# csiro-crop-informatics/biokanga

Hardware: AMD Instinct MI355X
Metric: aligned reads/s (SAM-identical) on 100 bp SE vs GRCh38, 1->8 MI355X (higher is better)
Workload: dtype u8

## Files before the change

biokanga_amd/csrc/bk_ctx_int.h:

```cpp
#pragma once
#include <atomic>
#include <thread>
#include <hip/hip_runtime.h>

#include <cstdio>
#include <string>
#include <vector>

#include "bk_device.h"
#include "bk_devbuf.h"

#define HIP_TRY(expr)                                                                              \
    do {                                                                                           \
        hipError_t e__ = (expr);                                                                   \
        if (e__ != hipSuccess) {                                                                   \
            fprintf(stderr, "biokanga_amd: %s failed: %s (%s:%d)\n", #expr, hipGetErrorString(e__), __FILE__, __LINE__); \
            return e__ == hipErrorOutOfMemory ? BK_ERR_MEM : BK_ERR_INTERNAL;                      \
        }                                                                                          \
    } while (0)

namespace bk {
struct BatchBufs {
    DevBuf<uint64_t> rd4, rd2, iv_first;
    DevBuf<uint2> iv2, iv32;
    DevBuf<uint32_t> iv_n, rmeta;
    DevBuf<uint32_t> act[2], heavy, wave, wave_work;
    DevBuf<uint32_t> stage[3], stripe_cnt;
    DevBuf<uint32_t> slist, slist_stage;
    DevBuf<uint32_t> sort[3];
    DevBuf<uint8_t> sort_tmp, scan_tmp;
    DevBuf<bk_seg2> seg2;
    DevBuf<uint8_t> in_bases;
    DevBuf<uint64_t> in_offs;
    DevBuf<uint32_t> in_lens;
    DevBuf<bk_hit> in_out;
    DevBuf<uint16_t> in_lens16;
    DevBuf<uint32_t> in_words;
    DevBuf<bk_nbase> in_exc;
    DevBuf<bk_snp_site> snp_sites;
    DevBuf<bk_site_req> site_reqs;
    DevBuf<bk_site_res> site_res;
    DevBuf<uint8_t> chrom_accept;
    DevBuf<unsigned long long> htab;
    DevBuf<uint32_t> slot_epoch;
    DevBuf<uint2> plan;
};
struct ImageBufs {
    DevBuf<uint64_t> tgt4, tgt2, tgt2s;
    DevBuf<uint32_t> sa_lo, isa;
    DevBuf<uint8_t> sa_hi, nflag;
    DevBuf<uint64_t> ent_start, ent_end;
    DevBuf<uint32_t> ent_id, id2idx;
    DevBuf<uint8_t> ktab;
    DevBuf<uint64_t> ktab_hi;
    DevBuf<uint32_t> k2, kx[kMoreKeys];
    DevBuf<uint8_t> swin;
    DevBuf<uint32_t> swmap;
    DevBuf<uint32_t> grow_kx[kMoreKeys];
    DevBuf<uint8_t> grow_ktab2;
};
struct FixedBufs {
    DevBuf<uint32_t> small;
    DevBuf<PhaseCtl> ctl;
    DevBuf<unsigned long long> seq_counts, ctr, ctr_aux, snp_tot;
    DevBuf<unsigned long long> seq_global;
    DevBuf<uint32_t> snp_planes;
};
}

struct bk_ctx {
    int device = 0;
    hipStream_t stream = nullptr;
    bk_align_params params{};
    bk::DevAlignCfg cfg{};
    bk::DevIndex ix{};
    bk::ImageBufs image;
    bk::FixedBufs fixed;
    void release_image_buffers() { image = bk::ImageBufs{}; fixed = bk::FixedBufs{}; }
    uint64_t n_tgt4_words = 0;
    uint32_t cap_rd2w = 0;
    int use_tgt2 = 2;
    int sort_lists = 7;
    bool sort_lists_set = false;
    int sort_shift = 0;
    int use_k2 = 1;
    int use_k3 = bk::kMoreKeys;
    bool grow_enabled = false, grow_wait = false;
    uint64_t grow_after = 5 * BK_POLICY_MIN_READS, grow_seen = 0;
    std::atomic<int> grow_state{0};
    std::thread grow_thread;
    bk::DevIndex grow_ix{};
    bool grow_want_ktab2 = false;
    bool grow_elem = false, grow_want_elem = false;
    int use_ktab2 = 1;
    bool ktab_is2 = false;
    int use_iv32 = 1;
    uint32_t wave_waves = 256u * 8u * 4u;
    int use_isa = 1;
    int use_swin = 1;
    uint64_t swin_budget = 0;
    int swin_skip_short = 0;
    int swin_w = 0;
    uint64_t swin_bytes = 0;
    double swin_setup_s = 0;
    double swin_covered = 0;
    bool swin_denied = false;
    bool swin_rebuilt = false;
    int iv_poison = 0;
    int use_wave = 1;
    int lazy_search = 1;
    bool ktab64 = false;
    int ktab_wide = 0;
    int k_req = -1;
    int use_ktab = 1;
    uint32_t el_size = 4;
    uint64_t tot_seq_len = 0;
    std::string dataset;
    std::vector<bk_entry_info> entries;
    std::vector<bk_snp_site> snp_sites;

    bk::BatchBufs buf;
    void release_batch_buffers() { buf = bk::BatchBufs{}; }
    uint32_t cap_reads = 0, cap_wpr = 0, cap_iv_cores = 0;
    uint32_t *h_small = nullptr;
    bk::PhaseCtl *h_ctl = nullptr;
    hipEvent_t ev_ctl = nullptr;
    bool ctl_pending = false, hist_valid = false;
    uint32_t ctl_pending_reads = 0, ctl_pending_maxlen = 0;
    int ctl_pending_phases = 0;
    double hist_slist[bk::kMaxPhases] = {0}, hist_wave[bk::kMaxPhases] = {0};
    int async_error = 0;
    int async_phases = 1;
    bool force_rccl = false;
    uint64_t rccl_allreduces = 0;
    int rccl_ranks = 0;
    uint2 *h_plan = nullptr;
    size_t h_plan_cap = 0;
    uint32_t plan_maxlen = 0;
    int plan_key[4] = {-1, -1, -1, -1};
    hipEvent_t ev_plan = nullptr;
    bk::HeavyScratch hs{};
    int max_read_len = 500;
    uint32_t last_maxlen = 0;
    int dbg_stop_phase = -1, dbg_phase = 0, dbg_cur = 0;
    uint32_t dbg_n = 0, dbg_ivc = 0;
    bool dbg_valid = false;
    bool debug = false;
    uint32_t chunk_reads = 64u << 20;
    uint64_t site_chunk = 8u << 20;

    hipEvent_t ev_wait = nullptr;
    bool entries_set = false, tgt2_built = false;
    bool tables_built = false;
    bool tables_under_way = false;
    void *sam_text[2] = {nullptr, nullptr};
    uint64_t sam_text_cap = 0;
    uint32_t n_chrom_accept = 0;
    bk_timing timing{};
    std::vector<hipEvent_t> ev_pool;
    std::vector<uint64_t> loci_offs;
    std::vector<bk_loci> loci;
    std::vector<bk_loci_trims> loci_trims;
    std::vector<bk_seg2> seg2;
};


namespace bk {
struct DevReads {
    const uint8_t *bases = nullptr;
    const uint64_t *offs = nullptr;
    const uint32_t *lens = nullptr;
    const uint32_t *words = nullptr;
    const bk_nbase *exc = nullptr;
    uint64_t n_exc = 0;
};
int engine_align_device(bk_ctx *c, const DevReads &in, uint32_t nreads, bk_hit *d_out, hipStream_t s, uint32_t maxlen_known = 0);
void release_swin(bk_ctx *c);
void drop_swin(bk_ctx *c);
int engine_pair_device(bk_ctx *c, const DevReads &in, uint32_t n_pairs, bk_hit *d_hits, uint32_t maxlen, const bk_pe_params *pe, hipStream_t s,
                       bk_seg2 *seg2_host = nullptr, bk_seg2 *seg2_dev = nullptr);
int engine_prepare_packed(bk_ctx *c, const uint16_t *d_lens16, uint32_t nreads, uint64_t n_words, const bk_nbase *d_exc, uint64_t n_exc,
                          uint32_t *d_lens32, uint64_t *d_offs, uint32_t *maxlen, hipStream_t s);
}

namespace bk {
hipError_t dev_malloc_bytes(void **p, size_t bytes);
hipError_t dev_zero_now(void *p, size_t bytes);
template <class T> inline hipError_t dev_malloc(T **p, size_t bytes) { return dev_malloc_bytes(reinterpret_cast<void **>(p), bytes); }
int upload_host(void *d_dst, const void *h_src, size_t bytes, int device);
int upload_file(void *d_dst, int fd, uint64_t file_ofs, size_t bytes, int device);
bool host_is_pinned(const void *p);
}
```

biokanga_amd/csrc/bk_dev_k2.h:

```cpp
#pragma once
#include "bk_dev_util.h"

namespace bk {


constexpr uint32_t kKindShift = 30;
constexpr uint32_t kKindK2 = 1;
constexpr uint32_t kKindDeep = 2;
constexpr uint32_t kKindFull = 3;
constexpr uint32_t kInlineBucket = 16;
constexpr int kK2Bases = 15;
constexpr uint32_t kK2Above = 0xFFFFFFFFu;

constexpr uint64_t kTab2BitmapMax = 64;
__device__ __forceinline__ bool ktab2_absent(uint32_t bitmap, uint32_t m, uint32_t q2)
{
    const uint32_t m5 = m >> 27, lo5 = (q2 >> 27) & m5, hi5 = lo5 | (~m5 & 31u);
    const uint32_t upto = hi5 == 31u ? 0xFFFFFFFFu : (1u << (hi5 + 1)) - 1u;
    return (bitmap & upto & ~((1u << lo5) - 1u)) == 0u;
}

__device__ __forceinline__ int k2_cmp(uint32_t key, uint32_t m, uint32_t q2)
{
    if (key == kK2Above) return 1;
    key &= m;
    return key < q2 ? -1 : (key > q2 ? 1 : 0);
}
__device__ __forceinline__ bool k2_nkind(uint32_t key) { return key != kK2Above && (key & 3u) == 1u; }

__host__ __device__ __forceinline__ uint32_t k2_mask(int rem2)
{
    const int L = rem2 < kK2Bases ? rem2 : kK2Bases;
    return L <= 0 ? 0u : ~0u << (32 - 2 * L);
}

__device__ __forceinline__ uint32_t k2_make(const uint64_t *__restrict__ tgt4, uint64_t pos, int k)
{
    const uint64_t w0 = nib16(tgt4, pos);
    if (w0 & top_mask(k) & 0x4444444444444444ULL) return kK2Above;
    const uint64_t w1 = nib16(tgt4, pos + (uint64_t)k);
    const uint64_t bad = w1 & 0x4444444444444440ULL;
    const uint32_t code = squeeze2(w1) & ~3u;
    if (!bad) return code;
    const int j = __clzll((long long)bad) >> 2;
    return ((code | (0xFFFFFFFFu >> (2 * j))) & ~3u) | 1u;
}


#ifdef BK_DIAG_B
#define BK_K2_LINE(ctr) (ctr)++
#else
#define BK_K2_LINE(ctr) (void)0
#endif
__device__ __forceinline__ void k2_count_range(const uint32_t *__restrict__ L, uint64_t a, uint64_t b, uint32_t m, uint32_t q2, uint32_t &n_lt, uint32_t &n_le,
                                               unsigned long long &lines)
{
    n_lt = 0; n_le = 0;
    (void)lines;
    for (uint64_t base = a & ~15ULL; base < b; base += 16) {
        const uint4 *__restrict__ p = reinterpret_cast<const uint4 *>(L + base);
        const uint4 v0 = p[0], v1 = p[1], v2 = p[2], v3 = p[3];
        BK_K2_LINE(lines);
        const uint32_t key[16] = {v0.x, v0.y, v0.z, v0.w, v1.x, v1.y, v1.z, v1.w, v2.x, v2.y, v2.z, v2.w, v3.x, v3.y, v3.z, v3.w};
        const uint32_t lo = a > base ? (uint32_t)(a - base) : 0u, hi = b - base < 16 ? (uint32_t)(b - base) : 16u;
#pragma unroll
        for (uint32_t j = 0; j < 16; j++) {
            const bool in = j >= lo && j < hi;
            const uint32_t km = key[j] == kK2Above ? 0xFFFFFFFFu : (key[j] & m);
            n_lt += (in && km < q2) ? 1u : 0u;
            n_le += (in && km <= q2) ? 1u : 0u;
        }
        if ((uint64_t)n_le < base + hi - a) break;
    }
}

__device__ __forceinline__ void k2_bounds(const uint32_t *__restrict__ k2, const uint64_t *lv, uint64_t first, uint64_t cnt, uint32_t m, uint32_t q2,
                                          uint64_t &lb, uint64_t &ub, unsigned long long &lines)
{
    uint64_t l1 = first, h1 = first + cnt, l2 = l1, h2 = h1;
    int ktop = cnt >= 16 ? (63 - __clzll((long long)cnt)) >> 2 : 0;
    if (ktop > kK2Levels) ktop = kK2Levels;
    for (int j = ktop; j >= 0; j--) {
        const int sh = 4 * j;
        const uint32_t *__restrict__ L = j ? k2 + lv[j] : k2;
        const uint64_t a1 = l1 >> sh, b1 = h1 >> sh, a2 = l2 >> sh, b2 = h2 >> sh;
        uint32_t lt = 0, le = 0;
        if (a1 < b1) {
            k2_count_range(L, a1, b1, m, q2, lt, le, lines);
            const uint64_t g = a1 + lt;
            if (lt) l1 = g << sh;
            if (g < b1) h1 = ((g + 1) << sh) - 1;
        }
        if (a2 < b2) {
            if (a2 != a1 || b2 != b1) { uint32_t lt2; k2_count_range(L, a2, b2, m, q2, lt2, le, lines); }
            const uint64_t g = a2 + le;
            if (le) l2 = g << sh;
            if (g < b2) h2 = ((g + 1) << sh) - 1;
        }
    }
    lb = l1;
    ub = l2;
}

__device__ __forceinline__ uint32_t kx_make(const uint64_t *__restrict__ tgt4, uint64_t pos, int from, uint32_t before)
{
    if (before == kK2Above || (before & 3u) != 0u) return kK2Above;
    const uint64_t w1 = nib16(tgt4, pos + (uint64_t)from);
    const uint64_t bad = w1 & 0x4444444444444440ULL;
    const uint32_t code = squeeze2(w1) & ~3u;
    if (!bad) return code;
    const int j = __clzll((long long)bad) >> 2;
    return ((code | (0xFFFFFFFFu >> (2 * j))) & ~3u) | 1u;
}

template <typename Row>
__device__ __forceinline__ int cmp_core_from(const Row &rdw, int ofs, int cl, int start,
                                             const uint64_t *__restrict__ tgt, uint64_t pos)
{
    for (int i = start; i < cl; i += 16) {
        uint64_t m = top_mask(cl - i);
        uint64_t p = row_nib16(rdw, ofs + i) & m;
        uint64_t t = nib16(tgt, pos + i) & m;
        if (p != t) return p < t ? -1 : 1;
    }
    return 0;
}

}
```

biokanga_amd/csrc/bk_dev_util.h:

```cpp
#pragma once
#include "bk_device.h"

namespace bk {


__device__ __forceinline__ uint64_t nib16(const uint64_t *__restrict__ w, uint64_t pos)
{
    uint64_t i = pos >> 4;
    unsigned s = (unsigned)(pos & 15) << 2;
    uint64_t a = w[i];
    uint64_t b = w[i + 1];
    return (a << s) | ((b >> 1) >> (63 - s));
}

__device__ __forceinline__ uint64_t top_mask(int nibs)
{
    return nibs >= 16 ? ~0ULL : (~0ULL << (64 - 4 * nibs));
}

__device__ __forceinline__ uint64_t spread2to4(uint32_t v)
{
    uint64_t x = v;
    x = (x | (x << 16)) & 0x0000FFFF0000FFFFULL;
    x = (x | (x << 8)) & 0x00FF00FF00FF00FFULL;
    x = (x | (x << 4)) & 0x0F0F0F0F0F0F0F0FULL;
    x = (x | (x << 2)) & 0x3333333333333333ULL;
    return x;
}

__device__ __forceinline__ uint64_t bits64_2(const uint64_t *__restrict__ w, int pos)
{
    const int i = pos >> 5;
    const unsigned s = (unsigned)(pos & 31) << 1;
    const uint64_t a = w[i], b = w[i + 1];
    return (a << s) | ((b >> 1) >> (63 - s));
}

struct RdRow {
    const uint64_t *p;
    bool four;
    __device__ __forceinline__ uint64_t nib16(int pos) const
    {
        return four ? bk::nib16(p, (uint64_t)pos) : spread2to4((uint32_t)(bits64_2(p, pos) >> 32));
    }
    __device__ __forceinline__ uint64_t word16(int k) const
    {
        if (four) return p[k];
        const uint64_t v = p[k >> 1];
        return spread2to4((k & 1) ? (uint32_t)v : (uint32_t)(v >> 32));
    }
};

__device__ __forceinline__ RdRow read_row(const DevBatch &b, uint32_t r, int strand, bool has_n)
{
    RdRow q;
    q.four = b.rd2 == nullptr || has_n;
    q.p = q.four ? b.rd4 + ((uint64_t)r * 2 + strand) * b.wpr : b.rd2 + ((uint64_t)r * 2 + strand) * (b.nw / 2);
    return q;
}

__device__ __forceinline__ uint64_t iv_slot(const DevBatch &b, uint32_t a, int st, int c)
{
    return (uint64_t)(st * (int)b.iv_cores + c) * b.iv_stride + a;
}

__device__ __forceinline__ uint32_t iv_count(const DevBatch &b, uint64_t slot)
{
    return b.iv2 ? b.iv2[slot].y : b.iv_n[slot];
}
__device__ __forceinline__ uint64_t iv_start(const DevBatch &b, uint64_t slot)
{
    return b.iv2 ? (uint64_t)b.iv2[slot].x : b.iv_first[slot];
}
__device__ __forceinline__ void iv_get(const DevBatch &b, uint64_t slot, uint64_t &first, uint32_t &n)
{
    if (b.iv2) { const uint2 v = b.iv2[slot]; first = v.x; n = v.y; }
    else { first = b.iv_first[slot]; n = b.iv_n[slot]; }
}
__device__ __forceinline__ void iv_put(const DevBatch &b, uint64_t slot, uint64_t first, uint32_t n)
{
    if (b.iv2) b.iv2[slot] = make_uint2((uint32_t)first, n);
    else { b.iv_first[slot] = first; b.iv_n[slot] = n; }
}

__device__ __forceinline__ uint32_t stripe_reserve(const StripeSet &l, int li, uint32_t n)
{
    return atomicAdd(&l.cnt[(blockIdx.x & (kListStripes - 1)) * 16 + li], n);
}
__device__ __forceinline__ void stripe_put(const StripeSet &l, int li, uint32_t at, uint32_t v)
{
    l.stage[li][(uint64_t)(blockIdx.x & (kListStripes - 1)) * l.cap + at] = v;
}
__device__ __forceinline__ uint32_t stripe_reserve_tile(const StripeSet &l, int li, uint32_t n, uint64_t tile)
{
    return atomicAdd(&l.cnt[(uint32_t)(tile & (kListStripes - 1)) * 16 + li], n);
}
__device__ __forceinline__ void stripe_put_tile(const StripeSet &l, int li, uint32_t at, uint32_t v, uint64_t tile)
{
    l.stage[li][(tile & (kListStripes - 1)) * l.cap + at] = v;
}
__device__ __forceinline__ void stripe_max(const StripeSet &l, uint32_t v)
{
    atomicMax(&l.cnt[(kListStripes + (blockIdx.x & (kListStripes - 1))) * 16], v);
}

__device__ __forceinline__ uint32_t ctr_stripe() { return (blockIdx.x & (kCtrStripes - 1)) * 8; }

template <bool WIDE>
__device__ __forceinline__ uint64_t sa_get(const DevIndex &ix, uint64_t i)
{
    uint64_t v = ix.sa_lo[i];
    if (WIDE) v |= (uint64_t)ix.sa_hi[i] << 32;
    return v;
}

__device__ __forceinline__ uint64_t row_nib16(const uint64_t *__restrict__ rdw, int pos) { return nib16(rdw, (uint64_t)pos); }
__device__ __forceinline__ uint64_t row_nib16(const RdRow &rdw, int pos) { return rdw.nib16(pos); }

template <typename Row>
__device__ __forceinline__ int cmp_core(const Row &rdw, int ofs, int cl, uint64_t p0,
                                        const uint64_t *__restrict__ tgt, uint64_t pos)
{
    uint64_t t0 = nib16(tgt, pos) & top_mask(cl);
    if (p0 != t0) return p0 < t0 ? -1 : 1;
    for (int i = 16; i < cl; i += 16) {
        uint64_t m = top_mask(cl - i);
        uint64_t p = row_nib16(rdw, ofs + i) & m;
        uint64_t t = nib16(tgt, pos + i) & m;
        if (p != t) return p < t ? -1 : 1;
    }
    return 0;
}

struct LdsEntries {
    uint64_t start[128], end[128];
    bool on;
};
__device__ __forceinline__ void lds_entries_load(LdsEntries &le, const DevIndex &ix)
{
    le.on = ix.n_ent <= 128;
    if (le.on)
        for (uint32_t i = threadIdx.x; i < ix.n_ent; i += blockDim.x) { le.start[i] = ix.ent_start[i]; le.end[i] = ix.ent_end[i]; }
    __syncthreads();
}

__device__ __forceinline__ int find_entry(const DevIndex &ix, uint64_t t)
{
    int lo = 0, hi = (int)ix.n_ent - 1;
    while (lo <= hi) {
        int mid = (lo + hi) >> 1;
        if (t < ix.ent_start[mid]) hi = mid - 1;
        else if (t > ix.ent_end[mid]) lo = mid + 1;
        else return mid;
    }
    return -1;
}

__device__ __forceinline__ int find_entry_lds(const LdsEntries &le, const DevIndex &ix, uint64_t t)
{
    if (!le.on) return find_entry(ix, t);
    int lo = 0, hi = (int)ix.n_ent - 1;
    while (lo <= hi) {
        int mid = (lo + hi) >> 1;
        if (t < le.start[mid]) hi = mid - 1;
        else if (t > le.end[mid]) lo = mid + 1;
        else return mid;
    }
    return -1;
}

__device__ __forceinline__ int hamming(const uint64_t *__restrict__ rdw, int len, const uint64_t *__restrict__ tgt,
                                       uint64_t t, int limit)
{
    int mm = 0;
    for (int i = 0; i < len; i += 16) {
        uint64_t x = (nib16(rdw, i) ^ nib16(tgt, t + i)) & top_mask(len - i);
        x = (x | (x >> 1) | (x >> 2) | (x >> 3)) & 0x1111111111111111ULL;
        mm += __popcll(x);
        if (mm > limit) break;
    }
    return mm;
}

__device__ __forceinline__ int hamming_eos(const uint64_t *__restrict__ rdw, int len, const uint64_t *__restrict__ tgt,
                                           uint64_t t, int limit)
{
    int mm = 0;
    uint64_t eos = 0;
    for (int i = 0; i < len; i += 16) {
        const uint64_t w = nib16(tgt, t + i), m = top_mask(len - i);
        eos |= w & (w >> 1) & (w >> 2) & m & 0x1111111111111111ULL;
        uint64_t x = (nib16(rdw, i) ^ w) & m;
        x = (x | (x >> 1) | (x >> 2) | (x >> 3)) & 0x1111111111111111ULL;
        mm += __popcll(x);
    }
    return (eos || mm > limit) ? 127 : mm;
}

__device__ __forceinline__ uint32_t squeeze2(uint64_t x)
{
    x &= 0x3333333333333333ULL;
    x = (x | (x >> 2)) & 0x0F0F0F0F0F0F0F0FULL;
    x = (x | (x >> 4)) & 0x00FF00FF00FF00FFULL;
    x = (x | (x >> 8)) & 0x0000FFFF0000FFFFULL;
    x = (x | (x >> 16)) & 0x00000000FFFFFFFFULL;
    return (uint32_t)x;
}

__device__ __forceinline__ uint32_t flags_to_bits16(uint64_t f)
{
    uint64_t g = __brevll(f) >> 3;
    g = (g | (g >> 3)) & 0x0303030303030303ULL;
    g = (g | (g >> 6)) & 0x000F000F000F000FULL;
    g = (g | (g >> 12)) & 0x000000FF000000FFULL;
    g = (g | (g >> 24)) & 0xFFFFULL;
    return (uint32_t)g;
}

__device__ __forceinline__ uint64_t ktab_get(const DevIndex &ix, uint64_t c)
{
    if (ix.ktab2) return (uint64_t)ix.ktab2[c].x;
    if (ix.ktab_hi) return ix.ktab_hi[c >> 16] + (uint64_t)ix.ktab32[c];
    return ix.ktab32 ? (uint64_t)ix.ktab32[c] : ix.ktab64[c];
}

__device__ __forceinline__ void ktab_get_pair(const DevIndex &ix, uint64_t c, uint64_t &lo, uint64_t &hi)
{
    if (ix.ktab_hi && !ix.ktab2) {
        const uint64_t base = ix.ktab_hi[c >> 16];
        const uint32_t o0 = ix.ktab32[c], o1 = ix.ktab32[c + 1];
        lo = base + o0;
        hi = ((c + 1) & 0xFFFFULL) ? base + o1 : ix.ktab_hi[(c + 1) >> 16];
        return;
    }
    lo = ktab_get(ix, c);
    hi = ktab_get(ix, c + 1);
}

__device__ __forceinline__ void core_range(const DevIndex &ix, uint64_t p0, int cl, uint64_t &lo, uint64_t &hi)
{
    lo = 0;
    hi = ix.n;
    int k = ix.k;
    if (k <= 0) return;
    int kk = cl < k ? cl : k;
    if (p0 & 0x4444444444444444ULL & top_mask(kk)) return;
    uint32_t code = squeeze2(p0);
    uint64_t c_lo = (uint64_t)(code >> (32 - 2 * kk)) << (2 * (k - kk));
    uint64_t c_hi = c_lo | ((1ULL << (2 * (k - kk))) - 1);
    lo = ktab_get(ix, c_lo);
    hi = ktab_get(ix, c_hi + 1);
}

template <bool WIDE, typename Row>
__device__ __forceinline__ void search_core(const DevIndex &ix, const Row &rdw, int ofs, int cl,
                                            uint64_t cap, uint64_t &first, uint64_t &count)
{
    uint64_t p0 = row_nib16(rdw, ofs) & top_mask(cl);
    uint64_t lo, hi;
    core_range(ix, p0, cl, lo, hi);
    uint64_t end = hi;
    while (lo < hi) {
        uint64_t mid = lo + ((hi - lo) >> 1);
        int c = cmp_core(rdw, ofs, cl, p0, ix.tgt4, sa_get<WIDE>(ix, mid));
        if (c > 0) lo = mid + 1;
        else hi = mid;
    }
    first = lo;
    count = 0;
    if (lo >= end) return;
    if (cmp_core(rdw, ofs, cl, p0, ix.tgt4, sa_get<WIDE>(ix, lo)) != 0) return;
    if (end - lo == 1) { count = 1; return; }
    uint64_t limit = end - lo < cap ? end : lo + cap;
    uint64_t cur = lo, step = 1;
    while (cur + step < limit && cmp_core(rdw, ofs, cl, p0, ix.tgt4, sa_get<WIDE>(ix, cur + step)) == 0) {
        cur += step;
        step <<= 1;
    }
    uint64_t l2 = cur + 1, h2 = cur + step < limit ? cur + step : limit;
    while (l2 < h2) {
        uint64_t mid = l2 + ((h2 - l2) >> 1);
        if (cmp_core(rdw, ofs, cl, p0, ix.tgt4, sa_get<WIDE>(ix, mid)) == 0) l2 = mid + 1;
        else h2 = mid;
    }
    count = l2 - lo;
}

__device__ __forceinline__ int classify(int low_inst, int low_mm, int nxt, int init, int mm_delta, int max_hits)
{
    if (low_inst == 0 && low_mm == init) return BK_HR_NONE;
    if (low_inst >= 1 && (nxt - low_mm) < mm_delta) return BK_HR_MMDELTA;
    if (low_inst > max_hits) return BK_HR_HITINSTS;
    return BK_HR_HITS;
}

__device__ __forceinline__ void write_result(const DevIndex &ix, const DevAlignCfg &cfg, const DevBatch &b, uint32_t r,
                                             int len, int rslt, int low_inst, int low_mm, int nxt, uint64_t hit_left,
                                             int hit_ent, int hit_strand, int diag)
{
    bk_hit h;
    h.chrom_id = 0; h.match_loci = 0; h.match_len = 0; h.low_hit_instances = 0;
    h.rslt = (uint8_t)rslt; h.nar = BK_NAR_NOHIT; h.strand = '?'; h.low_mm = 0; h.nxt_low_mm = 0;
    h.num_hits = 0; h.mismatches = 0;
    h.flags = (uint8_t)diag;
    if (low_inst > cfg.max_hits) low_inst = cfg.max_hits + 1;
    switch (rslt) {
    case BK_HR_HITS:
        if (low_inst == 1) {
            h.nar = BK_NAR_ACCEPTED;
            h.num_hits = 1;
            h.strand = (uint8_t)hit_strand;
            h.chrom_id = ix.ent_id[hit_ent];
            h.match_loci = (uint32_t)(hit_left - ix.ent_start[hit_ent]);
            h.match_len = (uint16_t)len;
            h.mismatches = (uint8_t)low_mm;
        } else
            h.nar = BK_NAR_MULTIALIGN;
        break;
    case BK_HR_MMDELTA:
        h.nar = BK_NAR_MMDELTA;
        h.match_len = (uint16_t)len;
        break;
    case BK_HR_HITINSTS:
        h.nar = BK_NAR_MULTIALIGN;
        h.match_len = (uint16_t)len;
        break;
    default:
        break;
    }
    h.low_hit_instances = (int16_t)low_inst;
    h.low_mm = (int8_t)low_mm;
    h.nxt_low_mm = (int8_t)nxt;
    b.out[r] = h;
}

__device__ __forceinline__ uint64_t uniform64(uint64_t v)
{
    uint32_t lo = __builtin_amdgcn_readfirstlane((uint32_t)v), hi = __builtin_amdgcn_readfirstlane((uint32_t)(v >> 32));
    return ((uint64_t)hi << 32) | lo;
}

constexpr uint32_t kLazyBucket = 4;
constexpr uint32_t kLazyFlag = 0x80000000u;
constexpr uint32_t kElemFlag = 0x40000000u;
constexpr uint32_t kIvFlags = kLazyFlag | kElemFlag;
constexpr int kWaveGrab = 8;

void launch_fill_u64(unsigned long long *p, uint64_t n, unsigned long long v, hipStream_t s);
void launch_pack_rows(const DevBatch &b, hipStream_t s, const uint32_t *pairs = nullptr, uint32_t n_pairs = 0);
struct CompactJobs { StripeSet set; uint32_t *dense[3]; uint32_t *total[3]; uint32_t *max_out; int n; };
inline uint32_t stripe_cap(unsigned blocks, unsigned per_block) { return ((blocks + kListStripes - 1) / kListStripes) * per_block; }
void launch_compact(const StripeSet &set, uint32_t *const *dense, uint32_t *const *total, int n, uint32_t *max_out, hipStream_t s);
void expand_rd4(const DevBatch &b, const uint32_t *list, uint32_t n_list, hipStream_t s);

}
```

biokanga_amd/csrc/bk_device.h:

```cpp
#pragma once
#include <hip/hip_runtime.h>
#include <stdint.h>

#include "../../include/biokanga_amd.h"

namespace bk {

constexpr int kMoreKeys = 2;
constexpr int kK2Levels = 7;

__host__ __device__ __forceinline__ uint64_t k2s_pad(uint64_t words) { return (words + 15) & ~15ULL; }
__host__ __device__ __forceinline__ uint64_t k2s_count(uint64_t n, int j) { return (n + (1ULL << (4 * j)) - 1) >> (4 * j); }
__host__ __device__ __forceinline__ uint64_t k2s_start(uint64_t n, int j)
{
    uint64_t o = k2s_pad(n) + 16;
    for (int i = 1; i < j; i++) o += k2s_pad(k2s_count(n, i)) + 16;
    return o;
}


constexpr int kListStripes = 64;
struct StripeSet {
    uint32_t *cnt;
    uint32_t *stage[3];
    uint32_t cap;
};
constexpr int kCtrStripes = 64;
constexpr int kNwLong = 20;
constexpr int kNwLongest = 32;
constexpr int kPackedPadWords = 32;
constexpr int kMaxCoresFast = 16;
constexpr int kWave = 64;
constexpr int kMaxReadLenAbs = 2000;
constexpr uint32_t kNodeCap = 1024000;
constexpr uint64_t kEosWord = 0x7777777777777777ULL;
constexpr int kSwBases = 192, kSwPre = 92, kSwLen = 100;
template <int E> struct SwGeo { static constexpr int bases = 64 * E, pre = E == 3 ? 92 : 32 * E; };
template <int E> __host__ __device__ inline uint64_t sw_word_at(uint64_t idx, int q) { return (idx >> 5) * (32ULL * E) + (uint64_t)q * 32 + (idx & 31); }
constexpr int kSwBlkShift = 5;
constexpr uint32_t kSwNone = 0xFFFFFFFFu;
constexpr uint32_t kSwMinRun = 65, kSwHead = 192;
constexpr int kSwLevels = 8;
constexpr uint32_t kReadHasN = 1u << 15;
constexpr uint32_t kReadLenMask = kReadHasN - 1;

struct DevIndex {
    const uint64_t *tgt4;
    const uint64_t *tgt2;
    const uint64_t *tgt2s;
    const uint8_t *nflag;
    int flag_shift;
    uint32_t nflag_bytes;
    const uint32_t *sa_lo;
    const uint8_t *sa_hi;
    const uint64_t *ent_start;
    const uint64_t *ent_end;
    const uint32_t *ent_id;
    const uint32_t *id2idx;
    uint32_t max_id;
    const uint32_t *ktab32;
    const uint64_t *ktab64;
    const uint64_t *ktab_hi;
    const uint2 *ktab2;
    int ktab2_elem;
    const uint32_t *k2;
    const uint32_t *kx[kMoreKeys];
    const uint32_t *isa;
    const uint4 *swin;
    int sw_words;
    const uint32_t *swmap;
    uint64_t n;
    uint32_t n_ent;
    int k;
};

struct DevAlignCfg {
    int max_subs, mm_delta, align_strand, max_ns, max_hits;
    int min_core_len, slides_per100, max_iter;
    int heavy_thresh;
};

struct DevBatch {
    const uint8_t *bases;
    const uint64_t *offs;
    const uint32_t *lens;
    const uint32_t *pk_words;
    const bk_nbase *pk_exc;
    uint64_t pk_nexc;
    uint32_t pk_read0;
    uint64_t *rd4;
    uint64_t *rd2;
    uint32_t *rmeta;
    uint64_t *iv_first;
    uint32_t *iv_n;
    uint2 *iv2;
    uint32_t iv_stride;
    const uint32_t *act;
    uint32_t *wave_work;
    uint2 *iv32;
    bk_hit *out;
    unsigned long long *seq_counts;
    unsigned long long *ctr;
    uint32_t wpr;
    uint32_t n_reads;
    uint32_t nw;
    uint32_t iv_cores;
    const uint2 *plan;
    uint32_t plan_stride;
    uint32_t plan_n;
};

struct PhaseCtl {
    uint32_t n_act;
    uint32_t cmax;
    uint32_t n_slist;
    uint32_t n_wave;
    uint32_t n_heavy;
    uint32_t wave_cursor, heavy_cursor;
    uint32_t pad[9];
};
constexpr int kMaxPhases = 72;

struct HeavyScratch {
    unsigned long long *htab;
    uint32_t *slot_epoch;
    uint32_t tab_size;
    uint32_t n_slots;
};

struct ReadPlan {
    int len, max_tot_mm, core_len, core_delta, max_slides, n_loop, n_phases;
};

__host__ __device__ inline ReadPlan make_plan(int len, const DevAlignCfg &c)
{
    ReadPlan p;
    p.len = len;
    int m = c.max_subs == 0 ? 0 : (int)(0.5 + (double)(len * c.max_subs) / 100.0);
    if (c.max_subs != 0 && m < 1) m = 1;
    if (m > 63) m = 63;
    p.max_tot_mm = m;
    int cl = len / (c.mm_delta == 1 ? m + 1 : m + 2);
    p.core_len = cl > c.min_core_len ? cl : c.min_core_len;
    int ms = (c.slides_per100 * len + 99) / 100;
    p.max_slides = ms > 1 ? ms : 1;
    int cd = len / p.max_slides - 1;
    p.core_delta = cd > p.core_len ? cd : p.core_len;
    p.n_loop = 0;
    int has_final = 1;
    if (m > 0) {
        int a;
        for (a = 0; a <= m; a++) {
            if (len / (a + c.mm_delta) <= p.core_len) break;
            p.n_loop++;
        }
        has_final = a <= m;
    }
    p.n_phases = p.n_loop + has_final;
    return p;
}

__host__ __device__ inline void phase_params(const ReadPlan &p, const DevAlignCfg &c, int phase, int &mm, int &cl, int &cd)
{
    if (phase < p.n_loop) {
        mm = phase;
        cl = p.len / (phase + c.mm_delta);
        cd = cl;
    } else {
        mm = p.max_tot_mm;
        cl = p.core_len;
        cd = p.core_delta;
    }
}

__host__ __device__ inline int core_offsets(int plen, int cl, int cd, int max_slides, int *ofs, int maxn)
{
    int cur = cd, o = 0, n = 0;
    while (n < max_slides && o <= plen - cl && cur > cl / 3) {
        if (o + cl + cur > plen) cur = plen - (o + cl);
        n++;
        o += cur;
    }
    const int last = plen - cl;
    for (int i = 0; i < maxn; i++) {
        int v = i * cd;
        ofs[i] = v < last ? v : last;
    }
    return n;
}

}
```

biokanga_amd/csrc/bk_engine_int.h:

```cpp
#pragma once
#include <hip/hip_runtime.h>
#include <fcntl.h>
#include <unistd.h>
#include "bk_prim.h"

#include <algorithm>
#include <cstdio>
#include <cstdlib>
#include <ctime>
#include <cstring>
#include <map>
#include <mutex>
#include <string>
#include <atomic>
#include <thread>
#include <type_traits>
#include <vector>

#include <dlfcn.h>
#include <rccl/rccl.h>

#include "bk_ctx_int.h"
#include "bk_cpus.h"
#include "bk_wait.h"
#include "bk_env.h"
#include "sfx_file.h"


namespace bk {
void launch_pack_target(const uint8_t *seq, uint64_t n, uint64_t *tgt4, uint64_t nwords, hipStream_t s);
void launch_pack_target2(const uint64_t *tgt4, uint64_t nwords4, uint64_t *tgt2, unsigned int *nflag32, int flag_shift, hipStream_t s);
void launch_split_sa5(const uint8_t *sa5, uint64_t n, uint32_t *lo, uint8_t *hi, hipStream_t s);
void launch_build_ktab(const DevIndex &ix, void *tab, int k, bool tab64, hipStream_t s, uint64_t i0 = 0, uint64_t i1 = 0, unsigned long long *starts = nullptr, bool pairs = false);
void launch_fill_ktab2_y(void *tab2, const uint32_t *k2, uint64_t n_entries, hipStream_t s, const uint32_t *sa_elem = nullptr);
void launch_max_len(const uint32_t *lens, uint32_t n, uint32_t *out, hipStream_t s);
void launch_widen_lens(const uint16_t *lens16, uint32_t n, uint32_t *lens32, unsigned long long *nwords, hipStream_t s);
void launch_check_exc(const bk_nbase *exc, uint64_t n_exc, const uint32_t *lens, uint32_t n_reads, uint32_t *bad, hipStream_t s);
void launch_packed_extent(const uint64_t *offs, const uint32_t *lens, uint32_t n, unsigned long long *out, hipStream_t s);
void launch_snp_pileup(const DevIndex &ix, const uint8_t *bases, const uint64_t *offs, const uint32_t *id2idx, const bk_snp_aln *alns, uint64_t n_alns,
                       uint32_t *planes, hipStream_t s);
void launch_site_octamers(const DevIndex &ix, const bk_site_req *reqs, uint64_t n, int32_t rel_ofs, bk_site_res *out, hipStream_t s);
void launch_snp_gather(const DevIndex &ix, const uint32_t *planes, uint64_t g0, uint32_t n, uint32_t *out, hipStream_t s);
void launch_snp_centroids(const DevIndex &ix, const uint32_t *planes, uint64_t g0, uint32_t chrom_len, uint32_t min_reads, uint32_t *hist, hipStream_t s);
void launch_snp_sites(const DevIndex &ix, const uint32_t *planes, uint64_t g0, uint32_t chrom_len, uint32_t min_reads, double min_prop,
                      bk_snp_site *sites, uint32_t cap, uint32_t *n_sites, unsigned long long *totals, hipStream_t s);
void launch_count_seqs(const bk_hit *out, uint32_t n, const uint32_t *id2idx, uint32_t n_ent, unsigned long long *counts, hipStream_t s);
void launch_fill_u64(unsigned long long *p, uint64_t n, unsigned long long v, hipStream_t s);
void launch_prep(const DevAlignCfg &cfg, const DevBatch &b, uint32_t *act, uint32_t *act_cnt, uint32_t *cmax, uint32_t *stage,
                 uint32_t *stripe_cnt, hipStream_t s);
void launch_search(const DevIndex &ix, const DevAlignCfg &cfg, const DevBatch &b, const uint32_t *act, uint32_t n_act,
                   int phase, int cmax, int nstr, int lazy, hipStream_t s);
void launch_extend(const DevIndex &ix, const DevAlignCfg &cfg, const DevBatch &b, const uint32_t *act, uint32_t n_act,
                   int phase, uint32_t *next_act, uint32_t *next_cnt, uint32_t *heavy, uint32_t *heavy_cnt,
                   uint32_t *cmax_next, hipStream_t s);
void launch_build_isa(const uint32_t *sa, uint64_t n, uint32_t *isa, hipStream_t s, uint64_t i0 = 0, uint64_t i1 = 0);
void launch_build_swin(const DevIndex &ix, void *swin, int words, hipStream_t s);
void launch_swin_breaks(const DevIndex &ix, const int *w, int n_levels, unsigned long long *const *brk, uint64_t a, uint64_t e, uint64_t n_words,
                        const unsigned long long *starts, hipStream_t s);
void launch_swin_cover(const unsigned long long *brk, uint64_t n, uint32_t max_run, uint32_t min_run, uint32_t *flags, uint64_t n_blocks, int first_level, hipStream_t s);
void launch_pack_ktab64(const uint64_t *tab, uint64_t n_entries, uint32_t *off, uint64_t *hi, uint32_t *overflow, hipStream_t s);
void launch_count_nonzero(const uint32_t *flags, uint64_t n, unsigned long long *count, hipStream_t s);
void launch_swin_map(const uint32_t *flags, const uint32_t *incl, uint64_t n_blocks, uint32_t cap_blocks, uint32_t *used, uint32_t *map, hipStream_t s);
void launch_swin_fill(const DevIndex &ix, const uint32_t *map, void *swin, int words, uint64_t a, uint64_t e, hipStream_t s);
void launch_build_k2(const DevIndex &ix, uint32_t *k2, uint32_t *k3, uint32_t *k4, unsigned long long *bad, hipStream_t s, uint64_t i0 = 0, uint64_t i1 = 0, bool write_k2 = true);
void launch_build_k2_levels(uint32_t *k2, uint64_t n, hipStream_t s);
void launch_make_ktab2(const uint32_t *tab, const uint32_t *k2, uint64_t n_entries, uint64_t n, void *out, hipStream_t s, const uint32_t *sa_elem = nullptr);
void launch_search_a(const DevIndex &ix, const DevAlignCfg &cfg, const DevBatch &b, const uint32_t *act, const uint32_t *p_n_act, uint32_t n_act_bound,
                     int phase, int cmax, int nstr, int lazy, uint32_t *list, uint32_t *list_cnt, uint32_t *stage, uint32_t *stripe_cnt,
                     hipStream_t s);
void launch_search_b(const DevIndex &ix, const DevAlignCfg &cfg, const DevBatch &b, int phase, int lazy, const uint32_t *list, const uint32_t *sorted,
                     uint32_t n_sorted, const uint32_t *p_n_list, uint64_t n_bound, hipStream_t s);
void launch_clear_iv(const DevBatch &b, const uint32_t *p_n_act, uint32_t n_act_bound, int cmax, int st0, int st1, uint32_t word, hipStream_t s);
void launch_pe(const DevIndex &ix, const DevAlignCfg &cfg, const DevBatch &b, int pe_mode, int min_len, int max_len, int pair_strand,
               bk_hit *hits, uint32_t n_pairs, uint32_t *orphans, uint32_t *counters, uint32_t *h_count, bk_seg2 *seg2, int min_chim,
               int long_reads, const uint8_t *accept, uint32_t n_accept, hipStream_t s);
void launch_flat(const DevIndex &ix, const DevAlignCfg &cfg, const DevBatch &b, const uint32_t *act, const uint32_t *p_n_act, uint32_t n_act_bound, int phase,
                 int slots_max, uint32_t *next_act, uint32_t *next_cnt, uint32_t *heavy, uint32_t *heavy_cnt, uint32_t *wave,
                 uint32_t *wave_cnt, uint32_t *cmax_next, uint32_t *const *stage, uint32_t *stripe_cnt, int nw, hipStream_t s);
void launch_wave(const DevIndex &ix, const DevAlignCfg &cfg, const DevBatch &b, const HeavyScratch &hs, const uint32_t *list, const uint32_t *sorted,
                 uint32_t n_sorted, const uint32_t *p_n_list, uint32_t n_bound, int phase, uint32_t *cursor, uint32_t *next_act, uint32_t *next_cnt,
                 uint32_t *cmax_next, int nw, uint32_t max_waves, hipStream_t s);
void launch_heavy(const DevIndex &ix, const DevAlignCfg &cfg, const DevBatch &b, const HeavyScratch &hs, const uint32_t *list,
                  uint32_t n_list, int phase, uint32_t *cursor, uint32_t *next_act, uint32_t *next_cnt, uint32_t *cmax_next,
                  hipStream_t s);
int build_sa_device(const uint8_t *d_seq, uint64_t n, void *d_sa_out, int el_size, hipStream_t s);
int scan_counts_u64(const unsigned long long *in, unsigned long long *out, uint32_t n, void *tmp, size_t *tmp_bytes, hipStream_t s);
void launch_loci_count(const bk_hit *out, uint32_t n, int clamp_to, unsigned long long *cnt, hipStream_t s);
void launch_best(const DevIndex &ix, const DevAlignCfg &cfg, const DevBatch &b, const HeavyScratch &hs, const uint32_t *list,
                 uint32_t n_list, uint32_t *cursor, unsigned long long *cnt, bk_loci *dense, hipStream_t s);
void launch_indel(const DevIndex &ix, const DevAlignCfg &cfg, const DevBatch &b, uint32_t n, int max_indel, int max_junct, int keep_state, uint32_t *list,
                  uint32_t *list_cnt_dev, uint32_t *list_cnt_host, uint32_t *cursor, bk_seg2 *seg2, hipStream_t s);
void launch_unaligned_list(const bk_hit *out, uint32_t n, uint32_t *list, uint32_t *cnt, hipStream_t s);
void launch_chimeric(const DevIndex &ix, const DevAlignCfg &cfg, const DevBatch &b, const HeavyScratch &hs, const uint32_t *list, uint32_t n_list,
                     int min_pct, int long_reads, uint32_t *cursor, bk_seg2 *seg2, hipStream_t s);
void launch_loci_compact(const bk_loci *dense, uint32_t width, const unsigned long long *offs, uint32_t n, bk_loci *out, hipStream_t s);
void launch_loci_single(const bk_hit *out, uint32_t n, const unsigned long long *offs, bk_loci *loci, uint32_t *list, uint32_t *list_cnt,
                        const bk_seg2 *seg2, bk_loci_trims *trims, hipStream_t s);
void launch_loci_enum(const DevIndex &ix, const DevAlignCfg &cfg, const DevBatch &b, const HeavyScratch &hs, const uint32_t *list,
                      uint32_t n_list, uint32_t *cursor, const unsigned long long *offs, bk_loci *loci, uint32_t *err, int min_pct, int long_reads,
                      bk_seg2 *seg2, bk_loci_trims *trims, hipStream_t s);
int sort_list_by_key(const uint32_t *keys_in, uint32_t *keys_out, const uint32_t *vals_in, uint32_t *vals_out, uint32_t n,
                     void *tmp, size_t *tmp_bytes, hipStream_t s);
void launch_keys_search(const DevBatch &b, const uint32_t *list, const uint32_t *p_n, uint32_t n_sort, int shift, uint32_t *keys, hipStream_t s);
void launch_keys_wave(const DevAlignCfg &cfg, const DevBatch &b, int phase, const uint32_t *list, const uint32_t *p_n, uint32_t n_sort, int shift, uint32_t *keys,
                      const uint32_t *work_of, hipStream_t s);

struct StageClock {
    bool on = env::timing();
    double t0 = now();
    static double now() { timespec ts; clock_gettime(CLOCK_MONOTONIC, &ts); return (double)ts.tv_sec + 1e-9 * (double)ts.tv_nsec; }
    static double wall() { timespec ts; clock_gettime(CLOCK_REALTIME, &ts); return (double)(ts.tv_sec % 60) + 1e-9 * (double)ts.tv_nsec; }
    void lap(const char *what) { if (!on) return; const double t = now(); fprintf(stderr, "bk timing: %-28s %7.1f ms   (done at :%06.3f)\n", what, 1e3 * (t - t0), wall()); t0 = t; }
};


inline uint32_t words_per_read(uint32_t maxlen)
{
    return ((maxlen + 15) / 16 + 2) & ~1u;
}

inline uint32_t iv_cores_for(const bk_ctx *c, uint32_t maxlen)
{
    const uint32_t ms = std::max(1u, ((uint32_t)c->cfg.slides_per100 * maxlen + 99) / 100);
    return std::min<uint32_t>(ms, kMaxCoresFast);
}

inline uint32_t rd2w_for(uint32_t maxlen)
{
    return maxlen <= 128 ? 4u : (maxlen <= 256 ? 8u : (maxlen <= 16u * (uint32_t)kNwLong ? (uint32_t)kNwLong / 2 : (uint32_t)kNwLongest / 2));
}

inline uint64_t scratch_bytes_per_read(uint32_t wpr, uint32_t rd2w = 8, uint32_t iv_cores = kMaxCoresFast)
{
    return 2ULL * wpr * 8 + 2ULL * rd2w * 8 + 2ULL * iv_cores * (12 + 8) + 52 + 24;
}


int derive_cfg(bk_ctx *c);
hipError_t clear_dev(void *p, size_t bytes, hipStream_t s);
struct TablePlan {
    bool ktab = false, k2 = false, isa = false;
    bool ktab2 = false;
    int kx = 0;
    int k = 0;
    DevBuf<unsigned long long> d_bad;
};

int tables_begin(bk_ctx *c, TablePlan &tp);
int tables_range(bk_ctx *c, const TablePlan &tp, uint64_t i0, uint64_t i1, unsigned long long *bucket_starts = nullptr);
int tables_end(bk_ctx *c, TablePlan &tp);
int build_tables(bk_ctx *c);
int build_tgt2(bk_ctx *c);
void publish_index(bk_ctx *c);
void grow_take_in(bk_ctx *c);
void grow_drop(bk_ctx *c);
void grow_tick(bk_ctx *c, uint64_t nreads, bool now = false);
int setup_entries(bk_ctx *c, const bk_entry_info *entries, uint32_t n_entries);
int finish_ctx(bk_ctx *c, const bk_entry_info *entries, uint32_t n_entries);
int new_ctx(bk_ctx **out, int device_id, const bk_align_params *p, bk_ctx **pc);
int adopt_device_image(bk_ctx *c, const uint8_t *d_seq, uint64_t n, const uint8_t *d_sa, int el);
int maybe_build_swin(bk_ctx *c, uint32_t maxlen, uint32_t nreads, hipStream_t s);
int size_heavy_scratch(bk_ctx *c);
int ensure_batch_scratch(bk_ctx *c, uint32_t n_reads, uint32_t wpr, uint32_t rd2w = 0, uint32_t iv_cores = kMaxCoresFast);
int ensure_sort_scratch(bk_ctx *c, uint32_t n, hipStream_t s);
int ensure_slist(bk_ctx *c, uint64_t lanes, hipStream_t s);
int plan_table_for(bk_ctx *c, uint32_t maxlen, hipStream_t s);
bool plan_table_covers(const bk_ctx *c, uint32_t maxlen);
inline int ensure_seg2(bk_ctx *c, uint32_t n) { HIP_TRY(c->buf.seg2.ensure(n)); return BK_OK; }
struct HostExtent {
    uint64_t lo = ~0ULL, hi = 0;
    uint32_t maxlen = 0;
    std::vector<uint64_t> rel;
};
HostExtent host_extent(const uint64_t *offs, const uint32_t *lens, uint32_t nreads);
int align_device(bk_ctx *c, const DevReads &in, uint32_t nreads, bk_hit *d_out, hipStream_t s, uint32_t maxlen_known = 0, bool enqueue_only = false);
}
```

biokanga_amd/csrc/bk_env.h:

```cpp
#pragma once
#include <cstdlib>

namespace bk {
namespace env {

inline bool set(const char *name) { return getenv(name) != nullptr; }
inline unsigned long long u64(const char *name, unsigned long long dflt)
{
    const char *e = getenv(name);
    if (!e) return dflt;
    const unsigned long long v = strtoull(e, nullptr, 10);
    return v ? v : dflt;
}

inline bool timing() { static const bool v = set("BK_TIMING"); return v; }
inline bool debug_phases() { return set("BK_DEBUG"); }
inline int poison() { static const int v = set("BK_POISON") ? atoi(getenv("BK_POISON")) : -1; return v; }
inline bool inflate_debug() { static const bool v = set("BK_INFLATE_DEBUG"); return v; }
inline unsigned long long grow_after_reads() { return u64("BK_GROW_AFTER_READS", 0); }
inline unsigned long long table_slices() { return u64("BK_TABLE_SLICES", 0); }
inline unsigned long long sa_wide_chunk() { return u64("BK_SA_WIDE_CHUNK", 0); }
inline unsigned long long sam_device_min(unsigned long long dflt) { const char *e = getenv("BK_SAM_DEVICE_MIN"); return e ? strtoull(e, nullptr, 10) : dflt; }
inline unsigned long long sam_early_min(unsigned long long dflt) { const char *e = getenv("BK_SAM_EARLY_MIN"); return e ? strtoull(e, nullptr, 10) : dflt; }
inline bool sam_device_fail() { return set("BK_SAM_DEVICE_FAIL"); }
inline unsigned long long inflate_piece_min(unsigned long long dflt) { const char *e = getenv("BK_INFLATE_PIECE_MIN"); return e ? strtoull(e, nullptr, 10) : dflt; }
inline int local_world_size() { static const int v = [] { const char *e = getenv("LOCAL_WORLD_SIZE"); const int r = e ? atoi(e) : 1; return r > 1 ? r : 1; }(); return v; }

}
}
```

biokanga_amd/csrc/bk_image.cpp:

```cpp
#include "bk_engine_int.h"

#define SW_TRY(x) do { hipError_t e_ = (x); if (e_ != hipSuccess) { (void)hipGetLastError(); return e_ == hipErrorOutOfMemory ? BK_ERR_MEM : BK_ERR_INTERNAL; } } while (0)

namespace bk {
hipError_t dev_zero_now(void *p, size_t bytes)
{
    hipError_t e = hipMemset(p, 0, bytes);
    if (e == hipSuccess) e = hipStreamSynchronize(nullptr);
    return e;
}

hipError_t dev_malloc_bytes(void **p, size_t bytes)
{
    const int poison = env::poison();
    const bool timing = env::timing();
    timespec ta, tb;
    if (timing) clock_gettime(CLOCK_MONOTONIC, &ta);
    hipError_t e = hipMalloc(p, bytes);
    if (timing) {
        clock_gettime(CLOCK_MONOTONIC, &tb);
        const double ms = 1e3 * (double)(tb.tv_sec - ta.tv_sec) + 1e-6 * (double)(tb.tv_nsec - ta.tv_nsec);
        if (ms > 2.0) fprintf(stderr, "bk timing: hipMalloc of %.2f GB took %.1f ms\n", (double)bytes / 1e9, ms);
    }
    if (e == hipSuccess && poison >= 0 && bytes) {
        e = hipMemset(*p, poison & 0xff, bytes);
        if (e == hipSuccess) e = hipDeviceSynchronize();
    }
    return e;
}


int derive_cfg(bk_ctx *c)
{
    const bk_align_params &p = c->params;
    if (p.max_subs < 0 || p.max_subs > 25 || p.min_edit_dist < 1 || p.min_edit_dist > 2 || p.align_strand < 0 ||
        p.align_strand > 2 || p.pmode < 0 || p.pmode > 3 || p.max_ns < 0 || p.max_ns > 5)
        return BK_ERR_PARAMS;
    if (p.max_ml < 0 || p.max_ml > BK_MAX_ML) return BK_ERR_PARAMS;
    if (p.best_matches && p.max_ml < 2) return BK_ERR_PARAMS;
    if (p.micro_indel_len < 0 || p.micro_indel_len > 20) return BK_ERR_PARAMS;
    if ((p.micro_indel_len || p.splice_junct_len) && p.max_ml > 1 && p.best_matches) return BK_ERR_PARAMS;
    if (p.min_chimeric_len != 0 && (p.min_chimeric_len < 50 || p.min_chimeric_len > 99)) return BK_ERR_PARAMS;
    if (p.min_chimeric_len != 0 && p.max_ml > 1 && p.best_matches) return BK_ERR_PARAMS;
    if (p.splice_junct_len != 0 && (p.splice_junct_len < 25 || p.splice_junct_len > 100000)) return BK_ERR_PARAMS;
    DevAlignCfg &g = c->cfg;
    g.max_subs = p.max_subs;
    g.mm_delta = p.min_edit_dist;
    g.align_strand = p.align_strand;
    g.max_ns = p.max_ns;
    g.max_hits = p.max_ml > 1 ? p.max_ml : 1;
    uint64_t t = c->tot_seq_len;
    int m;
    if (t <= 500000ULL) m = 4;
    else if (t <= 20000000ULL) m = 7;
    else if (t <= 250000000ULL) m = 11;
    else if (t <= 3500000000ULL) m = 12;
    else m = 15;
    switch (p.pmode) {
    case 2: g.slides_per100 = 9; break;
    case 1: m += 1; g.slides_per100 = 8; break;
    case 0: m += 2; g.slides_per100 = 8; break;
    default: m += 4; g.slides_per100 = 6; break;
    }
    g.min_core_len = m;
    switch (p.pmode) {
    case 0: g.max_iter = 5000; break;
    case 1: g.max_iter = 10000; break;
    case 2: g.max_iter = 20000; break;
    default: g.max_iter = 2500; break;
    }
    if (g.heavy_thresh < 0 || g.heavy_thresh > 100) g.heavy_thresh = 64;
    return BK_OK;
}


void free_dev(void *p)
{
    if (!p) return;
    const bool timing = env::timing();
    timespec ta, tb;
    if (timing) clock_gettime(CLOCK_MONOTONIC, &ta);
    (void)hipFree(p);
    if (timing) {
        clock_gettime(CLOCK_MONOTONIC, &tb);
        const double ms = 1e3 * (double)(tb.tv_sec - ta.tv_sec) + 1e-6 * (double)(tb.tv_nsec - ta.tv_nsec);
        if (ms > 2.0) fprintf(stderr, "bk timing: hipFree took %.1f ms\n", ms);
    }
}

hipError_t clear_dev(void *p, size_t bytes, hipStream_t s)
{
    if (bytes < (1ULL << 30) || ((uintptr_t)p & 7)) {
        for (size_t at = 0; at < bytes; at += (1ULL << 30)) {
            hipError_t e = hipMemsetAsync((uint8_t *)p + at, 0, std::min<size_t>(1ULL << 30, bytes - at), s);
            if (e != hipSuccess) return e;
        }
        return hipSuccess;
    }
    const size_t words = bytes / 8;
    launch_fill_u64((unsigned long long *)p, words, 0ULL, s);
    hipError_t e = hipGetLastError();
    if (e == hipSuccess && (bytes & 7)) e = hipMemsetAsync((uint8_t *)p + words * 8, 0, bytes & 7, s);
    return e;
}


int pick_k(uint64_t n)
{
    int k = 1;
    while (k < 16 && (1ULL << (2 * k)) < n) k++;
    return k < 8 ? 8 : k;
}


void publish_index(bk_ctx *c)
{
    const ImageBufs &im = c->image;
    DevIndex &ix = c->ix;
    ix.tgt4 = im.tgt4.get(); ix.sa_lo = im.sa_lo.get(); ix.sa_hi = im.sa_hi.get();
    ix.ent_start = im.ent_start.get(); ix.ent_end = im.ent_end.get(); ix.ent_id = im.ent_id.get(); ix.id2idx = im.id2idx.get();
    const bool tabs = !c->tables_under_way;
    const void *kt = tabs ? im.ktab.get() : nullptr;
    const bool packed = c->ktab64 && im.ktab_hi.get() != nullptr, pairs = !c->ktab64 && c->ktab_is2;
    ix.ktab64 = c->ktab64 && !packed ? static_cast<const uint64_t *>(kt) : nullptr;
    ix.ktab_hi = packed ? im.ktab_hi.get() : nullptr;
    ix.ktab2 = pairs ? static_cast<const uint2 *>(kt) : nullptr;
    ix.ktab32 = packed || (!c->ktab64 && !pairs) ? static_cast<const uint32_t *>(kt) : nullptr;
    ix.k2 = tabs ? im.k2.get() : nullptr;
    for (int i = 0; i < kMoreKeys; i++) ix.kx[i] = tabs ? im.kx[i].get() : nullptr;
    ix.ktab2_elem = (ix.ktab2 != nullptr && c->use_ktab2 >= 2 && im.sa_hi.get() == nullptr && ix.k2 != nullptr) ? 1 : 0;
    ix.isa = tabs ? im.isa.get() : nullptr; ix.tgt2 = im.tgt2.get(); ix.tgt2s = im.tgt2s.get(); ix.nflag = im.nflag.get();
    ix.swin = reinterpret_cast<const uint4 *>(im.swin.get()); ix.swmap = im.swmap.get();
}

void grow_worker(bk_ctx *c)
{
    int st = 3;
    hipStream_t s = nullptr;
    DevBuf<unsigned long long> d_bad;
    ImageBufs &im = c->image;
    do {
        if (hipSetDevice(c->device) != hipSuccess || hipStreamCreateWithFlags(&s, hipStreamNonBlocking) != hipSuccess) break;
        const DevIndex &ix = c->grow_ix;
        const uint64_t n = ix.n;
        const uint64_t n_keys = k2s_start(n, kK2Levels + 1), need = n_keys * 4;
        int nk = 0;
        if (ix.k2 != nullptr && ix.kx[0] == nullptr) {
            for (int i = 0; i < kMoreKeys; i++) {
                size_t free_b = 0, total_b = 0;
                if (hipMemGetInfo(&free_b, &total_b) != hipSuccess || need > free_b || free_b - need < total_b / 5) break;
                if (im.grow_kx[i].ensure(n_keys) != hipSuccess) { (void)hipGetLastError(); break; }
                nk = i + 1;
            }
        }
        if (nk) {
            unsigned long long bad2[2] = {0, 0};
            bool ok = d_bad.ensure(2) == hipSuccess && hipMemsetAsync(d_bad.get(), 0, 16, s) == hipSuccess;
            if (ok) {
                launch_build_k2(ix, const_cast<uint32_t *>(ix.k2), im.grow_kx[0].get(), nk > 1 ? im.grow_kx[1].get() : nullptr, d_bad.get(), s, 0, n, false);
                ok = hipMemcpyAsync(bad2, d_bad.get(), 16, hipMemcpyDeviceToHost, s) == hipSuccess && hipStreamSynchronize(s) == hipSuccess && !bad2[0] && !bad2[1];
            }
            if (ok) {
                for (int i = 0; i < nk; i++) launch_build_k2_levels(im.grow_kx[i].get(), n, s);
                ok = hipStreamSynchronize(s) == hipSuccess;
            }
            if (!ok) {
                (void)hipGetLastError();
                for (auto &b : im.grow_kx) b.reset();
                nk = 0;
            }
        }
        if (c->grow_want_ktab2 && ix.k2 != nullptr && ix.ktab32 != nullptr) {
            const uint64_t n_entries = (1ULL << (2 * ix.k)) + 1;
            size_t free_b = 0, total_b = 0;
            if (hipMemGetInfo(&free_b, &total_b) == hipSuccess && n_entries * 8 + (total_b / 5) < free_b && im.grow_ktab2.ensure(n_entries * 8) == hipSuccess) {
                launch_make_ktab2(ix.ktab32, ix.k2, n_entries, n, im.grow_ktab2.get(), s, c->grow_want_elem ? ix.sa_lo : nullptr);
                if (hipStreamSynchronize(s) != hipSuccess) { (void)hipGetLastError(); im.grow_ktab2.reset(); }
            } else
                (void)hipGetLastError();
        }
        st = (nk || im.grow_ktab2.get()) ? 2 : 3;
    } while (false);
    if (s) (void)hipStreamDestroy(s);
    c->grow_state.store(st, std::memory_order_release);
}

void grow_take_in(bk_ctx *c)
{
    if (c->grow_thread.joinable()) c->grow_thread.join();
    if (c->grow_state.load(std::memory_order_acquire) == 2) {
        ImageBufs &im = c->image;
        for (int i = 0; i < kMoreKeys; i++)
            if (im.grow_kx[i].get()) im.kx[i] = std::move(im.grow_kx[i]);
        if (im.kx[0].get()) c->use_k3 = kMoreKeys;
        if (im.grow_ktab2.get()) {
            (void)hipDeviceSynchronize();
            im.ktab = std::move(im.grow_ktab2);
            c->ktab_is2 = true;
            c->use_ktab2 = c->grow_want_elem ? 2 : 1;
        }
        publish_index(c);
        if (!c->sort_lists_set) c->sort_lists = (c->sort_lists & ~1) | (c->ix.kx[0] == nullptr ? 1 : 0);
        if (env::timing())
            fprintf(stderr, "biokanga_amd: long-run tables taken in after %llu reads: %d key array(s) behind the second-level keys%s\n",
                    (unsigned long long)c->grow_seen, (c->ix.kx[0] != nullptr) + (c->ix.kx[1] != nullptr), c->ix.ktab2 ? ", first keys in the k-mer table" : "");
    }
    c->grow_state.store(4, std::memory_order_release);
}

void grow_drop(bk_ctx *c)
{
    if (c->grow_thread.joinable()) c->grow_thread.join();
    for (auto &b : c->image.grow_kx) b.reset();
    c->image.grow_ktab2.reset();
    if (c->grow_state.load() != 0) c->grow_state.store(4);
}

void grow_tick(bk_ctx *c, uint64_t nreads, bool now)
{
    if (!c->grow_enabled) return;
    const int st = c->grow_state.load(std::memory_order_acquire);
    if (st != 0 && st != 4) c->grow_seen += nreads;
    if (st == 0) {
        c->grow_seen += nreads;
        if ((now || c->grow_seen >= c->grow_after) && c->tables_built && c->ix.k2 != nullptr) {
            c->grow_ix = c->ix;
            c->grow_want_ktab2 = !c->ktab64 && !c->ktab_is2;
            c->grow_want_elem = c->grow_elem && c->image.sa_hi.get() == nullptr;
            c->grow_state.store(1);
            c->grow_thread = std::thread(grow_worker, c);
        }
    } else if (st == 2 || st == 3 || (st == 1 && c->grow_wait))
        grow_take_in(c);
}

int tables_begin(bk_ctx *c, TablePlan &tp)
{
    ImageBufs &im = c->image;
    grow_drop(c);
    im.ktab.reset(); im.ktab_hi.reset(); im.k2.reset(); im.isa.reset();
    for (auto &b : im.kx) b.reset();
    c->ktab_is2 = false;
    c->ix.k = 0;
    c->tables_under_way = true;
    publish_index(c);
    if (c->use_ktab) {
        int k = c->k_req > 0 ? c->k_req : pick_k(c->ix.n);
        if (k > 16) k = 16;
        if (k < 2) k = 2;
        const uint64_t ncodes = 1ULL << (2 * k);
        c->ktab64 = c->ix.n >= (1ULL << 32) || c->ktab_wide != 0;
        const uint64_t ktab_bytes = (ncodes + 1) * (c->ktab64 ? 8 : 4);
        const uint64_t need = k2s_start(c->ix.n, kK2Levels + 1) * 4;
        const bool want_isa = c->use_wave && c->use_isa && im.sa_hi.get() == nullptr && c->ix.n < (1ULL << 32);
        size_t free_b = 0, total_b = 0;
        HIP_TRY(hipMemGetInfo(&free_b, &total_b));
        uint64_t planned = ktab_bytes;
        auto fits = [&](uint64_t more) { return planned + more <= free_b && free_b - planned - more >= total_b / 5; };
        if (c->use_k2 && fits(need)) { tp.k2 = true; planned += need; }
        if (want_isa) planned += c->ix.n * 4;
        for (int i = 0; tp.k2 && i < kMoreKeys && i < c->use_k3; i++) {
            if (!fits(need)) break;
            tp.kx = i + 1;
            planned += need;
        }
        if (tp.k2 && c->use_ktab2 && !c->ktab64 && fits(ktab_bytes)) tp.ktab2 = true;
        HIP_TRY(im.ktab.ensure((size_t)ktab_bytes * (tp.ktab2 ? 2 : 1)));
        tp.ktab = true;
        tp.k = k;
        if (tp.k2) {
            HIP_TRY(im.k2.ensure(need / 4));
            HIP_TRY(tp.d_bad.ensure(2));
            HIP_TRY(hipMemsetAsync(tp.d_bad.get(), 0, 16, c->stream));
            for (int i = 0; i < tp.kx; i++) HIP_TRY(im.kx[i].ensure(need / 4));
        }
    }
    if (c->use_wave && c->use_isa && im.sa_hi.get() == nullptr && c->ix.n < (1ULL << 32)) {
        HIP_TRY(im.isa.ensure(c->ix.n));
        tp.isa = true;
    }
    return BK_OK;
}

int tables_range(bk_ctx *c, const TablePlan &tp, uint64_t i0, uint64_t i1, unsigned long long *bucket_starts)
{
    DevIndex ix = c->ix;
    ix.k = tp.k;
    const bool last = i1 >= c->ix.n;
    const ImageBufs &im = c->image;
    if (tp.ktab) launch_build_ktab(ix, im.ktab.get(), tp.k, c->ktab64, c->stream, i0, last ? c->ix.n + 1 : i1, bucket_starts, tp.ktab2);
    if (tp.k2) launch_build_k2(ix, im.k2.get(), tp.kx > 0 ? im.kx[0].get() : nullptr, tp.kx > 1 ? im.kx[1].get() : nullptr, tp.d_bad.get(), c->stream, i0, i1);
    if (tp.isa) launch_build_isa(im.sa_lo.get(), c->ix.n, im.isa.get(), c->stream, i0, i1);
    HIP_TRY(hipGetLastError());
    return BK_OK;
}

int tables_end(bk_ctx *c, TablePlan &tp)
{
    ImageBufs &im = c->image;
    unsigned long long bad2[2] = {0, 0};
    if (tp.k2) HIP_TRY(hipMemcpyAsync(bad2, tp.d_bad.get(), 16, hipMemcpyDeviceToHost, c->stream));
    HIP_TRY(hipStreamSynchronize(c->stream));
    if (tp.ktab && c->ktab64 && c->ktab_wide != 2) {
        const uint64_t n_entries = (1ULL << (2 * tp.k)) + 1, n_hi = (n_entries >> 16) + 2;
        DevBuf<uint8_t> d_off;
        DevBuf<uint64_t> d_hi;
        DevBuf<uint32_t> d_flag;
        uint32_t flag = 1;
        if (d_off.ensure(n_entries * 4) == hipSuccess && d_hi.ensure(n_hi) == hipSuccess && d_flag.ensure(1) == hipSuccess &&
            hipMemsetAsync(d_flag.get(), 0, 4, c->stream) == hipSuccess) {
            launch_pack_ktab64((const uint64_t *)im.ktab.get(), n_entries, (uint32_t *)d_off.get(), d_hi.get(), d_flag.get(), c->stream);
            if (hipMemcpyAsync(&flag, d_flag.get(), 4, hipMemcpyDeviceToHost, c->stream) != hipSuccess || hipStreamSynchronize(c->stream) != hipSuccess) flag = 1;
        }
        (void)hipGetLastError();
        d_flag.reset();
        if (flag == 0) {
            im.ktab = std::move(d_off);
            im.ktab_hi = std::move(d_hi);
        }
    }
    if (tp.ktab) {
        c->ktab_is2 = tp.ktab2;
        c->ix.k = tp.k;
    }
    const unsigned long long bad = bad2[0];
    if (tp.kx && (bad || bad2[1])) {
        if (!bad) fprintf(stderr, "biokanga_amd: suffix array not in nibble order at %llu place(s) beyond the second-level keys; third-level keys disabled\n", bad2[1]);
        for (auto &b : im.kx) b.reset();
        tp.kx = 0;
    }
    if (tp.k2 && bad) {
        fprintf(stderr, "biokanga_amd: suffix array not in nibble order inside %llu k-mer bucket(s); second-level keys disabled\n", bad);
        im.k2.reset();
    } else if (tp.k2) {
        launch_build_k2_levels(im.k2.get(), c->ix.n, c->stream);
        for (int i = 0; i < tp.kx; i++) launch_build_k2_levels(im.kx[i].get(), c->ix.n, c->stream);
        HIP_TRY(hipGetLastError());
    }
    c->tables_under_way = false;
    publish_index(c);
    if (tp.ktab2) {
        launch_fill_ktab2_y(im.ktab.get(), im.k2.get(), (1ULL << (2 * tp.k)) + 1, c->stream, c->ix.ktab2_elem ? im.sa_lo.get() : nullptr);
        HIP_TRY(hipGetLastError());
    }
    HIP_TRY(hipStreamSynchronize(c->stream));
    if (!c->sort_lists_set) c->sort_lists = (c->sort_lists & ~1) | (c->ix.kx[0] == nullptr ? 1 : 0);
    c->tables_built = true;
    return BK_OK;
}

int build_tables(bk_ctx *c)
{
    TablePlan tp;
    int rc = tables_begin(c, tp);
    if (!rc) rc = tables_range(c, tp, 0, c->ix.n);
    if (!rc) rc = tables_end(c, tp);
    return rc;
}

int build_tgt2(bk_ctx *c)
{
    ImageBufs &im = c->image;
    im.tgt2.reset(); im.nflag.reset(); im.tgt2s.reset();
    publish_index(c);
    if (!c->use_tgt2) return BK_OK;
    const uint64_t nblocks = c->n_tgt4_words / 4;
    static_assert(16 * kNwLongest <= 512, "a register-kernel window must not span more than two flag regions");
    int shift = 9;
    while ((((nblocks * 64) >> shift) + 7) / 8 > 16384) shift++;
    const uint64_t flag_bytes = (((((nblocks * 64) >> shift) + 1) + 31) / 32) * 4 + 16;
    HIP_TRY(im.tgt2.ensure(nblocks * 2 + 8));
    HIP_TRY(im.nflag.ensure(flag_bytes));
    HIP_TRY(hipMemsetAsync(im.nflag.get(), 0, flag_bytes, c->stream));
    HIP_TRY(hipMemsetAsync(im.tgt2.get() + nblocks * 2, 0, 64, c->stream));
    launch_pack_target2(im.tgt4.get(), c->n_tgt4_words, im.tgt2.get(), (unsigned int *)im.nflag.get(), shift, c->stream);
    HIP_TRY(hipGetLastError());
    HIP_TRY(hipStreamSynchronize(c->stream));
    c->ix.nflag_bytes = (uint32_t)flag_bytes;
    if (c->use_tgt2 >= 2) {
        HIP_TRY(im.tgt2s.ensure(nblocks * 2 + 8));
        HIP_TRY(clear_dev(im.tgt2s.get(), nblocks * 16 + 64, c->stream));
        HIP_TRY(hipMemcpyAsync(im.tgt2s.get(), im.tgt2.get() + 4, (nblocks * 2 - 4) * 8, hipMemcpyDeviceToDevice, c->stream));
        HIP_TRY(hipStreamSynchronize(c->stream));
    }
    c->ix.flag_shift = shift;
    publish_index(c);
    return BK_OK;
}


int setup_entries(bk_ctx *c, const bk_entry_info *entries, uint32_t n_entries)
{
    StageClock clk0;
    c->entries.assign(entries, entries + n_entries);
    c->tot_seq_len = 0;
    std::vector<uint64_t> es(n_entries), ee(n_entries);
    std::vector<uint32_t> ei(n_entries);
    for (uint32_t i = 0; i < n_entries; i++) {
        es[i] = entries[i].start_ofs;
        ee[i] = entries[i].end_ofs;
        ei[i] = entries[i].entry_id;
        c->tot_seq_len += entries[i].seq_len;
        if (i && es[i] <= ee[i - 1]) return BK_ERR_PARAMS;
    }
    ImageBufs &im = c->image; FixedBufs &fx = c->fixed;
    HIP_TRY(im.ent_start.ensure(n_entries));
    HIP_TRY(im.ent_end.ensure(n_entries));
    HIP_TRY(im.ent_id.ensure(n_entries));
    HIP_TRY(hipMemcpy(im.ent_start.get(), es.data(), n_entries * 8, hipMemcpyHostToDevice));
    HIP_TRY(hipMemcpy(im.ent_end.get(), ee.data(), n_entries * 8, hipMemcpyHostToDevice));
    HIP_TRY(hipMemcpy(im.ent_id.get(), ei.data(), n_entries * 4, hipMemcpyHostToDevice));
    {
        uint32_t max_id = 0;
        for (uint32_t i = 0; i < n_entries; i++) max_id = std::max(max_id, ei[i]);
        if ((uint64_t)max_id > 16ULL * n_entries + (1u << 20)) return BK_ERR_PARAMS;
        std::vector<uint32_t> map((size_t)max_id + 1, 0xFFFFFFFFu);
        for (uint32_t i = 0; i < n_entries; i++) map[ei[i]] = i;
        HIP_TRY(im.id2idx.ensure(map.size()));
        HIP_TRY(hipMemcpy(im.id2idx.get(), map.data(), map.size() * 4, hipMemcpyHostToDevice));
        c->ix.max_id = max_id;
    }
    c->ix.n_ent = n_entries;
    publish_index(c);
    HIP_TRY(fx.seq_counts.ensure(n_entries));
    HIP_TRY(dev_zero_now(fx.seq_counts.get(), n_entries * 8));
    HIP_TRY(fx.ctr.ensure((size_t)kCtrStripes * 8));
    HIP_TRY(dev_zero_now(fx.ctr.get(), (size_t)kCtrStripes * 8 * 8));
    HIP_TRY(fx.small.ensure(16));
    HIP_TRY(fx.ctl.ensure(kMaxPhases + 2));
    HIP_TRY(hipHostMalloc(&c->h_ctl, sizeof(PhaseCtl) * (kMaxPhases + 2)));
    HIP_TRY(bk::make_wait_event(&c->ev_ctl));
    HIP_TRY(bk::make_wait_event(&c->ev_wait));
    HIP_TRY(fx.ctr_aux.ensure(4));
    HIP_TRY(hipHostMalloc(&c->h_small, 2 * sizeof(PhaseCtl)));
    int rc = derive_cfg(c);
    clk0.lap("entry table, small buffers");
    return rc;
}

int finish_ctx(bk_ctx *c, const bk_entry_info *entries, uint32_t n_entries)
{
    int rc = c->entries_set ? BK_OK : setup_entries(c, entries, n_entries);
    if (rc) return rc;
    c->entries_set = true;
    StageClock clk;
    if (!c->tables_built) {
        rc = build_tables(c);
        clk.lap("k-mer table, second-level keys, inverse suffix array");
        if (rc) return rc;
    }
    if (!c->tgt2_built) {
        rc = build_tgt2(c);
        clk.lap("2-bit target");
    }
    return rc;
}

int new_ctx(bk_ctx **out, int device_id, const bk_align_params *p, bk_ctx **pc)
{
    if (!out || !p) return BK_ERR_PARAMS;
    *out = nullptr;
    int ndev = 0;
    if (hipGetDeviceCount(&ndev) != hipSuccess || ndev <= 0) return BK_ERR_NODEVICE;
    if (device_id < 0 || device_id >= ndev) return BK_ERR_PARAMS;
    HIP_TRY(hipSetDevice(device_id));
    bk_ctx *c = new bk_ctx();
    bk::live_contexts()++;
    c->device = device_id;
    c->params = *p;
    c->cfg.heavy_thresh = 64;
    c->debug = env::debug_phases();
    if (c->params.max_ml == 0) c->params.max_ml = 1;
    if (hipStreamCreate(&c->stream) != hipSuccess) { bk::live_contexts()--; delete c; return BK_ERR_INTERNAL; }
    *pc = c;
    return BK_OK;
}

int adopt_device_image(bk_ctx *c, const uint8_t *d_seq, uint64_t n, const uint8_t *d_sa, int el)
{
    c->el_size = (uint32_t)el;
    c->ix.n = n;
    uint64_t nwords = ((n + 15) / 16 + (kMaxReadLenAbs / 16) + 4 + 3) & ~3ULL;
    ImageBufs &im = c->image;
    HIP_TRY(im.tgt4.ensure(nwords));
    launch_pack_target(d_seq, n, im.tgt4.get(), nwords, c->stream);
    HIP_TRY(hipGetLastError());
    c->n_tgt4_words = nwords;
    c->sort_shift = 0;
    while ((n >> c->sort_shift) >= (1ULL << 32)) c->sort_shift++;
    if (d_sa == nullptr) {
        if (el != 4 || !im.sa_lo.get()) return BK_ERR_INTERNAL;
    } else {
        HIP_TRY(im.sa_lo.ensure(n));
        if (el == 5) {
            HIP_TRY(im.sa_hi.ensure(n));
            launch_split_sa5(d_sa, n, im.sa_lo.get(), im.sa_hi.get(), c->stream);
            HIP_TRY(hipGetLastError());
        } else
            HIP_TRY(hipMemcpyAsync(im.sa_lo.get(), d_sa, n * 4, hipMemcpyDeviceToDevice, c->stream));
    }
    HIP_TRY(hipStreamSynchronize(c->stream));
    publish_index(c);
    return BK_OK;
}


}

void bk::drop_swin(bk_ctx *c)
{
    c->image.swin.reset();
    c->image.swmap.reset();
    publish_index(c);
    c->swin_bytes = 0;
}

void bk::release_swin(bk_ctx *c)
{
    if (!c || !c->image.swin.get()) return;
    (void)hipSetDevice(c->device);
    if (c->stream) (void)hipStreamSynchronize(c->stream);
    (void)hipDeviceSynchronize();
    drop_swin(c);
    c->swin_denied = true;
    fprintf(stderr, "biokanga_amd: window array released to make room\n");
}


namespace bk {
struct SwinBuild {
    int w[kSwLevels] = {}, n_levels = 0;
    int words = 3;
    uint32_t max_run = 0, cap_blocks = 0;
    uint32_t min_run = kSwMinRun;
    int mode = 0;
    uint64_t done = 0;
    uint64_t range_cap = 0;
    DevBuf<unsigned long long> d_brk[kSwLevels];
    DevBuf<uint32_t> d_flags, d_incl, d_map, d_used;
    DevBuf<uint8_t> d_tmp, d_ent;
    size_t tmp_bytes = 0;
    DevBuf<unsigned long long> d_starts;
    std::thread ent_alloc;
    std::atomic<int> ent_state{0};
    DevBuf<uint8_t> ent_mem;
    uint64_t filled = 0;
    double t0 = 0;
    void drop_scratch() { for (auto &q : d_brk) q.reset(); d_flags.reset(); d_incl.reset(); d_tmp.reset(); d_starts.reset(); }
    ~SwinBuild() { if (ent_alloc.joinable()) ent_alloc.join(); }
    void take_ahead() { if (ent_state == 2) { if (ent_alloc.joinable()) ent_alloc.join(); if (ent_mem.get()) d_ent = std::move(ent_mem); } }
    void brk_ptrs(unsigned long long **out) { for (int l = 0; l < kSwLevels; l++) out[l] = d_brk[l].get(); }
    void alloc_ahead(int device, uint64_t bytes)
    {
        ent_state = 1;
        ent_alloc = std::thread([this, device, bytes]() {
            if (hipSetDevice(device) != hipSuccess || ent_mem.ensure(bytes) != hipSuccess) { (void)hipGetLastError(); ent_state = 3; return; }
            ent_state = 2;
        });
    }
};


int swin_core_lens_k(const bk_ctx *c, uint32_t maxlen, int k, int *w, double *wave_share = nullptr)
{
    const ReadPlan p = make_plan((int)std::max<uint32_t>(maxlen, 1), c->cfg);
    int n = 0;
    for (int ph = p.n_phases - 1; ph >= 0; ph--) {
        int mm, cl, cd;
        phase_params(p, c->cfg, ph, mm, cl, cd);
        cl = std::min(std::max(cl, k), 120);
        if (n == 0 || cl > w[n - 1]) {
            if (n == kSwLevels) break;
            w[n] = cl;
            if (wave_share) wave_share[n] = 0.0;
            n++;
        }
        if (wave_share && ph < kMaxPhases) wave_share[n - 1] += c->hist_wave[ph];
    }
    return n;
}
int swin_core_lens(const bk_ctx *c, uint32_t maxlen, int *w, bool skip_auto = false)
{
    double share[kSwLevels];
    int n = swin_core_lens_k(c, maxlen, c->ix.k, w, share);
    int skip = c->swin_skip_short > 0 ? std::min(c->swin_skip_short, n - 1) : 0;
    if (!skip && skip_auto && c->hist_valid) {
        double total = 0.0, acc = 0.0;
        for (int i = 0; i < n; i++) total += share[i];
        while (skip < n - 1 && acc + share[skip] < 0.05 * total) acc += share[skip++];
    }
    if (skip) { for (int i = skip; i < n; i++) w[i - skip] = w[i]; n -= skip; }
    return n;
}


int swin_begin(bk_ctx *c, SwinBuild &sb, const int *w, int n_levels, int words, uint64_t budget, uint64_t range_cap, int mode, hipStream_t s)
{
    const uint64_t n = c->ix.n;
    const uint64_t n_blocks = (n + (1u << kSwBlkShift) - 1) >> kSwBlkShift;
    sb.words = words;
    const uint64_t block_bytes = (uint64_t)(16 * words) << kSwBlkShift;
    sb.t0 = StageClock::now();
    sb.n_levels = n_levels;
    for (int l = 0; l < n_levels; l++) sb.w[l] = w[l];
    sb.max_run = c->cfg.max_iter > 0 ? (uint32_t)c->cfg.max_iter + 256u : 1u << 20;
    sb.cap_blocks = (uint32_t)std::min<uint64_t>(n_blocks, budget / block_bytes);
    if (sb.cap_blocks == 0) return 1;
    sb.range_cap = std::min<uint64_t>(range_cap, n) + 64;
    const uint64_t brk_words = (sb.range_cap >> 6) + 4, blocks = (sb.range_cap >> kSwBlkShift) + 2;
    for (int l = 0; l < n_levels; l++) SW_TRY(sb.d_brk[l].ensure(brk_words));
    SW_TRY(sb.d_flags.ensure(blocks));
    SW_TRY(sb.d_incl.ensure(blocks));
    SW_TRY(sb.d_map.ensure(n_blocks));
    SW_TRY(sb.d_used.ensure(1));
    SW_TRY(hipMemsetAsync(sb.d_used.get(), 0, 4, s));
    SW_TRY(bk::prim::inclusive_sum(nullptr, sb.tmp_bytes, sb.d_flags.get(), sb.d_incl.get(), (size_t)blocks, s));
    SW_TRY(sb.d_tmp.ensure(sb.tmp_bytes + 256));
    sb.mode = mode;
    if (mode == 1) {
        if (sb.ent_state == 0) SW_TRY(sb.d_ent.ensure((uint64_t)sb.cap_blocks * block_bytes));
        SW_TRY(sb.d_starts.ensure((n >> 6) + 4));
        SW_TRY(clear_dev(sb.d_starts.get(), ((n >> 6) + 4) * 8, s));
    }
    return BK_OK;
}

int swin_range(bk_ctx *c, SwinBuild &sb, const DevIndex &ix, uint64_t upto, hipStream_t s)
{
    const uint64_t n = ix.n;
    unsigned long long *brk[kSwLevels];
    sb.brk_ptrs(brk);
    while (sb.done < n) {
        uint64_t e = upto >= n ? n : (upto & ~63ULL);
        if (e > sb.done && e - sb.done > sb.range_cap - 64) e = (sb.done + sb.range_cap - 64) & ~63ULL;
        if (e <= sb.done) break;
        const uint64_t a = sb.done, len = e - a;
        const uint64_t n_words = (len >> 6) + 2, n_blocks = (len + (1u << kSwBlkShift) - 1) >> kSwBlkShift;
        launch_swin_breaks(ix, sb.w, sb.n_levels, brk, a, e, n_words, sb.d_starts.get(), s);
        for (int l = 0; l < sb.n_levels; l++) launch_swin_cover(brk[l], len, sb.max_run, sb.min_run, sb.d_flags.get(), n_blocks, l == 0, s);
        SW_TRY(hipGetLastError());
        size_t tb = sb.tmp_bytes;
        SW_TRY(bk::prim::inclusive_sum(sb.d_tmp.get(), tb, sb.d_flags.get(), sb.d_incl.get(), (size_t)n_blocks, s));
        launch_swin_map(sb.d_flags.get(), sb.d_incl.get(), n_blocks, sb.cap_blocks, sb.d_used.get(), sb.d_map.get() + (a >> kSwBlkShift), s);
        if (sb.d_ent.get() == nullptr) sb.take_ahead();
        if (sb.d_ent.get() == nullptr && sb.ent_state == 1) { sb.done = e; continue; }
        if (sb.d_ent.get() == nullptr && sb.ent_state == 3) return BK_ERR_MEM;
        if (sb.d_ent.get() == nullptr) {
            if (a != 0 || e != n) return BK_ERR_INTERNAL;
            uint32_t used = 0;
            SW_TRY(hipMemcpyAsync(&used, sb.d_used.get(), 4, hipMemcpyDeviceToHost, s));
            SW_TRY(hipStreamSynchronize(s));
            if (used == 0) { sb.done = e; return BK_OK; }
            sb.cap_blocks = used;
            SW_TRY(sb.d_ent.ensure((uint64_t)used * ((uint64_t)(16 * sb.words) << kSwBlkShift)));
        }
        launch_swin_fill(ix, sb.d_map.get(), sb.d_ent.get(), sb.words, sb.filled, e, s);
        SW_TRY(hipGetLastError());
        sb.filled = e;
        sb.done = e;
    }
    return BK_OK;
}

int swin_fit(bk_ctx *c, SwinBuild &sb, const DevIndex &ix, hipStream_t s)
{
    static const uint32_t ladder[] = {kSwMinRun, 96, 128, 160, 192, 224, 256, 288, 320, 352, 384, 416, 448, 480, 512, 576, 640, 704, 768, 832, 896, 960, 1024, 1088, 1152, 1216, 1280,
                                      1344, 1408, 1472, 1536, 1664, 1792, 1920, 2048, 2304, 2560, 3072, 4096, 6144, 8192};
    constexpr int NL = (int)(sizeof(ladder) / sizeof(ladder[0]));
    const uint64_t n = ix.n;
    DevBuf<unsigned long long> d_cnt;
    unsigned long long *brk[kSwLevels];
    sb.brk_ptrs(brk);
    SW_TRY(d_cnt.ensure(NL));
    SW_TRY(hipMemsetAsync(d_cnt.get(), 0, NL * 8, s));
    for (uint64_t a = 0; a < n;) {
        uint64_t e = std::min<uint64_t>(n, (a + sb.range_cap - 64) & ~63ULL);
        const uint64_t len = e - a, n_words = (len >> 6) + 2, n_blocks = (len + (1u << kSwBlkShift) - 1) >> kSwBlkShift;
        launch_swin_breaks(ix, sb.w, sb.n_levels, brk, a, e, n_words, nullptr, s);
        for (int q = 0; q < NL; q++) {
            if (ladder[q] > sb.max_run) break;
            for (int l = 0; l < sb.n_levels; l++) launch_swin_cover(brk[l], len, sb.max_run, ladder[q], sb.d_flags.get(), n_blocks, l == 0, s);
            launch_count_nonzero(sb.d_flags.get(), n_blocks, d_cnt.get() + q, s);
        }
        SW_TRY(hipGetLastError());
        a = e;
    }
    unsigned long long cnt[NL] = {};
    SW_TRY(hipMemcpyAsync(cnt, d_cnt.get(), NL * 8, hipMemcpyDeviceToHost, s));
    SW_TRY(hipStreamSynchronize(s));
    d_cnt.reset();
    int pick = 0;
    while (pick + 1 < NL && ladder[pick + 1] <= sb.max_run && cnt[pick] > sb.cap_blocks) pick++;
    sb.min_run = ladder[pick];
    const uint64_t blocks = std::min<uint64_t>(cnt[pick], sb.cap_blocks);
    if (blocks == 0) return 1;
    sb.cap_blocks = (uint32_t)blocks;
    SW_TRY(sb.d_ent.ensure(blocks * ((uint64_t)(16 * sb.words) << kSwBlkShift)));
    StageClock clk;
    if (clk.on) fprintf(stderr, "biokanga_amd: window array: runs of %u and more suffixes covered whole (the rule at 65: %.1f %% of the suffix array, this: %.1f %%, room for %.1f %%)\n", sb.min_run,
                        100.0 * (double)cnt[0] * 32.0 / (double)n, 100.0 * (double)cnt[pick] * 32.0 / (double)n, 100.0 * (double)blocks * 32.0 / (double)n);
    return BK_OK;
}

int swin_end(bk_ctx *c, SwinBuild &sb, hipStream_t s)
{
    if (sb.ent_alloc.joinable()) sb.ent_alloc.join();
    if (sb.ent_state == 3) return BK_ERR_MEM;
    if (sb.d_ent.get() == nullptr) sb.take_ahead();
    if (sb.d_ent.get() != nullptr && sb.filled < sb.done) {
        launch_swin_fill(c->ix, sb.d_map.get(), sb.d_ent.get(), sb.words, sb.filled, sb.done, s);
        sb.filled = sb.done;
    }
    uint32_t used = 0;
    SW_TRY(hipMemcpyAsync(&used, sb.d_used.get(), 4, hipMemcpyDeviceToHost, s));
    SW_TRY(hipStreamSynchronize(s));
    sb.drop_scratch();
    if (sb.done < c->ix.n) return BK_ERR_INTERNAL;
    if (used == 0) return 1;
    const uint64_t block_bytes = (uint64_t)(16 * sb.words) << kSwBlkShift;
    const uint64_t n_blocks = (c->ix.n + (1u << kSwBlkShift) - 1) >> kSwBlkShift;
    c->image.swin = std::move(sb.d_ent);
    c->image.swmap = std::move(sb.d_map);
    c->swin_w = sb.w[0] | (sb.w[sb.n_levels - 1] << 8) | (sb.n_levels << 16) | (sb.words << 24);
    c->ix.sw_words = sb.words;
    c->swin_bytes = (uint64_t)std::max(used, sb.cap_blocks) * block_bytes + n_blocks * 4;
    c->swin_covered = (double)used / (double)n_blocks;
    publish_index(c);
    c->swin_setup_s = StageClock::now() - sb.t0;
    return BK_OK;
}

uint64_t swin_budget_for(const bk_ctx *c, uint64_t free_b, uint64_t reserve, int words)
{
    const bool ranged = c->ix.n >= (1ULL << 32);
    const uint64_t span = ranged ? (1ULL << 31) : c->ix.n;
    const uint64_t work = ((span >> kSwBlkShift) + 1) * 8 + ((c->ix.n >> kSwBlkShift) + 1) * 4 + (span >> 3) * (kSwLevels + 1) + (64ULL << 20);
    if (free_b < reserve + work + (1ULL << 30)) return 0;
    uint64_t budget = std::min<uint64_t>(c->ix.n * 16 * (uint64_t)words / 3, ranged ? (free_b - reserve - work) / 16 * 15 : (free_b - reserve - work) / 2);
    if (c->swin_budget) budget = std::min<uint64_t>(budget, c->swin_budget);
    return budget;
}

int maybe_build_swin(bk_ctx *c, uint32_t maxlen, uint32_t nreads, hipStream_t s)
{
    ImageBufs &im = c->image;
    const bool wide = im.sa_hi.get() != nullptr || c->ix.n >= (1ULL << 32);
    if (!c->use_swin || c->swin_denied || !c->ix.tgt2 || (!wide && !c->ix.isa) || !c->ix.k2 || !c->use_wave) return BK_OK;
    if (wide && c->use_swin != 2) return BK_OK;
    const bool full = c->use_swin == 3;
    if (wide && !c->hist_valid && c->swin_skip_short == 0) return BK_OK;
    int w[kSwLevels];
    const int n_levels = swin_core_lens(c, maxlen, w, wide);
    const int words = maxlen <= 128 ? 3 : 5;
    const int w_key = w[0] | (w[n_levels - 1] << 8) | (n_levels << 16) | (words << 24);
    if (wide && im.swin.get() && c->ix.sw_words == words) return BK_OK;
    if (im.swin.get()) {
        if (full == (im.swmap.get() == nullptr) && (full ? c->ix.sw_words == words : (c->swin_w == w_key || (c->swin_rebuilt && c->ix.sw_words == words)))) return BK_OK;
        c->swin_rebuilt = true;
        HIP_TRY(hipStreamSynchronize(s));
        drop_swin(c);
    }
    if (c->use_swin == 1 && maxlen > 256) return BK_OK;
    size_t free_b = 0, total_b = 0;
    HIP_TRY(hipMemGetInfo(&free_b, &total_b));
    const uint64_t want = (uint64_t)std::min(nreads, c->chunk_reads) * scratch_bytes_per_read(words_per_read(maxlen), rd2w_for(maxlen), iv_cores_for(c, maxlen));
    const uint64_t have = (uint64_t)c->cap_reads * scratch_bytes_per_read(c->cap_wpr, c->cap_rd2w, c->cap_iv_cores);
    const uint64_t missing = want > have ? want - have : 0;
    const uint64_t reserve = missing * 4 / 3 + (6ULL << 30);
    StageClock clk;
    const double t0 = StageClock::now();
    if (full) {
        const uint64_t need = ((c->ix.n + 31) & ~31ULL) * 16 * (uint64_t)words;
        if ((uint64_t)free_b < need + reserve) { c->swin_denied = true; return BK_OK; }
        if (im.swin.ensure(need) != hipSuccess) { (void)hipGetLastError(); c->swin_denied = true; return BK_OK; }
        launch_build_swin(c->ix, im.swin.get(), words, s);
        HIP_TRY(hipGetLastError());
        HIP_TRY(hipStreamSynchronize(s));
        c->swin_bytes = need;
        c->swin_covered = 1.0;
        c->ix.sw_words = words;
    } else {
        const uint64_t budget = swin_budget_for(c, (uint64_t)free_b, reserve, words);
        if (!budget) { c->swin_denied = true; return BK_OK; }
        SwinBuild sb;
        const bool ranged = c->ix.n >= (1ULL << 32);
        int rb = swin_begin(c, sb, w, n_levels, words, budget, ranged ? (1ULL << 31) : c->ix.n, ranged ? 2 : 0, s);
        if (!rb && ranged) rb = swin_fit(c, sb, c->ix, s);
        if (!rb) rb = swin_range(c, sb, c->ix, c->ix.n, s);
        if (!rb) rb = swin_end(c, sb, s);
        if (rb == BK_ERR_INTERNAL) return rb;
        if (rb) { c->swin_denied = true; return BK_OK; }
    }
    publish_index(c);
    if (full) c->swin_setup_s = StageClock::now() - t0;
    if (clk.on) fprintf(stderr, "biokanga_amd: window array for %.1f %% of the suffix array (runs sharing %d .. %d bases, %d levels), entries of %d bytes, %.2f GB\n", 100.0 * c->swin_covered, w[0], w[n_levels - 1], n_levels, 16 * words, c->swin_bytes / 1e9);
    clk.lap("suffix-ordered windows");
    return BK_OK;
}


}

using namespace bk;

extern "C" {

uint32_t bk_image_policy(uint64_t reads_per_device)
{
    return reads_per_device >= BK_POLICY_MIN_READS ? BK_CTX_WINDOW_ARRAY_EAGER : BK_CTX_GROW_IMAGE;
}

int bk_ctx_create(bk_ctx **out, const char *sfx_path, int device_id, const bk_align_params *p)
{
    return bk_ctx_create_ex(out, sfx_path, device_id, p, 0);
}

int bk_ctx_create_ex(bk_ctx **out, const char *sfx_path, int device_id, const bk_align_params *p, uint32_t flags)
{
    if (!sfx_path) return BK_ERR_PARAMS;
    bk_ctx *c = nullptr;
    StageClock clk;
    int rc = new_ctx(out, device_id, p, &c);
    if (rc) return rc;
    clk.lap("HIP runtime + device + stream");
    if (flags & BK_CTX_LEAN_IMAGE) { c->use_ktab2 = 0; c->use_k3 = 0; }
    if (flags & BK_CTX_NO_DEEP_KEYS) c->use_k3 = 0;
    if (flags & BK_CTX_GROW_IMAGE) {
        c->use_ktab2 = 0; c->use_k3 = 0; c->grow_enabled = true;
        if (const unsigned long long v = env::grow_after_reads()) { c->grow_after = v; c->grow_wait = true; }
    }
    SfxFile f;
    std::string err;
    rc = sfx_open(sfx_path, f, &err);
    clk.lap("sfx_open");
    if (rc) {
        fprintf(stderr, "biokanga_amd: %s\n", err.c_str());
        bk_ctx_destroy(c);
        return rc;
    }
    c->dataset = f.dataset;
    const bool eager_swin = (flags & BK_CTX_WINDOW_ARRAY_EAGER) && f.el_size == 4 && f.concat_len < (1ULL << 32) && c->use_swin && c->use_swin != 3;
    SwinBuild sb;
    uint64_t swin_ahead = 0;
    if (eager_swin) {
        size_t free_b = 0, total_b = 0;
        if (hipMemGetInfo(&free_b, &total_b) == hipSuccess && free_b > f.concat_len * 24 + (16ULL << 30)) {
            swin_ahead = std::min<uint64_t>(f.concat_len * 10, total_b / 4);
            if (c->swin_budget) swin_ahead = std::min<uint64_t>(swin_ahead, c->swin_budget);
        } else
            (void)hipGetLastError();
    }
    std::vector<bk_entry_info> ents(f.entries.size());
    for (size_t i = 0; i < ents.size(); i++) {
        ents[i].entry_id = f.entries[i].entry_id;
        ents[i].seq_len = f.entries[i].seq_len;
        ents[i].start_ofs = f.entries[i].start_ofs;
        ents[i].end_ofs = f.entries[i].end_ofs;
        memcpy(ents[i].name, f.entries[i].name, 81);
    }
    DevBuf<uint8_t> d_seq, d_sa;
    const bool sa_in_place = f.el_size == 4;
    if (d_seq.ensure(f.concat_len + 16) != hipSuccess ||
        (sa_in_place ? c->image.sa_lo.ensure(f.concat_len) : d_sa.ensure(f.concat_len * f.el_size)) != hipSuccess) {
        bk_ctx_destroy(c); return BK_ERR_MEM;
    }
    clk.lap("device allocations");
    const int fd = ::open(sfx_path, O_RDONLY);
    if (fd < 0) { bk_ctx_destroy(c); return BK_ERR_OPNFILE; }
    const uint64_t seq_ofs = (uint64_t)(f.seq - (const uint8_t *)f.map_base), sa_ofs = (uint64_t)(f.sa - (const uint8_t *)f.map_base);
    bool sent = upload_file(d_seq.get(), fd, seq_ofs, f.concat_len, device_id) == BK_OK;
    clk.lap("upload bases");
    if (sent && sa_in_place) {
        rc = adopt_device_image(c, d_seq.get(), f.concat_len, nullptr, 4);
        d_seq.reset();
        TablePlan tp;
        if (!rc) rc = tables_begin(c, tp);
        const uint64_t n = f.concat_len;
        uint64_t n_slices = std::max<uint64_t>(1, std::min<uint64_t>(16, n >> 26));
        if (const unsigned long long ts = env::table_slices()) n_slices = std::max<uint64_t>(1, std::min<uint64_t>(ts, n));
        bool swin_sliced = false;
        if (!rc && eager_swin && swin_ahead && tp.ktab && tp.k2 && tp.isa && !c->ktab64 && c->use_wave && c->use_tgt2) {
            rc = setup_entries(c, ents.data(), (uint32_t)ents.size());
            if (!rc) { c->entries_set = true; rc = build_tgt2(c); }
            if (!rc) {
                c->tgt2_built = true;
                clk.lap("entry table, 2-bit target");
                int w[kSwLevels];
                const int n_levels = swin_core_lens_k(c, 100, tp.k, w);
                sb.ent_state = 1;
                swin_sliced = swin_begin(c, sb, w, n_levels, 3, swin_ahead, n / n_slices + 128, 1, c->stream) == BK_OK;
                if (!swin_sliced) { (void)hipGetLastError(); sb.ent_state = 0; }
                else sb.alloc_ahead(device_id, swin_ahead);
            }
        }
        for (uint64_t k = 0; k < n_slices && !rc && sent; k++) {
            const uint64_t i0 = (n * k / n_slices) & ~63ULL, i1 = k + 1 == n_slices ? n : (n * (k + 1) / n_slices) & ~63ULL;
            if (i1 <= i0) continue;
            sent = upload_file(c->image.sa_lo.get() + i0, fd, sa_ofs + i0 * 4, (i1 - i0) * 4, device_id) == BK_OK;
            if (sent) rc = tables_range(c, tp, i0, i1, swin_sliced ? sb.d_starts.get() : nullptr);
            if (sent && !rc && swin_sliced) {
                DevIndex ix = c->ix;
                ix.k = tp.k;
                ix.k2 = c->image.k2.get();
                if (swin_range(c, sb, ix, i1, c->stream) != BK_OK) { (void)hipGetLastError(); swin_sliced = false; }
            }
        }
        clk.lap("upload suffix array, tables enqueued behind its slices");
        if (!rc && sent) rc = tables_end(c, tp);
        clk.lap("tables finished");
        if (!rc && sent && swin_sliced && c->ix.k2 != nullptr) {
            const int re = swin_end(c, sb, c->stream);
            if (re == BK_ERR_INTERNAL) rc = re;
            clk.lap("window array finished");
            if (clk.on && c->image.swin.get()) fprintf(stderr, "biokanga_amd: window array for %.1f %% of the suffix array, %.2f GB, made behind the upload\n", 100.0 * c->swin_covered, c->swin_bytes / 1e9);
        }
    } else if (sent) {
        sent = upload_file(d_sa.get(), fd, sa_ofs, f.concat_len * f.el_size, device_id) == BK_OK;
        clk.lap("upload suffix array");
        if (sent) rc = adopt_device_image(c, d_seq.get(), f.concat_len, d_sa.get(), (int)f.el_size);
        clk.lap("pack target, adopt");
    }
    ::close(fd);
    d_seq.reset(); d_sa.reset();
    if (!sent) { bk_ctx_destroy(c); return BK_ERR_INTERNAL; }
    if (rc) { bk_ctx_destroy(c); return rc; }
    rc = finish_ctx(c, ents.data(), (uint32_t)ents.size());
    if (rc) { bk_ctx_destroy(c); return rc; }
    clk.lap("(rest of bk_ctx_create)");
    if (eager_swin) {
        rc = maybe_build_swin(c, 100, c->chunk_reads, c->stream);
        if (rc) { bk_ctx_destroy(c); return rc; }
    }
    *out = c;
    return BK_OK;
}

int bk_ctx_create_from_device(bk_ctx **out, const void *d_seq, uint64_t concat_len, const void *d_sa, int sfx_el_size,
                              const bk_entry_info *entries, uint32_t n_entries, int device_id, const bk_align_params *p)
{
    if (!d_seq || !d_sa || !entries || !n_entries || !concat_len || (sfx_el_size != 4 && sfx_el_size != 5)) return BK_ERR_PARAMS;
    bk_ctx *c = nullptr;
    int rc = new_ctx(out, device_id, p, &c);
    if (rc) return rc;
    c->dataset = "device";
    rc = adopt_device_image(c, (const uint8_t *)d_seq, concat_len, (const uint8_t *)d_sa, sfx_el_size);
    if (!rc) rc = finish_ctx(c, entries, n_entries);
    if (rc) { bk_ctx_destroy(c); return rc; }
    *out = c;
    return BK_OK;
}

int bk_ctx_clone(bk_ctx **out, const bk_ctx *src, int device_id)
{
    if (!src) return BK_ERR_PARAMS;
    bk_ctx *c = nullptr;
    int rc = new_ctx(out, device_id, &src->params, &c);
    if (rc) return rc;
    StageClock clk;
    c->dataset = src->dataset;
    c->el_size = src->el_size;
    c->n_tgt4_words = src->n_tgt4_words;
    c->sort_shift = src->sort_shift;
    c->ktab64 = src->ktab64;
    c->ktab_wide = src->ktab_wide;
    c->ktab_is2 = src->ktab_is2;
    c->use_ktab2 = src->use_ktab2;
    c->grow_elem = src->grow_elem;
    c->use_k3 = src->use_k3;
    c->sort_lists = src->sort_lists; c->sort_lists_set = src->sort_lists_set;
    c->grow_enabled = src->grow_enabled && src->grow_state.load() != 4; c->grow_after = src->grow_after; c->grow_wait = src->grow_wait;
    c->use_ktab = src->use_ktab; c->k_req = src->k_req; c->use_k2 = src->use_k2; c->use_isa = src->use_isa; c->use_wave = src->use_wave; c->use_tgt2 = src->use_tgt2;
    c->ix.n = src->ix.n;
    c->ix.k = src->ix.k;
    c->ix.flag_shift = src->ix.flag_shift;
    c->ix.nflag_bytes = src->ix.nflag_bytes;
    bool ok = true;
    auto dup = [&](auto &dst, const auto &from) {
        if (!ok || !from.get()) return;
        if (dst.ensure(from.cap()) != hipSuccess) { ok = false; rc = BK_ERR_MEM; return; }
        const size_t bytes = from.cap() * sizeof(*from.get());
        hipError_t e = c->device == src->device ? hipMemcpyAsync(dst.get(), from.get(), bytes, hipMemcpyDeviceToDevice, c->stream)
                                                : hipMemcpyPeerAsync(dst.get(), c->device, from.get(), src->device, bytes, c->stream);
        if (e != hipSuccess) { ok = false; rc = BK_ERR_INTERNAL; }
    };
    ImageBufs &im = c->image;
    const ImageBufs &sim = src->image;
    dup(im.tgt4, sim.tgt4);
    dup(im.sa_lo, sim.sa_lo);
    dup(im.sa_hi, sim.sa_hi);
    dup(im.ktab, sim.ktab);
    dup(im.ktab_hi, sim.ktab_hi);
    dup(im.k2, sim.k2);
    for (int i = 0; i < kMoreKeys; i++) dup(im.kx[i], sim.kx[i]);
    dup(im.isa, sim.isa);
    dup(im.tgt2, sim.tgt2);
    dup(im.tgt2s, sim.tgt2s);
    dup(im.nflag, sim.nflag);
    c->use_swin = src->use_swin;
    if (ok && hipStreamSynchronize(c->stream) != hipSuccess) { ok = false; rc = BK_ERR_INTERNAL; }
    if (!ok) { bk_ctx_destroy(c); return rc; }
    publish_index(c);
    clk.lap("index image copied from the first device");
    rc = setup_entries(c, src->entries.data(), (uint32_t)src->entries.size());
    if (rc) { bk_ctx_destroy(c); return rc; }
    *out = c;
    return BK_OK;
}

void bk_ctx_destroy(bk_ctx *c)
{
    if (!c) return;
    (void)hipSetDevice(c->device);
    grow_drop(c);
    if (c->stream) (void)hipStreamSynchronize(c->stream);
    c->release_image_buffers();
    c->release_batch_buffers();
    if (c->h_small) (void)hipHostFree(c->h_small);
    for (void *&t : c->sam_text) if (t) { (void)hipHostFree(t); t = nullptr; }
    if (c->h_ctl) (void)hipHostFree(c->h_ctl);
    if (c->h_plan) (void)hipHostFree(c->h_plan);
    if (c->ev_plan) (void)hipEventDestroy(c->ev_plan);
    if (c->ev_ctl) (void)hipEventDestroy(c->ev_ctl);
    if (c->ev_wait) (void)hipEventDestroy(c->ev_wait);
    for (hipEvent_t e : c->ev_pool) (void)hipEventDestroy(e);
    if (c->stream) (void)hipStreamDestroy(c->stream);
    bk::live_contexts()--;
    delete c;
}


}
```

biokanga_amd/csrc/bk_index.hip:

```cpp
#include <algorithm>

#include "bk_dev_k2.h"
#include "bk_dev_window.h"

namespace bk {


__global__ void k_pack_target(const uint8_t *__restrict__ seq, uint64_t n, uint64_t *__restrict__ tgt4, uint64_t nwords)
{
    uint64_t w = (uint64_t)blockIdx.x * blockDim.x + threadIdx.x;
    uint64_t stride = (uint64_t)gridDim.x * blockDim.x;
    for (; w < nwords; w += stride) {
        uint64_t base = w << 4;
        uint64_t v = 0;
        if (base + 16 <= n) {
            const uint4 q = *reinterpret_cast<const uint4 *>(seq + base);
            uint32_t d[4] = {q.x, q.y, q.z, q.w};
#pragma unroll
            for (int j = 0; j < 4; j++)
#pragma unroll
                for (int k = 0; k < 4; k++) v = (v << 4) | ((d[j] >> (8 * k)) & 0x0f);
        } else {
            for (int k = 0; k < 16; k++) {
                uint64_t p = base + k;
                uint64_t nb = p < n ? (uint64_t)(seq[p] & 0x0f) : 7ULL;
                v = (v << 4) | nb;
            }
        }
        tgt4[w] = v;
    }
}

__global__ void k_pack_target2(const uint64_t *__restrict__ tgt4, uint64_t nwords4, uint64_t *__restrict__ tgt2,
                               unsigned int *__restrict__ nflag32, int flag_shift)
{
    uint64_t nblocks = nwords4 / 4;
    for (uint64_t blk = (uint64_t)blockIdx.x * blockDim.x + threadIdx.x; blk < nblocks; blk += (uint64_t)gridDim.x * blockDim.x) {
        uint64_t a = tgt4[4 * blk], b = tgt4[4 * blk + 1], c = tgt4[4 * blk + 2], d = tgt4[4 * blk + 3];
        tgt2[2 * blk] = ((uint64_t)squeeze2(a) << 32) | squeeze2(b);
        tgt2[2 * blk + 1] = ((uint64_t)squeeze2(c) << 32) | squeeze2(d);
        if ((a | b | c | d) & 0x4444444444444444ULL) {
            uint64_t g = blk >> (flag_shift - 6);
            atomicOr(&nflag32[g >> 5], 1u << (g & 31));
        }
    }
}

__global__ void k_split_sa5(const uint8_t *__restrict__ sa5, uint64_t n, uint32_t *__restrict__ lo, uint8_t *__restrict__ hi)
{
    uint64_t i = (uint64_t)blockIdx.x * blockDim.x + threadIdx.x;
    uint64_t stride = (uint64_t)gridDim.x * blockDim.x;
    for (; i < n; i += stride) {
        const uint8_t *p = sa5 + i * 5;
        lo[i] = (uint32_t)p[0] | ((uint32_t)p[1] << 8) | ((uint32_t)p[2] << 16) | ((uint32_t)p[3] << 24);
        hi[i] = p[4];
    }
}

__device__ __forceinline__ uint64_t suffix_bucket(const uint64_t *__restrict__ tgt, uint64_t pos, int k)
{
    uint64_t w = nib16(tgt, pos);
    uint64_t bad = w & 0x4444444444444444ULL;
    if (bad) {
        int j = __clzll(bad) >> 2;
        if (j < 16) w |= (~0ULL >> (4 * j)) & 0x3333333333333333ULL;
    }
    return (uint64_t)(squeeze2(w) >> (32 - 2 * k));
}

template <bool WIDE, typename TabT>
__global__ void k_build_ktab(DevIndex ix, TabT *__restrict__ tab, int k, uint64_t i0, uint64_t i1, unsigned long long *__restrict__ starts, int tab_stride)
{
    uint64_t n = ix.n;
    uint64_t ncodes = 1ULL << (2 * k);
    uint64_t i = i0 + (uint64_t)blockIdx.x * blockDim.x + threadIdx.x;
    uint64_t stride = (uint64_t)gridDim.x * blockDim.x;
    for (; i < i1; i += stride) {
        uint64_t cur = i < n ? suffix_bucket(ix.tgt4, sa_get<WIDE>(ix, i), k) : ncodes;
        uint64_t from = i > 0 ? suffix_bucket(ix.tgt4, sa_get<WIDE>(ix, i - 1), k) + 1 : 0;
        for (uint64_t c = from; c <= cur; c++) tab[c * (uint64_t)tab_stride] = (TabT)i;
        if (starts != nullptr) {
            const unsigned long long m = __ballot(from != cur + 1);
            if ((i & 63) == 0 && m) atomicOr(&starts[i >> 6], m);
        }
    }
}

template <bool WIDE>
__global__ void k_build_k2(DevIndex ix, uint32_t *__restrict__ k2, uint32_t *__restrict__ k3, uint32_t *__restrict__ k4, uint64_t i0, uint64_t i1)
{
    for (uint64_t i = i0 + (uint64_t)blockIdx.x * blockDim.x + threadIdx.x; i < i1; i += (uint64_t)gridDim.x * blockDim.x) {
        const uint64_t pos = sa_get<WIDE>(ix, i);
        const uint32_t key = k2_make(ix.tgt4, pos, ix.k);
        if (k2 != nullptr) k2[i] = key;
        if (k3 != nullptr) {
            const uint32_t key3 = kx_make(ix.tgt4, pos, ix.k + kK2Bases, key);
            k3[i] = key3;
            if (k4 != nullptr) k4[i] = kx_make(ix.tgt4, pos, ix.k + 2 * kK2Bases, key3);
        }
    }
}

__global__ void k_build_k2_levels(uint32_t *__restrict__ k2, uint64_t n)
{
    const uint64_t w0 = n, w1 = k2s_start(n, kK2Levels + 1);
    for (uint64_t w = w0 + (uint64_t)blockIdx.x * blockDim.x + threadIdx.x; w < w1; w += (uint64_t)gridDim.x * blockDim.x) {
        uint32_t v = kK2Above;
        uint64_t start = k2s_start(n, 1);
        for (int j = 1; j <= kK2Levels && w >= start; j++) {
            const uint64_t cnt = k2s_count(n, j);
            if (w - start < cnt) {
                const uint64_t src = ((w - start + 1) << (4 * j)) - 1;
                v = k2[src < n ? src : n - 1];
                break;
            }
            start += k2s_pad(cnt) + 16;
        }
        k2[w] = v;
    }
}

template <bool WIDE>
__global__ void k_check_k2(DevIndex ix, const uint32_t *__restrict__ k2, unsigned long long *__restrict__ bad, uint64_t i0, uint64_t i1)
{
    for (uint64_t i = i0 + (uint64_t)blockIdx.x * blockDim.x + threadIdx.x; i < i1 && i + 1 < ix.n; i += (uint64_t)gridDim.x * blockDim.x) {
        const uint32_t a = k2[i], c = k2[i + 1];
        if (a < c) continue;
        if (a == c) {
            if ((a & 3u) != 0u || ix.kx[0] == nullptr) continue;
            const uint32_t a3 = ix.kx[0][i], c3 = ix.kx[0][i + 1];
            if (a3 < c3) continue;
            if (a3 == c3 && ((a3 & 3u) != 0u || ix.kx[1] == nullptr || ix.kx[1][i] <= ix.kx[1][i + 1])) continue;
        }
        if (suffix_bucket(ix.tgt4, sa_get<WIDE>(ix, i), ix.k) == suffix_bucket(ix.tgt4, sa_get<WIDE>(ix, i + 1), ix.k))
            atomicAdd(bad + (a == c ? 1 : 0), 1ULL);
    }
}

template <int E>
__device__ __forceinline__ void swin_entry(const DevIndex &ix, uint64_t i, uint4 *__restrict__ swin, uint64_t idx)
{
    const int64_t base0 = (int64_t)(ix.sa_hi != nullptr ? sa_get<true>(ix, i) : (uint64_t)ix.sa_lo[i]) - SwGeo<E>::pre;
    uint64_t wd[2 * E];
#pragma unroll
    for (int k = 0; k < 2 * E; k++) {
        const int64_t pos = base0 + 32 * k;
        uint64_t v;
        if (pos >= 0) {
            const uint64_t wi = (uint64_t)pos >> 5;
            const unsigned sh = (unsigned)(pos & 31) << 1;
            const uint64_t a = ix.tgt2[wi], bq = ix.tgt2[wi + 1];
            v = (a << sh) | ((bq >> 1) >> (63 - sh));
        } else if (pos > -32)
            v = ix.tgt2[0] >> (unsigned)(2 * (-pos));
        else
            v = 0;
        wd[k] = v;
    }
#pragma unroll
    for (int q = 0; q < E; q++)
        swin[sw_word_at<E>(idx, q)] = make_uint4((uint32_t)wd[2 * q], (uint32_t)(wd[2 * q] >> 32), (uint32_t)wd[2 * q + 1], (uint32_t)(wd[2 * q + 1] >> 32));
}

template <int E>
__global__ void __launch_bounds__(256) k_build_swin(DevIndex ix, uint4 *__restrict__ swin)
{
    for (uint64_t i = (uint64_t)blockIdx.x * blockDim.x + threadIdx.x; i < ix.n; i += (uint64_t)gridDim.x * blockDim.x)
        swin_entry<E>(ix, i, swin, i);
}

void launch_build_swin(const DevIndex &ix, void *swin, int words, hipStream_t s)
{
    if (words == 5) hipLaunchKernelGGL(k_build_swin<5>, dim3(65536), dim3(256), 0, s, ix, reinterpret_cast<uint4 *>(swin));
    else hipLaunchKernelGGL(k_build_swin<3>, dim3(65536), dim3(256), 0, s, ix, reinterpret_cast<uint4 *>(swin));
}


struct SwinLevels {
    int n;
    int w[kSwLevels];
    unsigned long long *brk[kSwLevels];
};

__device__ __forceinline__ uint64_t tgt2_bases32(const uint64_t *__restrict__ tgt2, uint64_t pos)
{
    const uint64_t wi = pos >> 5;
    const unsigned sh = (unsigned)(pos & 31) << 1;
    const uint64_t a = tgt2[wi], bq = tgt2[wi + 1];
    return (a << sh) | ((bq >> 1) >> (63 - sh));
}

__global__ void __launch_bounds__(256) k_swin_breaks(DevIndex ix, SwinLevels lv, uint64_t a, uint64_t e, uint64_t n_words, const unsigned long long *__restrict__ starts)
{
    const int lane = threadIdx.x & 63;
    const uint64_t n = ix.n;
    const int k = ix.k, deep_from = k + kK2Bases;
    const int w_max = lv.w[lv.n - 1];
    for (uint64_t w = ((uint64_t)blockIdx.x * blockDim.x + threadIdx.x) >> 6; w < n_words; w += ((uint64_t)gridDim.x * blockDim.x) >> 6) {
        const uint64_t i = a + (w << 6) + lane;
        int shared = (i == a || i == e) ? 0 : 1 << 20;
        if (starts != nullptr && i < e && ((starts[i >> 6] >> (i & 63)) & 1)) shared = 0;
        if (shared && i > a && i < e) {
            const uint32_t a = ix.k2[i - 1], c = ix.k2[i];
            if (a == kK2Above || c == kK2Above) shared = 0;
            else {
                const uint32_t x = (a ^ c) & ~3u;
                if (x) shared = k + (__clz((int)x) >> 1);
                else if ((a | c) & 3u) shared = deep_from - 1;
                else if (w_max > deep_from) {
                    const bool wide_el = ix.sa_hi != nullptr;
                    const uint64_t pa = (wide_el ? sa_get<true>(ix, i - 1) : (uint64_t)ix.sa_lo[i - 1]) + (uint64_t)deep_from, pb = (wide_el ? sa_get<true>(ix, i) : (uint64_t)ix.sa_lo[i]) + (uint64_t)deep_from;
                    const int span = w_max - deep_from;
                    shared = deep_from;
                    if (pa + (uint64_t)span < n && pb + (uint64_t)span < n && !window_flagged(ix, pa, span) && !window_flagged(ix, pb, span)) {
                        for (int q = 0; q < span; q += 32) {
                            const uint64_t d = tgt2_bases32(ix.tgt2, pa + (uint64_t)q) ^ tgt2_bases32(ix.tgt2, pb + (uint64_t)q);
                            if (d) { shared += __clzll((long long)d) >> 1; break; }
                            shared += 32;
                        }
                    }
                }
            }
        }
        for (int l = 0; l < lv.n; l++) {
            const unsigned long long m = __ballot(i <= e && shared < lv.w[l]);
            if (lane == 0) lv.brk[l][w] = m;
        }
    }
}

__global__ void __launch_bounds__(256) k_swin_bucket_starts(DevIndex ix, uint64_t n_codes, SwinLevels lv, uint64_t a, uint64_t e)
{
    const int lane = threadIdx.x & 63;
    const uint64_t span = (n_codes + 63) & ~63ULL;
    for (uint64_t c = (uint64_t)blockIdx.x * blockDim.x + threadIdx.x; c < span; c += (uint64_t)gridDim.x * blockDim.x) {
        uint64_t lo = ~0ULL, hi = ~0ULL;
        if (c < n_codes) {
            if (ix.ktab2) { lo = ix.ktab2[c].x; hi = ix.ktab2[c + 1].x; }
            else { lo = ktab_get(ix, c); hi = ktab_get(ix, c + 1); }
        }
        const bool in = c < n_codes && hi != lo && lo >= a && lo < e;
        const uint32_t w = in ? (uint32_t)((lo - a) >> 5) : 0xFFFFFFFFu;
        uint32_t bits = in ? 1u << (uint32_t)(lo & 31) : 0u;
        for (int off = 1; off < 64; off <<= 1) {
            const uint32_t ob = __shfl_up(bits, off), ow = __shfl_up(w, off);
            if (lane >= off && ow == w) bits |= ob;
        }
        const uint32_t nw = __shfl_down(w, 1);
        if (bits && (lane == 63 || nw != w))
            for (int l = 0; l < lv.n; l++) atomicOr(reinterpret_cast<uint32_t *>(lv.brk[l]) + w, bits);
    }
}

__device__ __forceinline__ uint64_t swin_next_break(const unsigned long long *__restrict__ brk, uint64_t p, uint64_t limit)
{
    const uint64_t last = p + limit;
    uint64_t q = p + 1;
    while (q <= last) {
        unsigned long long w = brk[q >> 6] >> (q & 63);
        if (w) { const uint64_t r = q + (uint64_t)(__ffsll(w) - 1); return r <= last ? r : 0; }
        q = (q | 63) + 1;
    }
    return 0;
}

__device__ __forceinline__ uint64_t swin_prev_break(const unsigned long long *__restrict__ brk, uint64_t p, uint64_t limit)
{
    const uint64_t first = p > limit ? p - limit : 0;
    uint64_t q = p;
    for (;;) {
        unsigned long long w = brk[q >> 6] << (63 - (q & 63));
        if (w) { const uint64_t r = q - (uint64_t)__clzll((long long)w); return r >= first ? r : ~0ULL; }
        if ((q >> 6) == 0 || (q & ~63ULL) <= first) return ~0ULL;
        q = (q & ~63ULL) - 1;
    }
}

__global__ void __launch_bounds__(256) k_swin_cover(const unsigned long long *__restrict__ brk, uint64_t n, uint32_t max_run, uint32_t min_run, uint32_t *__restrict__ flags, uint64_t n_blocks, int first_level)
{
    constexpr uint64_t B = 1ULL << kSwBlkShift;
    for (uint64_t blk = (uint64_t)blockIdx.x * blockDim.x + threadIdx.x; blk < n_blocks; blk += (uint64_t)gridDim.x * blockDim.x) {
        const uint64_t b0 = blk << kSwBlkShift;
        bool cov = !first_level && flags[blk] != 0;
        if (cov) continue;
        const uint64_t s0 = swin_prev_break(brk, b0, max_run);
        if (s0 != ~0ULL) {
            const uint64_t e0 = swin_next_break(brk, b0, s0 + max_run - b0);
            if (e0) cov = e0 - s0 >= min_run;
            else cov = b0 - s0 < kSwHead;
        }
        if (!cov) {
            const unsigned long long w = (brk[b0 >> 6] >> (b0 & 63)) & ((1ULL << B) - 1) & ~1ULL;
            if (w) {
                const uint64_t s = b0 + (uint64_t)(63 - __clzll((long long)w));
                if (s < n) cov = swin_next_break(brk, s, min_run - 1) == 0;
            }
        }
        flags[blk] = cov ? 1u : 0u;
    }
}

__global__ void __launch_bounds__(256) k_swin_map(const uint32_t *__restrict__ flags, const uint32_t *__restrict__ incl, uint64_t n_blocks, uint32_t cap_blocks,
                                                  const uint32_t *__restrict__ used, uint32_t *__restrict__ map)
{
    const uint32_t base = *used;
    for (uint64_t blk = (uint64_t)blockIdx.x * blockDim.x + threadIdx.x; blk < n_blocks; blk += (uint64_t)gridDim.x * blockDim.x) {
        const uint64_t slot = (uint64_t)base + incl[blk] - 1;
        map[blk] = (flags[blk] && slot < cap_blocks) ? (uint32_t)slot : kSwNone;
    }
}

__global__ void k_swin_advance(const uint32_t *__restrict__ incl_last, uint32_t cap_blocks, uint32_t *__restrict__ used)
{
    const uint64_t u = (uint64_t)*used + *incl_last;
    *used = u < cap_blocks ? (uint32_t)u : cap_blocks;
}

template <int E>
__global__ void __launch_bounds__(256) k_swin_fill(DevIndex ix, const uint32_t *__restrict__ map, uint4 *__restrict__ swin, uint64_t a, uint64_t e)
{
    for (uint64_t i = a + (uint64_t)blockIdx.x * blockDim.x + threadIdx.x; i < e; i += (uint64_t)gridDim.x * blockDim.x) {
        const uint32_t s = map[i >> kSwBlkShift];
        if (s == kSwNone) continue;
        swin_entry<E>(ix, i, swin, ((uint64_t)s << kSwBlkShift) + (i & ((1u << kSwBlkShift) - 1)));
    }
}

void launch_swin_breaks(const DevIndex &ix, const int *w, int n_levels, unsigned long long *const *brk, uint64_t a, uint64_t e, uint64_t n_words,
                        const unsigned long long *starts, hipStream_t s)
{
    SwinLevels lv{};
    lv.n = n_levels;
    for (int l = 0; l < n_levels; l++) { lv.w[l] = w[l]; lv.brk[l] = brk[l]; }
    const unsigned blocks = (unsigned)std::min<uint64_t>((n_words + 3) / 4, 32768);
    hipLaunchKernelGGL(k_swin_breaks, dim3(blocks), dim3(256), 0, s, ix, lv, a, e, n_words, starts);
    if (starts == nullptr) {
        const uint64_t n_codes = 1ULL << (2 * ix.k);
        hipLaunchKernelGGL(k_swin_bucket_starts, dim3((unsigned)std::min<uint64_t>((n_codes + 255) / 256, 65536)), dim3(256), 0, s, ix, n_codes, lv, a, e);
    }
}

void launch_swin_cover(const unsigned long long *brk, uint64_t n, uint32_t max_run, uint32_t min_run, uint32_t *flags, uint64_t n_blocks, int first_level, hipStream_t s)
{
    const unsigned blocks = (unsigned)std::min<uint64_t>((n_blocks + 255) / 256, 262144);
    hipLaunchKernelGGL(k_swin_cover, dim3(blocks), dim3(256), 0, s, brk, n, max_run, min_run, flags, n_blocks, first_level);
}

void launch_swin_map(const uint32_t *flags, const uint32_t *incl, uint64_t n_blocks, uint32_t cap_blocks, uint32_t *used, uint32_t *map, hipStream_t s)
{
    if (!n_blocks) return;
    const unsigned blocks = (unsigned)std::min<uint64_t>((n_blocks + 255) / 256, 262144);
    hipLaunchKernelGGL(k_swin_map, dim3(blocks), dim3(256), 0, s, flags, incl, n_blocks, cap_blocks, used, map);
    hipLaunchKernelGGL(k_swin_advance, dim3(1), dim3(1), 0, s, incl + (n_blocks - 1), cap_blocks, used);
}

__global__ void __launch_bounds__(256) k_count_nonzero(const uint32_t *__restrict__ flags, uint64_t n, unsigned long long *__restrict__ count)
{
    unsigned long long mine = 0;
    for (uint64_t i = (uint64_t)blockIdx.x * blockDim.x + threadIdx.x; i < ((n + 63) & ~63ULL); i += (uint64_t)gridDim.x * blockDim.x)
        mine += (unsigned long long)__popcll(__ballot(i < n && flags[i] != 0));
    if ((threadIdx.x & 63) == 0 && mine) atomicAdd(count, mine);
}

void launch_count_nonzero(const uint32_t *flags, uint64_t n, unsigned long long *count, hipStream_t s)
{
    if (!n) return;
    const unsigned blocks = (unsigned)std::min<uint64_t>((n + 255) / 256, 16384);
    hipLaunchKernelGGL(k_count_nonzero, dim3(blocks), dim3(256), 0, s, flags, n, count);
}

void launch_swin_fill(const DevIndex &ix, const uint32_t *map, void *swin, int words, uint64_t a, uint64_t e, hipStream_t s)
{
    if (e <= a) return;
    const unsigned blocks = (unsigned)std::min<uint64_t>((e - a + 255) / 256, 65536);
    if (words == 5) hipLaunchKernelGGL(k_swin_fill<5>, dim3(blocks), dim3(256), 0, s, ix, map, reinterpret_cast<uint4 *>(swin), a, e);
    else hipLaunchKernelGGL(k_swin_fill<3>, dim3(blocks), dim3(256), 0, s, ix, map, reinterpret_cast<uint4 *>(swin), a, e);
}

__global__ void k_build_isa(const uint32_t *__restrict__ sa, uint64_t i0, uint64_t i1, uint32_t *__restrict__ isa)
{
    uint64_t i = i0 + (uint64_t)blockIdx.x * blockDim.x + threadIdx.x;
    uint64_t stride = (uint64_t)gridDim.x * blockDim.x;
    for (; i < i1; i += stride) isa[sa[i]] = (uint32_t)i;
}

__global__ void k_fill_u64(unsigned long long *__restrict__ p, uint64_t n, unsigned long long v)
{
    uint64_t i = (uint64_t)blockIdx.x * blockDim.x + threadIdx.x;
    uint64_t stride = (uint64_t)gridDim.x * blockDim.x;
    for (; i < n; i += stride) p[i] = v;
}


void launch_pack_target(const uint8_t *seq, uint64_t n, uint64_t *tgt4, uint64_t nwords, hipStream_t s)
{
    uint64_t blocks = (nwords + 255) / 256;
    if (blocks > 65536) blocks = 65536;
    hipLaunchKernelGGL(k_pack_target, dim3((unsigned)blocks), dim3(256), 0, s, seq, n, tgt4, nwords);
}

void launch_split_sa5(const uint8_t *sa5, uint64_t n, uint32_t *lo, uint8_t *hi, hipStream_t s)
{
    uint64_t blocks = (n + 255) / 256;
    if (blocks > 65536) blocks = 65536;
    hipLaunchKernelGGL(k_split_sa5, dim3((unsigned)blocks), dim3(256), 0, s, sa5, n, lo, hi);
}

void launch_build_ktab(const DevIndex &ix, void *tab, int k, bool tab64, hipStream_t s, uint64_t i0, uint64_t i1, unsigned long long *starts, bool pairs)
{
    const int stride = (pairs && !tab64) ? 2 : 1;
    if (i0 & 63) starts = nullptr;
    if (i1 == 0) i1 = ix.n + 1;
    if (i1 <= i0) return;
    uint64_t blocks = (i1 - i0 + 255) / 256;
    if (blocks > 262144) blocks = 262144;
    bool wide = ix.sa_hi != nullptr;
    if (wide) {
        if (tab64) hipLaunchKernelGGL((k_build_ktab<true, uint64_t>), dim3((unsigned)blocks), dim3(256), 0, s, ix, (uint64_t *)tab, k, i0, i1, starts, stride);
        else hipLaunchKernelGGL((k_build_ktab<true, uint32_t>), dim3((unsigned)blocks), dim3(256), 0, s, ix, (uint32_t *)tab, k, i0, i1, starts, stride);
    } else {
        if (tab64) hipLaunchKernelGGL((k_build_ktab<false, uint64_t>), dim3((unsigned)blocks), dim3(256), 0, s, ix, (uint64_t *)tab, k, i0, i1, starts, stride);
        else hipLaunchKernelGGL((k_build_ktab<false, uint32_t>), dim3((unsigned)blocks), dim3(256), 0, s, ix, (uint32_t *)tab, k, i0, i1, starts, stride);
    }
}

void launch_fill_u64(unsigned long long *p, uint64_t n, unsigned long long v, hipStream_t s)
{
    uint64_t blocks = (n + 255) / 256;
    if (blocks > 65536) blocks = 65536;
    if (!blocks) return;
    hipLaunchKernelGGL(k_fill_u64, dim3((unsigned)blocks), dim3(256), 0, s, p, n, v);
}

__global__ void __launch_bounds__(256) k_pack_ktab64(const uint64_t *__restrict__ tab, uint64_t n_entries, uint32_t *__restrict__ off, uint64_t *__restrict__ hi,
                                                     uint32_t *__restrict__ overflow)
{
    for (uint64_t c = (uint64_t)blockIdx.x * blockDim.x + threadIdx.x; c < n_entries; c += (uint64_t)gridDim.x * blockDim.x) {
        const uint64_t base = tab[c & ~0xFFFFULL], v = tab[c] - base;
        if (v >> 32) atomicOr(overflow, 1u);
        off[c] = (uint32_t)v;
        if ((c & 0xFFFFULL) == 0) hi[c >> 16] = base;
    }
}

void launch_pack_ktab64(const uint64_t *tab, uint64_t n_entries, uint32_t *off, uint64_t *hi, uint32_t *overflow, hipStream_t s)
{
    hipLaunchKernelGGL(k_pack_ktab64, dim3(65536), dim3(256), 0, s, tab, n_entries, off, hi, overflow);
}

void launch_pack_target2(const uint64_t *tgt4, uint64_t nwords4, uint64_t *tgt2, unsigned int *nflag32, int flag_shift, hipStream_t s)
{
    uint64_t blocks = (nwords4 / 4 + 255) / 256;
    if (blocks > 65536) blocks = 65536;
    hipLaunchKernelGGL(k_pack_target2, dim3((unsigned)blocks), dim3(256), 0, s, tgt4, nwords4, tgt2, nflag32, flag_shift);
}

__global__ void __launch_bounds__(256) k_make_ktab2(const uint32_t *__restrict__ tab, const uint32_t *__restrict__ k2, uint64_t n_entries, uint64_t n,
                                                    uint2 *__restrict__ out, const uint32_t *__restrict__ sa_elem)
{
    for (uint64_t c = (uint64_t)blockIdx.x * blockDim.x + threadIdx.x; c < n_entries; c += (uint64_t)gridDim.x * blockDim.x) {
        const uint32_t lo = tab[c];
        const uint64_t hi = c + 1 < n_entries ? (uint64_t)tab[c + 1] : (uint64_t)lo;
        uint32_t y = 0u;
        if (hi == (uint64_t)lo + 1) y = sa_elem != nullptr ? sa_elem[lo] : k2[lo];
        else if (hi > (uint64_t)lo + kTab2BitmapMax) y = 0xFFFFFFFFu;
        else
            for (uint64_t i = lo; i < hi; i++) {
                const uint32_t key = k2[i];
                if (key != kK2Above) y |= 1u << (key >> 27);
            }
        out[c] = make_uint2(lo, y);
    }
}

__global__ void __launch_bounds__(256) k_fill_ktab2_y(uint2 *__restrict__ tab, const uint32_t *__restrict__ k2, uint64_t n_entries, const uint32_t *__restrict__ sa_elem)
{
    for (uint64_t c = (uint64_t)blockIdx.x * blockDim.x + threadIdx.x; c < n_entries; c += (uint64_t)gridDim.x * blockDim.x) {
        const uint32_t lo = tab[c].x;
        const uint64_t hi = c + 1 < n_entries ? (uint64_t)tab[c + 1].x : (uint64_t)lo;
        uint32_t y = 0u;
        if (k2 == nullptr) y = 0xFFFFFFFFu;
        else if (hi == (uint64_t)lo + 1) y = sa_elem != nullptr ? sa_elem[lo] : k2[lo];
        else if (hi > (uint64_t)lo + kTab2BitmapMax) y = 0xFFFFFFFFu;
        else
            for (uint64_t i = lo; i < hi; i++) {
                const uint32_t key = k2[i];
                if (key != kK2Above) y |= 1u << (key >> 27);
            }
        tab[c].y = y;
    }
}

void launch_fill_ktab2_y(void *tab2, const uint32_t *k2, uint64_t n_entries, hipStream_t s, const uint32_t *sa_elem)
{
    hipLaunchKernelGGL(k_fill_ktab2_y, dim3(65536), dim3(256), 0, s, reinterpret_cast<uint2 *>(tab2), k2, n_entries, sa_elem);
}

void launch_make_ktab2(const uint32_t *tab, const uint32_t *k2, uint64_t n_entries, uint64_t n, void *out, hipStream_t s, const uint32_t *sa_elem)
{
    hipLaunchKernelGGL(k_make_ktab2, dim3(65536), dim3(256), 0, s, tab, k2, n_entries, n, reinterpret_cast<uint2 *>(out), sa_elem);
}

void launch_build_k2(const DevIndex &ix, uint32_t *k2, uint32_t *k3, uint32_t *k4, unsigned long long *bad, hipStream_t s, uint64_t i0, uint64_t i1, bool write_k2)
{
    if (i1 == 0) i1 = ix.n;
    if (i1 <= i0) return;
    uint64_t blocks = (i1 - i0 + 255) / 256;
    if (blocks > 262144) blocks = 262144;
    DevIndex t = ix;
    t.k2 = k2;
    t.kx[0] = k3;
    t.kx[1] = k3 ? k4 : nullptr;
    const uint64_t c0 = i0 ? i0 - 1 : 0, c1 = i1 == ix.n ? i1 : i1 - 1;
    if (ix.sa_hi) {
        hipLaunchKernelGGL(k_build_k2<true>, dim3((unsigned)blocks), dim3(256), 0, s, t, write_k2 ? k2 : nullptr, k3, t.kx[1] ? k4 : nullptr, i0, i1);
        hipLaunchKernelGGL(k_check_k2<true>, dim3((unsigned)blocks), dim3(256), 0, s, t, k2, bad, c0, c1);
    } else {
        hipLaunchKernelGGL(k_build_k2<false>, dim3((unsigned)blocks), dim3(256), 0, s, t, write_k2 ? k2 : nullptr, k3, t.kx[1] ? k4 : nullptr, i0, i1);
        hipLaunchKernelGGL(k_check_k2<false>, dim3((unsigned)blocks), dim3(256), 0, s, t, k2, bad, c0, c1);
    }
}

void launch_build_k2_levels(uint32_t *k2, uint64_t n, hipStream_t s)
{
    const uint64_t words = k2s_start(n, kK2Levels + 1) - n;
    uint64_t blocks = (words + 255) / 256;
    if (blocks > 262144) blocks = 262144;
    hipLaunchKernelGGL(k_build_k2_levels, dim3((unsigned)blocks), dim3(256), 0, s, k2, n);
}

void launch_build_isa(const uint32_t *sa, uint64_t n, uint32_t *isa, hipStream_t s, uint64_t i0, uint64_t i1)
{
    if (i1 == 0) i1 = n;
    if (i1 <= i0) return;
    uint64_t blocks = (i1 - i0 + 255) / 256;
    if (blocks > 262144) blocks = 262144;
    hipLaunchKernelGGL(k_build_isa, dim3((unsigned)blocks), dim3(256), 0, s, sa, i0, i1, isa);
}

}
```

biokanga_amd/csrc/bk_search.hip:

```cpp
#include <algorithm>

#include "bk_dev_k2.h"
#include "bk_dev_prof.h"
#include "bk_plan_table.h"

namespace bk {



template <bool WIDE>
__global__ void __launch_bounds__(256) k_search(DevIndex ix, DevAlignCfg cfg, DevBatch b, const uint32_t *__restrict__ act,
                                                uint32_t n_act, int phase, int cmax, int nstr, int lazy)
{
    uint64_t tid = (uint64_t)blockIdx.x * blockDim.x + threadIdx.x;
    uint32_t per_read = (uint32_t)(nstr * cmax);
    uint64_t a = tid / per_read;
    if (a >= n_act) return;
    uint32_t rem = (uint32_t)(tid - a * per_read);
    int si = (int)(rem / (uint32_t)cmax), c = (int)(rem % (uint32_t)cmax);
    uint32_t r = act[a];
    const uint32_t meta = b.rmeta[r];
    int len = (int)(meta & kReadLenMask);
    ReadPlan p = make_plan(len, cfg);
    int mm, cl, cd;
    phase_params(p, cfg, phase, mm, cl, cd);
    int cur = cd, o = 0, n = 0, my_ofs = -1;
    while (n < p.max_slides && o <= len - cl && cur > cl / 3) {
        if (o + cl + cur > len) cur = len - (o + cl);
        if (n == c) my_ofs = o;
        n++;
        o += cur;
    }
    if (my_ofs < 0 || n > kMaxCoresFast) return;
    int strand = cfg.align_strand == 2 ? 1 : si;
    const RdRow rdw = read_row(b, r, strand, (meta & kReadHasN) != 0);
    uint64_t first, count;
    uint64_t slot = iv_slot(b, (uint32_t)a, strand, c);
    if (lazy && ix.k > 0 && cl >= ix.k) {
        uint64_t p0 = rdw.nib16(my_ofs) & top_mask(cl);
        uint64_t lo, hi;
        core_range(ix, p0, cl, lo, hi);
        if (hi - lo <= kLazyBucket && !(lo == 0 && hi == ix.n)) {
            iv_put(b, slot, lo, (uint32_t)(hi - lo) | (hi > lo ? kLazyFlag : 0u));
            return;
        }
    }
    search_core<WIDE>(ix, rdw, my_ofs, cl, ~0ULL >> 1, first, count);
    iv_put(b, slot, first, count > 0x7FFFFFFFULL ? 0x7FFFFFFFu : (uint32_t)count);
}


template <int ILP>
__global__ void __launch_bounds__(256) k_search_a_ilp(DevIndex ix, DevAlignCfg cfg, DevBatch b, const uint32_t *__restrict__ act,
                                                      const uint32_t *__restrict__ p_n_act, int phase, int cmax, int nstr, int lazy,
                                                      StripeSet out, ItemGeo ig)
{
    __shared__ uint32_t s_cnt, s_base;
    extern __shared__ uint2 s_plan[];
    plan_stage(s_plan, b, phase, threadIdx.x, 256);
#if defined(BK_PROF) && BK_PROF == 2
    PROF_BEGIN;
#endif
    const uint32_t n_act = *p_n_act;
    const uint32_t per_read = (uint32_t)(nstr * cmax);
    const uint64_t total = (uint64_t)n_act * per_read;
    constexpr uint64_t stride = 256;
    const int k = ix.k;
    ItemCursor cur = item_cursor((uint64_t)blockIdx.x * (256 * ILP), per_read);
  for (uint64_t tile0 = (uint64_t)blockIdx.x * (256 * ILP); tile0 < total; tile0 += (uint64_t)gridDim.x * (256 * ILP), item_advance(cur, ig)) {
    if (threadIdx.x == 0) s_cnt = 0;
    __syncthreads();
    bool on[ILP], push[ILP], have_code[ILP];
    uint64_t slot[ILP], p0[ILP], first[ILP], lo[ILP], hi[ILP];
    uint32_t nval[ILP], q2raw[ILP];
    int cl[ILP];
    constexpr uint32_t kNoIv32 = 0xFFFFFFFFu;
    uint32_t cix[ILP];
    uint2 cv[ILP];
    bool cached[ILP];
    uint32_t key0[ILP];
#pragma unroll
    for (int u = 0; u < ILP; u++) {
        on[u] = false; push[u] = false; have_code[u] = false; slot[u] = 0; p0[u] = 0; q2raw[u] = 0; first[u] = 0; nval[u] = 0; cl[u] = 1; lo[u] = hi[u] = 0;
        cix[u] = kNoIv32; cv[u] = make_uint2(0, kNoIv32); cached[u] = false;
        uint64_t a;
        int si, c;
        item_decode(cur, threadIdx.x + (uint32_t)u * (uint32_t)stride, ig, a, si, c);
        if (a < n_act) {
            const uint32_t r = act[a];
            const uint32_t meta = b.rmeta[r];
            const int len = (int)(meta & kReadLenMask);
            const int strand_c = cfg.align_strand == 2 ? 1 : si;
            if (b.iv32 != nullptr && c == 0 && phase > 0) cv[u] = b.iv32[(uint32_t)strand_c * b.n_reads + r];
            const PlanGeo g = plan_lookup(s_plan, b.plan_n, len);
            const int cd = g.cd, nc = g.nc;
            cl[u] = g.cl;
            if (c < nc && nc <= kMaxCoresFast) {
                on[u] = true;
                if (b.iv32 != nullptr && c == 0 && cl[u] >= k + kK2Bases) {
                    cix[u] = (uint32_t)strand_c * b.n_reads + r;
                    cached[u] = phase > 0 && cv[u].y != kNoIv32 && (cv[u].y < (1u << kKindShift) || (lazy && (cv[u].y & kIvFlags) == kIvFlags));
                }
                const int my_ofs = c * cd < len - cl[u] ? c * cd : len - cl[u];
                const int strand = cfg.align_strand == 2 ? 1 : si;
                slot[u] = iv_slot(b, (uint32_t)a, strand, c);
                if (b.rd2 != nullptr && !(meta & kReadHasN)) {
                    const uint64_t *row = b.rd2 + ((uint64_t)r * 2 + strand) * (b.nw / 2);
                    const uint64_t x = bits64_2(row, my_ofs);
                    p0[u] = spread2to4((uint32_t)(x >> 32)) & top_mask(cl[u]);
                    q2raw[u] = k == 16 ? (uint32_t)x : (uint32_t)(bits64_2(row, my_ofs + k) >> 32);
                } else {
                    const uint64_t *rdw = b.rd4 + ((uint64_t)r * 2 + strand) * b.wpr;
                    p0[u] = nib16(rdw, my_ofs) & top_mask(cl[u]);
                    const uint64_t q4 = nib16(rdw, my_ofs + k);
                    q2raw[u] = squeeze2(q4);
                    const int rem2 = cl[u] - k;
                    if (rem2 > 0 && (q4 & 0x4444444444444444ULL & top_mask(rem2 < kK2Bases ? rem2 : kK2Bases))) p0[u] |= 0x4000000000000000ULL;
                }
            }
        }
    }
    PROFS(0);
#pragma unroll
    for (int u = 0; u < ILP; u++) {
        nval[u] = kKindFull << kKindShift;
        push[u] = on[u];
        have_code[u] = on[u] && !cached[u] && cl[u] >= k && !(p0[u] & 0x4444444444444444ULL & top_mask(k));
        key0[u] = kK2Above;
        if (have_code[u]) {
            const uint64_t code = (uint64_t)(squeeze2(p0[u]) >> (32 - 2 * k));
            if (ix.ktab2 != nullptr) {
                const uint2 e0 = ix.ktab2[code], e1 = ix.ktab2[code + 1];
                lo[u] = e0.x; hi[u] = e1.x; key0[u] = e0.y;
            } else {
                ktab_get_pair(ix, code, lo[u], hi[u]);
            }
        }
    }
    PROFS(1);
    uint32_t key[ILP][kInlineBucket];
    bool absent[ILP];
    bool carry[ILP];
#pragma unroll
    for (int u = 0; u < ILP; u++) {
        const uint64_t size = hi[u] - lo[u];
        const uint32_t m = k2_mask(cl[u] - k);
        absent[u] = have_code[u] && ix.ktab2 != nullptr && size >= 2 && ktab2_absent(key0[u], m, q2raw[u] & m);
        carry[u] = have_code[u] && lazy && ix.ktab2 != nullptr && ix.ktab2_elem && size == 1;
        const bool key_in_entry = size == 1 && ix.ktab2 != nullptr && !ix.ktab2_elem;
#pragma unroll
        for (uint32_t j = 0; j < kInlineBucket; j++)
            key[u][j] = (have_code[u] && !absent[u] && !carry[u] && size <= kInlineBucket && j < size) ? (key_in_entry ? key0[u] : ix.k2[lo[u] + j]) : kK2Above;
    }
    PROFS(2);
#pragma unroll
    for (int u = 0; u < ILP; u++) {
        uint2 leave = make_uint2(0, kNoIv32);
        if (cached[u] && (cv[u].y & kElemFlag)) {
            first[u] = cv[u].x;
            nval[u] = cv[u].y;
            push[u] = false;
        } else if (cached[u]) {
            first[u] = cv[u].x;
            const uint32_t cnt = cv[u].y;
            if (cnt == 0 || cl[u] <= k + kK2Bases) { nval[u] = cnt; push[u] = false; }
            else if (lazy && cnt <= kLazyBucket) { nval[u] = cnt | kLazyFlag; push[u] = false; }
            else nval[u] = cnt | (kKindDeep << kKindShift);
        }
        if (carry[u]) {
            first[u] = key0[u];
            nval[u] = 1u | kIvFlags;
            push[u] = false;
            leave = make_uint2(key0[u], 1u | kIvFlags);
        } else if (have_code[u]) {
            const uint64_t size = hi[u] - lo[u];
            if (size == 0 || absent[u]) { first[u] = lo[u]; nval[u] = 0; push[u] = false; leave = make_uint2((uint32_t)lo[u], 0u); }
            else if (size <= kInlineBucket) {
                const uint32_t m = k2_mask(cl[u] - k), q2 = q2raw[u] & m;
                uint32_t lb = 0, ub = 0;
                bool suspect = false;
#pragma unroll
                for (uint32_t j = 0; j < kInlineBucket; j++) {
                    const int cm = k2_cmp(key[u][j], m, q2);
                    lb += cm < 0;
                    ub += cm <= 0;
                    suspect |= cm == 0 && k2_nkind(key[u][j]);
                }
                if (suspect) {
                    first[u] = lo[u];
                    nval[u] = (uint32_t)size | (kKindK2 << kKindShift);
                } else {
                    first[u] = lo[u] + lb;
                    const uint32_t cnt = ub - lb;
                    leave = make_uint2((uint32_t)first[u], cnt);
                    if (cnt == 0 || cl[u] <= k + kK2Bases) { nval[u] = cnt; push[u] = false; }
                    else if (lazy && cnt <= kLazyBucket) { nval[u] = cnt | kLazyFlag; push[u] = false; }
                    else nval[u] = cnt | (kKindDeep << kKindShift);
                }
            } else if (size < (1ULL << kKindShift)) {
                first[u] = lo[u];
                nval[u] = (uint32_t)size | (kKindK2 << kKindShift);
            }
        }
        if (phase == 0 && cix[u] != kNoIv32) b.iv32[cix[u]] = leave;
    }
    PROFS(3);
    const int lane = threadIdx.x & 63;
    uint32_t my_off[ILP];
#pragma unroll
    for (int u = 0; u < ILP; u++) {
        my_off[u] = 0;
        const uint64_t m = __ballot(push[u]);
        if (m) {
            uint32_t w = 0;
            if (lane == 0) w = atomicAdd(&s_cnt, (uint32_t)__popcll(m));
            w = __builtin_amdgcn_readfirstlane(w);
            my_off[u] = w + (uint32_t)__popcll(m & ((1ULL << lane) - 1));
        }
    }
    PROFS(4);
    __syncthreads();
    const uint64_t tile = tile0 / (256 * ILP);
    if (threadIdx.x == 0 && s_cnt) s_base = stripe_reserve_tile(out, 0, s_cnt, tile);
    __syncthreads();
    PROFS(5);
#pragma unroll
    for (int u = 0; u < ILP; u++) {
        if (push[u]) stripe_put_tile(out, 0, s_base + my_off[u], (uint32_t)slot[u], tile);
        if (on[u]) iv_put(b, slot[u], first[u], nval[u]);
    }
    __syncthreads();
  }
#if defined(BK_PROF) && BK_PROF == 2
    PROFS(6);
    PROF_END;
#endif
}

template <bool WIDE>
__global__ void __launch_bounds__(256) k_search_b(DevIndex ix, DevAlignCfg cfg, DevBatch b, int phase, int lazy,
                                                  const uint32_t *__restrict__ list, const uint32_t *__restrict__ sorted, uint32_t n_sorted,
                                                  const uint32_t *__restrict__ p_n_list, SlotGeo sg)
{
    __shared__ uint64_t s_lv[kK2Levels + 1];
    extern __shared__ uint2 s_plan[];
    plan_stage(s_plan, b, phase, threadIdx.x, 256);
    if (threadIdx.x <= (unsigned)kK2Levels) s_lv[threadIdx.x] = threadIdx.x ? k2s_start(ix.n, (int)threadIdx.x) : 0;
    __syncthreads();
    const uint32_t n_list = *p_n_list;
    const uint32_t n_grouped = sorted != nullptr ? (n_list < n_sorted ? n_list : n_sorted) : 0u;
  for (uint32_t i = blockIdx.x * blockDim.x + threadIdx.x; i < n_list; i += gridDim.x * blockDim.x) {
#ifdef BK_DIAG_B
    unsigned long long d_k2 = 0, d_deep = 0, d_sa = 0;
    struct Fin { unsigned long long &a, &b, &c; DevBatch &bb; __device__ ~Fin() { if (a + b) atomicAdd(&bb.ctr[ctr_stripe() + 5], a + b); if (c) atomicAdd(&bb.ctr[ctr_stripe() + 6], c); } } fin{d_k2, d_deep, d_sa, b};
#endif
    const uint32_t slot32 = i < n_grouped ? sorted[i] : list[i];
    const uint64_t slot = slot32;
    uint32_t a;
    int strand, c;
    slot_decode(slot32, sg, a, strand, c);
    const uint32_t r = b.act[a];
    const uint32_t meta = b.rmeta[r];
    const int len = (int)(meta & kReadLenMask);
    const PlanGeo g = plan_lookup(s_plan, b.plan_n, len);
    const int cl = g.cl, cd = g.cd;
    const int my_ofs = c * cd < len - cl ? c * cd : len - cl;
    const RdRow rdw = read_row(b, r, strand, (meta & kReadHasN) != 0);
    uint64_t first;
    uint32_t raw;
    iv_get(b, slot, first, raw);
    const uint32_t kind = raw >> kKindShift;
    uint64_t cnt = raw & ((1u << kKindShift) - 1);
    const int k = ix.k;
    if (kind == kKindFull) {
        search_core<WIDE>(ix, rdw, my_ofs, cl, ~0ULL >> 1, first, cnt);
        iv_put(b, slot, first, cnt > 0x7FFFFFFFULL ? 0x7FFFFFFFu : (uint32_t)cnt);
        continue;
    }
    if (kind == kKindK2) {
        const uint32_t m = k2_mask(cl - k);
        const uint32_t q2 = squeeze2(rdw.nib16(my_ofs + k)) & m;
        uint64_t l1, l2;
        unsigned long long k2_lines = 0;
        k2_bounds(ix.k2, s_lv, first, cnt, m, q2, l1, l2, k2_lines);
#ifdef BK_DIAG_B
        d_k2 += 1 + (k2_lines << 32);
#endif
        {
            const int upto = cl < k + kK2Bases ? cl : k + kK2Bases;
            while (l2 > l1) {
                const uint32_t kv = ix.k2[l2 - 1];
                if (!k2_nkind(kv) || cmp_core_from(rdw, my_ofs, upto, k, ix.tgt4, sa_get<WIDE>(ix, l2 - 1)) == 0) break;
                l2--;
            }
        }
        first = l1;
        cnt = l2 - l1;
        if (!WIDE && b.iv32 != nullptr && phase == 0 && c == 0 && cl >= k + kK2Bases)
            b.iv32[(uint32_t)strand * b.n_reads + r] = make_uint2((uint32_t)first, (uint32_t)cnt);
        if (cnt == 0 || cl <= k + kK2Bases) {
            iv_put(b, slot, first, cnt > 0x7FFFFFFFULL ? 0x7FFFFFFFu : (uint32_t)cnt);
            continue;
        }
    }
    if (lazy && cnt <= kLazyBucket) {
        iv_put(b, slot, first, (uint32_t)cnt | kLazyFlag);
        continue;
    }
    int start = k + kK2Bases;
    bool settled = false;
    for (int lv = 0; lv < kMoreKeys && ix.kx[lv] != nullptr; lv++) {
        const uint32_t *__restrict__ kx = ix.kx[lv];
        const uint64_t p3 = rdw.nib16(my_ofs + start);
        if (p3 & 0x4444444444444444ULL & top_mask(cl - start < kK2Bases ? cl - start : kK2Bases)) break;
        const uint32_t m3 = k2_mask(cl - start);
        const uint32_t q3 = squeeze2(p3) & m3;
        uint64_t l1, l2;
        unsigned long long k3_lines = 0;
        k2_bounds(kx, s_lv, first, cnt, m3, q3, l1, l2, k3_lines);
#ifdef BK_DIAG_B
        d_deep += 1 + (k3_lines << 32);
#endif
        {
            const int upto = cl < start + kK2Bases ? cl : start + kK2Bases;
            while (l2 > l1) {
                const uint32_t kv = kx[l2 - 1];
                if (!k2_nkind(kv) || cmp_core_from(rdw, my_ofs, upto, start, ix.tgt4, sa_get<WIDE>(ix, l2 - 1)) == 0) break;
                l2--;
            }
        }
        first = l1;
        cnt = l2 - l1;
        start += kK2Bases;
        if (cnt == 0 || cl <= start) {
            iv_put(b, slot, first, cnt > 0x7FFFFFFFULL ? 0x7FFFFFFFu : (uint32_t)cnt);
            settled = true;
            break;
        }
        if (lazy && cnt <= kLazyBucket) {
            iv_put(b, slot, first, (uint32_t)cnt | kLazyFlag);
            settled = true;
            break;
        }
    }
    if (settled) continue;
    {
        uint64_t l1 = first, h1 = first + cnt, l2 = first, h2 = first + cnt;
        while (l1 < h1 || l2 < h2) {
            const bool a1 = l1 < h1, a2 = l2 < h2;
            const uint64_t m1 = l1 + ((h1 - l1) >> 1), m2 = l2 + ((h2 - l2) >> 1);
#ifdef BK_DIAG_B
            d_sa += (2ULL << 32) * (a1 + (a2 && m1 != m2));
#endif
            const uint64_t s1 = a1 ? sa_get<WIDE>(ix, m1) : 0, s2 = a2 ? sa_get<WIDE>(ix, m2) : 0;
            const int c1 = a1 ? cmp_core_from(rdw, my_ofs, cl, start, ix.tgt4, s1) : 0;
            const int c2 = a2 ? cmp_core_from(rdw, my_ofs, cl, start, ix.tgt4, s2) : 0;
            if (a1) { if (c1 > 0) l1 = m1 + 1; else h1 = m1; }
            if (a2) { if (c2 >= 0) l2 = m2 + 1; else h2 = m2; }
        }
        first = l1;
#ifdef BK_DIAG_B
        d_sa += 1;
#endif
        cnt = l2 - l1;
    }
    iv_put(b, slot, first, cnt > 0x7FFFFFFFULL ? 0x7FFFFFFFu : (uint32_t)cnt);
  }
}

void launch_search(const DevIndex &ix, const DevAlignCfg &cfg, const DevBatch &b, const uint32_t *act, uint32_t n_act,
                   int phase, int cmax, int nstr, int lazy, hipStream_t s)
{
    uint64_t threads = (uint64_t)n_act * (uint64_t)(cmax * nstr);
    unsigned blocks = (unsigned)((threads + 255) / 256);
    if (ix.sa_hi) hipLaunchKernelGGL(k_search<true>, dim3(blocks), dim3(256), 0, s, ix, cfg, b, act, n_act, phase, cmax, nstr, lazy);
    else hipLaunchKernelGGL(k_search<false>, dim3(blocks), dim3(256), 0, s, ix, cfg, b, act, n_act, phase, cmax, nstr, lazy);
}

__global__ void __launch_bounds__(256) k_keys_search(DevBatch b, const uint32_t *__restrict__ list, const uint32_t *__restrict__ p_n, uint32_t n_sort, int shift,
                                                     uint32_t *__restrict__ keys)
{
    const uint32_t n = *p_n;
    for (uint32_t i = blockIdx.x * blockDim.x + threadIdx.x; i < n_sort; i += gridDim.x * blockDim.x)
        keys[i] = i < n ? (uint32_t)(iv_start(b, list[i]) >> shift) : 0xFFFFFFFFu;
}

void launch_keys_search(const DevBatch &b, const uint32_t *list, const uint32_t *p_n, uint32_t n_sort, int shift, uint32_t *keys, hipStream_t s)
{
    if (!n_sort) return;
    unsigned blocks = (n_sort + 255) / 256;
    if (blocks > 16384) blocks = 16384;
    hipLaunchKernelGGL(k_keys_search, dim3(blocks), dim3(256), 0, s, b, list, p_n, n_sort, shift, keys);
}

void launch_search_a(const DevIndex &ix, const DevAlignCfg &cfg, const DevBatch &b, const uint32_t *act, const uint32_t *p_n_act, uint32_t n_act_bound,
                     int phase, int cmax, int nstr, int lazy, uint32_t *list, uint32_t *list_cnt, uint32_t *stage, uint32_t *stripe_cnt,
                     hipStream_t s)
{
    uint64_t threads = (uint64_t)n_act_bound * (uint64_t)(cmax * nstr);
    if (!threads) return;
    lazy &= 0xff;
    constexpr int ilp = 2;
    const uint64_t per = (uint64_t)256 * (uint64_t)ilp;
    const uint64_t tiles = (threads + per - 1) / per;
    const unsigned blocks = (unsigned)std::min<uint64_t>(tiles, 16384);
    StripeSet out;
    out.cnt = stripe_cnt;
    out.stage[0] = out.stage[1] = out.stage[2] = stage;
    out.cap = stripe_cap((unsigned)tiles, (unsigned)per);
    static_assert(256 * ilp <= (int)kItemMaxLaneOfs, "a lane's offset within a tile must stay in item_decode's range");
    const ItemGeo ig = item_geo_make((uint32_t)(cmax * nstr), (uint32_t)cmax, (uint64_t)blocks * per);
    const size_t lds = (size_t)b.plan_n * sizeof(uint2);
    hipLaunchKernelGGL(k_search_a_ilp<ilp>, dim3(blocks), dim3(256), lds, s, ix, cfg, b, act, p_n_act, phase, cmax, nstr, lazy, out, ig);
    launch_compact(out, &list, &list_cnt, 1, nullptr, s);
}

void launch_search_b(const DevIndex &ix, const DevAlignCfg &cfg, const DevBatch &b, int phase, int lazy, const uint32_t *list, const uint32_t *sorted,
                     uint32_t n_sorted, const uint32_t *p_n_list, uint64_t n_bound, hipStream_t s)
{
    if (!n_bound) return;
    unsigned blocks = (unsigned)std::min<uint64_t>((n_bound + 255) / 256, 32768);
    const SlotGeo sg = slot_geo_make(b.iv_stride, b.iv_cores);
    const size_t lds = (size_t)b.plan_n * sizeof(uint2);
    if (ix.sa_hi) hipLaunchKernelGGL(k_search_b<true>, dim3(blocks), dim3(256), lds, s, ix, cfg, b, phase, lazy, list, sorted, n_sorted, p_n_list, sg);
    else hipLaunchKernelGGL(k_search_b<false>, dim3(blocks), dim3(256), lds, s, ix, cfg, b, phase, lazy, list, sorted, n_sorted, p_n_list, sg);
}

__global__ void __launch_bounds__(256) k_clear_iv(DevBatch b, const uint32_t *__restrict__ p_n_act, int cmax, int st0, int st1, uint32_t word)
{
    const uint32_t n_act = *p_n_act;
    const uint64_t per_strand = (uint64_t)cmax * n_act, total = per_strand * (uint64_t)(st1 - st0 + 1);
    for (uint64_t i = (uint64_t)blockIdx.x * blockDim.x + threadIdx.x; i < total; i += (uint64_t)gridDim.x * blockDim.x) {
        const int st = st0 + (int)(i / per_strand);
        const uint64_t q = i % per_strand;
        const uint64_t slot = iv_slot(b, (uint32_t)(q % n_act), st, (int)(q / n_act));
        if (b.iv2) b.iv2[slot] = make_uint2(word, word);
        else { b.iv_first[slot] = word ? ~0ULL : 0ULL; b.iv_n[slot] = word; }
    }
}

void launch_clear_iv(const DevBatch &b, const uint32_t *p_n_act, uint32_t n_act_bound, int cmax, int st0, int st1, uint32_t word, hipStream_t s)
{
    const uint64_t total = (uint64_t)n_act_bound * (uint64_t)cmax * (uint64_t)(st1 - st0 + 1);
    if (!total) return;
    const unsigned blocks = (unsigned)std::min<uint64_t>((total + 255) / 256, 16384);
    hipLaunchKernelGGL(k_clear_iv, dim3(blocks), dim3(256), 0, s, b, p_n_act, cmax, st0, st1, word);
}

}

namespace bk { int prof_read_flat(unsigned long long *out16); }
extern "C" int bk_debug_prof(unsigned long long *out16)
{
#if defined(BK_PROF) && BK_PROF == 2
    return bk::prof_read(out16);
#elif defined(BK_PROF)
    return bk::prof_read_flat(out16);
#else
    (void)out16;
    return 1;
#endif
}
```

biokanga_amd/csrc/bk_tune.cpp:

```cpp
#include "bk_engine_int.h"

using namespace bk;

extern "C" {

int bk_ctx_reserve(bk_ctx *c, uint32_t max_batch_reads, uint32_t max_read_len)
{
    if (!c || !max_batch_reads || !max_read_len || max_read_len > (uint32_t)kMaxReadLenAbs) return BK_ERR_PARAMS;
    HIP_TRY(hipSetDevice(c->device));
    const uint32_t n = std::min(max_batch_reads, c->chunk_reads);
    const uint32_t wpr = words_per_read(max_read_len);
    const bool reg_path = c->use_wave && max_read_len <= 16u * (uint32_t)kNwLongest;
    const bool two_bit = reg_path && c->ix.tgt2 != nullptr;
    const uint32_t ivc = iv_cores_for(c, max_read_len);
    int rc = ensure_batch_scratch(c, n, wpr, two_bit ? rd2w_for(max_read_len) : 0u, ivc);
    if (rc) return rc;
    if (c->ix.k2) {
        const uint64_t lanes = (uint64_t)n * ivc * (c->cfg.align_strand == 0 ? 2u : 1u);
        rc = ensure_slist(c, lanes, c->stream);
        if (rc) return rc;
    }
    if (c->sort_lists) { rc = ensure_sort_scratch(c, n, c->stream); if (rc) return rc; }
    if (c->use_wave && c->ix.isa == nullptr) { rc = size_heavy_scratch(c); if (rc) return rc; }
    rc = plan_table_for(c, max_read_len, c->stream);
    if (rc) return rc;
    HIP_TRY(hipStreamSynchronize(c->stream));
    return BK_OK;
}

int bk_ctx_set_chrom_filter(bk_ctx *c, const uint8_t *accept, uint32_t n)
{
    if (!c || (n && !accept)) return BK_ERR_PARAMS;
    HIP_TRY(hipSetDevice(c->device));
    HIP_TRY(hipStreamSynchronize(c->stream));
    c->buf.chrom_accept.reset();
    c->n_chrom_accept = 0;
    if (!n) return BK_OK;
    HIP_TRY(c->buf.chrom_accept.ensure(n));
    HIP_TRY(hipMemcpy(c->buf.chrom_accept.get(), accept, n, hipMemcpyHostToDevice));
    c->n_chrom_accept = n;
    return BK_OK;
}

int bk_ctx_set_params(bk_ctx *c, const bk_align_params *p)
{
    if (!c || !p) return BK_ERR_PARAMS;
    bk_align_params old = c->params;
    c->params = *p;
    if (c->params.max_ml == 0) c->params.max_ml = 1;
    int rc = derive_cfg(c);
    if (rc) { c->params = old; derive_cfg(c); return rc; }
    (void)hipSetDevice(c->device);
    return BK_OK;
}

int64_t bk_ctx_tune(bk_ctx *c, const char *name, int64_t value)
{
    if (!c || !name) return BK_ERR_PARAMS;
    (void)hipSetDevice(c->device);
    std::string n(name);
    if (n == "heavy_thresh") {
        int64_t old = c->cfg.heavy_thresh;
        if (value < 0 || value > 100) return BK_ERR_PARAMS;
        c->cfg.heavy_thresh = (int)value;
        return old;
    }
    if (n == "chunk_reads") {
        int64_t old = c->chunk_reads;
        if (value < 1 || value > (1LL << 30)) return BK_ERR_PARAMS;
        c->chunk_reads = (uint32_t)value;
        return old;
    }
    if (n == "site_chunk") {
        int64_t old = (int64_t)c->site_chunk;
        if (value < 1 || value > (1LL << 30)) return BK_ERR_PARAMS;
        c->site_chunk = (uint64_t)value;
        return old;
    }
    if (n == "kmer_bits" || n == "use_ktab") {
        int64_t old = n == "use_ktab" ? c->use_ktab : c->ix.k;
        if (n == "use_ktab") c->use_ktab = value ? 1 : 0;
        else { if (value < 2 || value > 16) return BK_ERR_PARAMS; c->k_req = (int)value; }
        int rc = build_tables(c);
        return rc ? rc : old;
    }
    if (n == "ktab_wide") {
        int64_t old = c->ktab_wide;
        c->ktab_wide = value < 0 ? 0 : (value > 2 ? 2 : (int)value);
        int rc = build_tables(c);
        return rc ? rc : old;
    }
    if (n == "ktab_packed") return c->ix.ktab_hi != nullptr;
    if (n == "use_k3") {
        int64_t old = c->use_k3;
        c->use_k3 = value < 0 ? 0 : (value > kMoreKeys ? kMoreKeys : (int)value);
        int rc = build_tables(c);
        return rc ? rc : old;
    }
    if (n == "k3_resident") return (c->ix.kx[0] != nullptr) + (c->ix.kx[1] != nullptr);
    if (n == "ktab2_resident") return c->ix.ktab2 != nullptr;
    if (n == "ktab2_elem") return c->ix.ktab2 != nullptr && c->ix.ktab2_elem;
    if (n == "grow_after_reads") { int64_t old = (int64_t)c->grow_after; if (value > 0) c->grow_after = (uint64_t)value; return old; }
    if (n == "grow_state") return c->grow_enabled ? c->grow_state.load() : 5;
    if (n == "image_wait") {
        if (c->grow_enabled) {
            grow_tick(c, 0, true);
            if (c->grow_state.load() != 4 && c->grow_state.load() != 0) grow_take_in(c);
        }
        return (c->ix.kx[0] != nullptr) + (c->ix.kx[1] != nullptr) + (c->ix.ktab2 != nullptr ? 4 : 0);
    }
    if (n == "use_ktab2") {
        int64_t old = c->use_ktab2;
        c->use_ktab2 = value < 0 ? 0 : (value > 2 ? 2 : (int)value);
        c->grow_elem = c->use_ktab2 == 2;
        int rc = build_tables(c);
        return rc ? rc : old;
    }
    if (n == "sort_lists") {
        int64_t old = c->sort_lists;
        c->sort_lists = (int)value & 7;
        c->sort_lists_set = true;
        return old;
    }
    if (n == "use_tgt2") {
        int64_t old = c->use_tgt2;
        c->use_tgt2 = value < 0 ? 0 : (value > 2 ? 2 : (int)value);
        int rc = build_tgt2(c);
        return rc ? rc : old;
    }
    if (n == "wave_waves") {
        int64_t old = c->wave_waves;
        if (value < 64 || value > 65536) return BK_ERR_PARAMS;
        c->wave_waves = (uint32_t)value;
        return old;
    }
    if (n == "async_phases") {
        int64_t old = c->async_phases;
        c->async_phases = value ? 1 : 0;
        return old;
    }
    if (n == "swin_resident") return c->image.swin.get() != nullptr ? 1 : 0;
    if (n == "use_swin") {
        int64_t old = c->use_swin;
        c->use_swin = value < 0 ? 0 : (value > 3 ? 3 : (int)value);
        c->swin_denied = false;
        if (c->image.swin.get() && (!c->use_swin || (c->use_swin == 3) != (c->image.swmap.get() == nullptr))) {
            if (c->stream) (void)hipStreamSynchronize(c->stream);
            drop_swin(c);
        }
        return old;
    }
    if (n == "swin_skip_short") {
        int64_t old = c->swin_skip_short;
        c->swin_skip_short = value < 0 ? 0 : (int)std::min<int64_t>(value, kSwLevels - 1);
        return old;
    }
    if (n == "swin_budget_kb") {
        int64_t old = (int64_t)(c->swin_budget >> 10);
        c->swin_budget = value > 0 ? (uint64_t)value << 10 : 0;
        return old;
    }
    if (n == "swin_mbytes") return (int64_t)(c->swin_bytes >> 20);
    if (n == "swin_setup_us") return (int64_t)(c->swin_setup_s * 1e6);
    if (n == "swin_covered_ppm") return c->image.swin.get() ? (int64_t)(c->swin_covered * 1e6) : 0;
    if (n == "swin_core_lens") return c->image.swmap.get() ? c->swin_w : 0;
    if (n == "use_isa") {
        int64_t old = c->use_isa;
        c->use_isa = value ? 1 : 0;
        int rc = build_tables(c);
        return rc ? rc : old;
    }
    if (n == "use_k2") {
        int64_t old = c->use_k2;
        c->use_k2 = value ? 1 : 0;
        int rc = build_tables(c);
        return rc ? rc : old;
    }
    if (n == "use_iv32") {
        int64_t old = c->use_iv32;
        c->use_iv32 = value ? 1 : 0;
        return old;
    }
    if (n == "lazy_search") {
        int64_t old = c->lazy_search;
        c->lazy_search = value ? 1 : 0;
        return old;
    }
    if (n == "iv_poison") {
        int64_t old = c->iv_poison;
        c->iv_poison = value ? 1 : 0;
        return old;
    }
    if (n == "use_wave") {
        int64_t old = c->use_wave;
        c->use_wave = value ? 1 : 0;
        int rc = build_tables(c);
        return rc ? rc : old;
    }
    if (n == "force_rccl") {
        int64_t old = c->force_rccl ? 1 : 0;
        c->force_rccl = value != 0;
        return old;
    }
    if (n == "rccl_allreduces") return (int64_t)c->rccl_allreduces;
    if (n == "rccl_ranks") return (int64_t)c->rccl_ranks;
    if (n == "debug_stop_phase") {
        int64_t old = c->dbg_stop_phase + 1;
        c->dbg_stop_phase = value <= 0 ? -1 : (int)value - 1;
        c->dbg_valid = false;
        return old;
    }
    if (n == "max_read_len") {
        int64_t old = c->max_read_len;
        if (value < 16 || value > kMaxReadLenAbs) return BK_ERR_PARAMS;
        c->max_read_len = (int)value;
        return old;
    }
    return BK_ERR_PARAMS;
}


uint32_t bk_num_entries(const bk_ctx *c) { return c ? (uint32_t)c->entries.size() : 0; }
int bk_get_entry(const bk_ctx *c, uint32_t idx, bk_entry_info *out)
{
    if (!c || !out || idx >= c->entries.size()) return BK_ERR_PARAMS;
    *out = c->entries[idx];
    return BK_OK;
}
const char *bk_dataset_name(const bk_ctx *c) { return c ? c->dataset.c_str() : ""; }
uint64_t bk_concat_len(const bk_ctx *c) { return c ? c->ix.n : 0; }
int bk_sfx_el_size(const bk_ctx *c) { return c ? (int)c->el_size : 0; }
int bk_min_core_len(const bk_ctx *c) { return c ? c->cfg.min_core_len : 0; }


}
```

Baseline: 723.6 million.

## Add 16-byte quad k-mer table entries with start, key, element and next start

Adds a uint4 k-mer table layout that stores bucket start, key bitmap, the suffix-array element for singleton buckets, and the next bucket start in one entry. The seed search then needs a single 16-byte load instead of two pair loads, and for a singleton bucket with one match it hands the element straight on without a later SA lookup. The table doubles in memory relative to pairs, so it is only chosen when it fits. It is released back to the pair layout if that frees enough room for the sliding-window cache.

```diff
diff --git a/biokanga_amd/csrc/bk_ctx_int.h b/biokanga_amd/csrc/bk_ctx_int.h
--- a/biokanga_amd/csrc/bk_ctx_int.h
+++ b/biokanga_amd/csrc/bk_ctx_int.h
@@ -94,6 +94,9 @@
     bool grow_elem = false, grow_want_elem = false;
     int use_ktab2 = 1;
     bool ktab_is2 = false;
+    bool ktab_is4 = false;
+    int ktab_quad = 1;
+    bool ktab_quad_yielded = false;
     int use_iv32 = 1;
     uint32_t wave_waves = 256u * 8u * 4u;
     int use_isa = 1;
diff --git a/biokanga_amd/csrc/bk_dev_k2.h b/biokanga_amd/csrc/bk_dev_k2.h
--- a/biokanga_amd/csrc/bk_dev_k2.h
+++ b/biokanga_amd/csrc/bk_dev_k2.h
@@ -18,6 +18,24 @@
     const uint32_t m5 = m >> 27, lo5 = (q2 >> 27) & m5, hi5 = lo5 | (~m5 & 31u);
     const uint32_t upto = hi5 == 31u ? 0xFFFFFFFFu : (1u << (hi5 + 1)) - 1u;
     return (bitmap & upto & ~((1u << lo5) - 1u)) == 0u;
+}
+
+struct KtabCarry { uint32_t y, elem; };
+__host__ __device__ __forceinline__ KtabCarry ktab_carry(const uint32_t *__restrict__ k2, const uint32_t *__restrict__ sa, uint64_t lo, uint64_t hi, bool elem_for_key)
+{
+    KtabCarry r;
+    const bool one = hi == lo + 1;
+    r.elem = one && sa != nullptr ? sa[lo] : 0u;
+    r.y = 0u;
+    if (k2 == nullptr) r.y = 0xFFFFFFFFu;
+    else if (one) r.y = elem_for_key && sa != nullptr ? r.elem : k2[lo];
+    else if (hi > lo + kTab2BitmapMax) r.y = 0xFFFFFFFFu;
+    else
+        for (uint64_t i = lo; i < hi; i++) {
+            const uint32_t key = k2[i];
+            if (key != kK2Above) r.y |= 1u << (key >> 27);
+        }
+    return r;
 }
 
 __device__ __forceinline__ int k2_cmp(uint32_t key, uint32_t m, uint32_t q2)
diff --git a/biokanga_amd/csrc/bk_dev_util.h b/biokanga_amd/csrc/bk_dev_util.h
--- a/biokanga_amd/csrc/bk_dev_util.h
+++ b/biokanga_amd/csrc/bk_dev_util.h
@@ -219,6 +219,7 @@
 
 __device__ __forceinline__ uint64_t ktab_get(const DevIndex &ix, uint64_t c)
 {
+    if (ix.ktab4) return (uint64_t)ix.ktab4[c].x;
     if (ix.ktab2) return (uint64_t)ix.ktab2[c].x;
     if (ix.ktab_hi) return ix.ktab_hi[c >> 16] + (uint64_t)ix.ktab32[c];
     return ix.ktab32 ? (uint64_t)ix.ktab32[c] : ix.ktab64[c];
@@ -226,6 +227,12 @@
 
 __device__ __forceinline__ void ktab_get_pair(const DevIndex &ix, uint64_t c, uint64_t &lo, uint64_t &hi)
 {
+    if (ix.ktab4) {
+        const uint4 e = ix.ktab4[c];
+        lo = e.x;
+        hi = e.w;
+        return;
+    }
     if (ix.ktab_hi && !ix.ktab2) {
         const uint64_t base = ix.ktab_hi[c >> 16];
         const uint32_t o0 = ix.ktab32[c], o1 = ix.ktab32[c + 1];
diff --git a/biokanga_amd/csrc/bk_device.h b/biokanga_amd/csrc/bk_device.h
--- a/biokanga_amd/csrc/bk_device.h
+++ b/biokanga_amd/csrc/bk_device.h
@@ -63,6 +63,7 @@
     const uint64_t *ktab_hi;
     const uint2 *ktab2;
     int ktab2_elem;
+    const uint4 *ktab4;
     const uint32_t *k2;
     const uint32_t *kx[kMoreKeys];
     const uint32_t *isa;
diff --git a/biokanga_amd/csrc/bk_engine_int.h b/biokanga_amd/csrc/bk_engine_int.h
--- a/biokanga_amd/csrc/bk_engine_int.h
+++ b/biokanga_amd/csrc/bk_engine_int.h
@@ -31,7 +31,8 @@
 void launch_pack_target(const uint8_t *seq, uint64_t n, uint64_t *tgt4, uint64_t nwords, hipStream_t s);
 void launch_pack_target2(const uint64_t *tgt4, uint64_t nwords4, uint64_t *tgt2, unsigned int *nflag32, int flag_shift, hipStream_t s);
 void launch_split_sa5(const uint8_t *sa5, uint64_t n, uint32_t *lo, uint8_t *hi, hipStream_t s);
-void launch_build_ktab(const DevIndex &ix, void *tab, int k, bool tab64, hipStream_t s, uint64_t i0 = 0, uint64_t i1 = 0, unsigned long long *starts = nullptr, bool pairs = false);
+void launch_build_ktab(const DevIndex &ix, void *tab, int k, bool tab64, hipStream_t s, uint64_t i0 = 0, uint64_t i1 = 0, unsigned long long *starts = nullptr, int words = 1);
+void launch_fill_ktab4(void *tab4, const uint32_t *k2, uint64_t n_entries, hipStream_t s, const uint32_t *sa);
 void launch_fill_ktab2_y(void *tab2, const uint32_t *k2, uint64_t n_entries, hipStream_t s, const uint32_t *sa_elem = nullptr);
 void launch_max_len(const uint32_t *lens, uint32_t n, uint32_t *out, hipStream_t s);
 void launch_widen_lens(const uint16_t *lens16, uint32_t n, uint32_t *lens32, unsigned long long *nwords, hipStream_t s);
@@ -141,6 +142,8 @@
 struct TablePlan {
     bool ktab = false, k2 = false, isa = false;
     bool ktab2 = false;
+    bool ktab4 = false;
+    uint64_t reserve = 0;
     int kx = 0;
     int k = 0;
     DevBuf<unsigned long long> d_bad;
diff --git a/biokanga_amd/csrc/bk_env.h b/biokanga_amd/csrc/bk_env.h
--- a/biokanga_amd/csrc/bk_env.h
+++ b/biokanga_amd/csrc/bk_env.h
@@ -19,6 +19,7 @@
 inline bool inflate_debug() { static const bool v = set("BK_INFLATE_DEBUG"); return v; }
 inline unsigned long long grow_after_reads() { return u64("BK_GROW_AFTER_READS", 0); }
 inline unsigned long long table_slices() { return u64("BK_TABLE_SLICES", 0); }
+inline unsigned long long ktab_quad_max_bytes() { return u64("BK_KTAB_QUAD_MAX_BYTES", 0); }
 inline unsigned long long sa_wide_chunk() { return u64("BK_SA_WIDE_CHUNK", 0); }
 inline unsigned long long sam_device_min(unsigned long long dflt) { const char *e = getenv("BK_SAM_DEVICE_MIN"); return e ? strtoull(e, nullptr, 10) : dflt; }
 inline unsigned long long sam_early_min(unsigned long long dflt) { const char *e = getenv("BK_SAM_EARLY_MIN"); return e ? strtoull(e, nullptr, 10) : dflt; }
diff --git a/biokanga_amd/csrc/bk_image.cpp b/biokanga_amd/csrc/bk_image.cpp
--- a/biokanga_amd/csrc/bk_image.cpp
+++ b/biokanga_amd/csrc/bk_image.cpp
@@ -121,11 +121,12 @@
     ix.ent_start = im.ent_start.get(); ix.ent_end = im.ent_end.get(); ix.ent_id = im.ent_id.get(); ix.id2idx = im.id2idx.get();
     const bool tabs = !c->tables_under_way;
     const void *kt = tabs ? im.ktab.get() : nullptr;
-    const bool packed = c->ktab64 && im.ktab_hi.get() != nullptr, pairs = !c->ktab64 && c->ktab_is2;
+    const bool packed = c->ktab64 && im.ktab_hi.get() != nullptr, quads = !c->ktab64 && c->ktab_is4, pairs = !c->ktab64 && c->ktab_is2 && !quads;
     ix.ktab64 = c->ktab64 && !packed ? static_cast<const uint64_t *>(kt) : nullptr;
     ix.ktab_hi = packed ? im.ktab_hi.get() : nullptr;
     ix.ktab2 = pairs ? static_cast<const uint2 *>(kt) : nullptr;
-    ix.ktab32 = packed || (!c->ktab64 && !pairs) ? static_cast<const uint32_t *>(kt) : nullptr;
+    ix.ktab4 = quads ? static_cast<const uint4 *>(kt) : nullptr;
+    ix.ktab32 = packed || (!c->ktab64 && !pairs && !quads) ? static_cast<const uint32_t *>(kt) : nullptr;
     ix.k2 = tabs ? im.k2.get() : nullptr;
     for (int i = 0; i < kMoreKeys; i++) ix.kx[i] = tabs ? im.kx[i].get() : nullptr;
     ix.ktab2_elem = (ix.ktab2 != nullptr && c->use_ktab2 >= 2 && im.sa_hi.get() == nullptr && ix.k2 != nullptr) ? 1 : 0;
@@ -197,6 +198,7 @@
             (void)hipDeviceSynchronize();
             im.ktab = std::move(im.grow_ktab2);
             c->ktab_is2 = true;
+            c->ktab_is4 = false;
             c->use_ktab2 = c->grow_want_elem ? 2 : 1;
         }
         publish_index(c);
@@ -225,7 +227,7 @@
         c->grow_seen += nreads;
         if ((now || c->grow_seen >= c->grow_after) && c->tables_built && c->ix.k2 != nullptr) {
             c->grow_ix = c->ix;
-            c->grow_want_ktab2 = !c->ktab64 && !c->ktab_is2;
+            c->grow_want_ktab2 = !c->ktab64 && !c->ktab_is2 && !c->ktab_is4;
             c->grow_want_elem = c->grow_elem && c->image.sa_hi.get() == nullptr;
             c->grow_state.store(1);
             c->grow_thread = std::thread(grow_worker, c);
@@ -241,6 +243,7 @@
     im.ktab.reset(); im.ktab_hi.reset(); im.k2.reset(); im.isa.reset();
     for (auto &b : im.kx) b.reset();
     c->ktab_is2 = false;
+    c->ktab_is4 = false;
     c->ix.k = 0;
     c->tables_under_way = true;
     publish_index(c);
@@ -265,7 +268,13 @@
             planned += need;
         }
         if (tp.k2 && c->use_ktab2 && !c->ktab64 && fits(ktab_bytes)) tp.ktab2 = true;
-        HIP_TRY(im.ktab.ensure((size_t)ktab_bytes * (tp.ktab2 ? 2 : 1)));
+        if (tp.ktab2 && c->use_ktab2 == 1 && c->ktab_quad && !c->ktab_quad_yielded && im.sa_hi.get() == nullptr) {
+            planned += tp.reserve;
+            const unsigned long long cap = env::ktab_quad_max_bytes();
+            if (fits(3 * ktab_bytes) && (!cap || 4 * ktab_bytes <= cap)) tp.ktab4 = true;
+            planned -= tp.reserve;
+        }
+        HIP_TRY(im.ktab.ensure((size_t)ktab_bytes * (tp.ktab4 ? 4 : (tp.ktab2 ? 2 : 1))));
         tp.ktab = true;
         tp.k = k;
         if (tp.k2) {
@@ -288,7 +297,7 @@
     ix.k = tp.k;
     const bool last = i1 >= c->ix.n;
     const ImageBufs &im = c->image;
-    if (tp.ktab) launch_build_ktab(ix, im.ktab.get(), tp.k, c->ktab64, c->stream, i0, last ? c->ix.n + 1 : i1, bucket_starts, tp.ktab2);
+    if (tp.ktab) launch_build_ktab(ix, im.ktab.get(), tp.k, c->ktab64, c->stream, i0, last ? c->ix.n + 1 : i1, bucket_starts, tp.ktab4 ? 4 : (tp.ktab2 ? 2 : 1));
     if (tp.k2) launch_build_k2(ix, im.k2.get(), tp.kx > 0 ? im.kx[0].get() : nullptr, tp.kx > 1 ? im.kx[1].get() : nullptr, tp.d_bad.get(), c->stream, i0, i1);
     if (tp.isa) launch_build_isa(im.sa_lo.get(), c->ix.n, im.isa.get(), c->stream, i0, i1);
     HIP_TRY(hipGetLastError());
@@ -320,7 +329,8 @@
         }
     }
     if (tp.ktab) {
-        c->ktab_is2 = tp.ktab2;
+        c->ktab_is2 = tp.ktab2 && !tp.ktab4;
+        c->ktab_is4 = tp.ktab4;
         c->ix.k = tp.k;
     }
     const unsigned long long bad = bad2[0];
@@ -339,11 +349,16 @@
     }
     c->tables_under_way = false;
     publish_index(c);
-    if (tp.ktab2) {
+    if (tp.ktab4) {
+        launch_fill_ktab4(im.ktab.get(), im.k2.get(), (1ULL << (2 * tp.k)) + 1, c->stream, im.sa_lo.get());
+        HIP_TRY(hipGetLastError());
+    } else if (tp.ktab2) {
         launch_fill_ktab2_y(im.ktab.get(), im.k2.get(), (1ULL << (2 * tp.k)) + 1, c->stream, c->ix.ktab2_elem ? im.sa_lo.get() : nullptr);
         HIP_TRY(hipGetLastError());
     }
     HIP_TRY(hipStreamSynchronize(c->stream));
+    if (env::timing() && tp.ktab)
+        fprintf(stderr, "biokanga_amd: k-mer table of order %d: %s, %.2f GB\n", tp.k, tp.ktab4 ? "quads (start, key, element, next start)" : (tp.ktab2 ? "pairs (start, key)" : "bucket starts"), im.ktab.cap() / 1e9);
     if (!c->sort_lists_set) c->sort_lists = (c->sort_lists & ~1) | (c->ix.kx[0] == nullptr ? 1 : 0);
     c->tables_built = true;
     return BK_OK;
@@ -780,6 +795,13 @@
         c->swin_covered = 1.0;
         c->ix.sw_words = words;
     } else {
+        if (c->ktab_is4 && swin_budget_for(c, (uint64_t)free_b + im.ktab.cap() / 2, reserve, words) > swin_budget_for(c, (uint64_t)free_b, reserve, words)) {
+            HIP_TRY(hipDeviceSynchronize());
+            c->ktab_quad_yielded = true;
+            const int rt = build_tables(c);
+            if (rt) return rt;
+            HIP_TRY(hipMemGetInfo(&free_b, &total_b));
+        }
         const uint64_t budget = swin_budget_for(c, (uint64_t)free_b, reserve, words);
         if (!budget) { c->swin_denied = true; return BK_OK; }
         SwinBuild sb;
@@ -874,6 +896,7 @@
         rc = adopt_device_image(c, d_seq.get(), f.concat_len, nullptr, 4);
         d_seq.reset();
         TablePlan tp;
+        tp.reserve = swin_ahead;
         if (!rc) rc = tables_begin(c, tp);
         const uint64_t n = f.concat_len;
         uint64_t n_slices = std::max<uint64_t>(1, std::min<uint64_t>(16, n >> 26));
@@ -964,7 +987,9 @@
     c->ktab64 = src->ktab64;
     c->ktab_wide = src->ktab_wide;
     c->ktab_is2 = src->ktab_is2;
+    c->ktab_is4 = src->ktab_is4;
     c->use_ktab2 = src->use_ktab2;
+    c->ktab_quad = src->ktab_quad; c->ktab_quad_yielded = src->ktab_quad_yielded;
     c->grow_elem = src->grow_elem;
     c->use_k3 = src->use_k3;
     c->sort_lists = src->sort_lists; c->sort_lists_set = src->sort_lists_set;
diff --git a/biokanga_amd/csrc/bk_index.hip b/biokanga_amd/csrc/bk_index.hip
--- a/biokanga_amd/csrc/bk_index.hip
+++ b/biokanga_amd/csrc/bk_index.hip
@@ -236,7 +236,8 @@
     for (uint64_t c = (uint64_t)blockIdx.x * blockDim.x + threadIdx.x; c < span; c += (uint64_t)gridDim.x * blockDim.x) {
         uint64_t lo = ~0ULL, hi = ~0ULL;
         if (c < n_codes) {
-            if (ix.ktab2) { lo = ix.ktab2[c].x; hi = ix.ktab2[c + 1].x; }
+            if (ix.ktab4) { const uint4 e = ix.ktab4[c]; lo = e.x; hi = e.w; }
+            else if (ix.ktab2) { lo = ix.ktab2[c].x; hi = ix.ktab2[c + 1].x; }
             else { lo = ktab_get(ix, c); hi = ktab_get(ix, c + 1); }
         }
         const bool in = c < n_codes && hi != lo && lo >= a && lo < e;
@@ -406,9 +407,9 @@
     hipLaunchKernelGGL(k_split_sa5, dim3((unsigned)blocks), dim3(256), 0, s, sa5, n, lo, hi);
 }
 
-void launch_build_ktab(const DevIndex &ix, void *tab, int k, bool tab64, hipStream_t s, uint64_t i0, uint64_t i1, unsigned long long *starts, bool pairs)
-{
-    const int stride = (pairs && !tab64) ? 2 : 1;
+void launch_build_ktab(const DevIndex &ix, void *tab, int k, bool tab64, hipStream_t s, uint64_t i0, uint64_t i1, unsigned long long *starts, int words)
+{
+    const int stride = tab64 ? 1 : words;
     if (i0 & 63) starts = nullptr;
     if (i1 == 0) i1 = ix.n + 1;
     if (i1 <= i0) return;
@@ -461,14 +462,7 @@
     for (uint64_t c = (uint64_t)blockIdx.x * blockDim.x + threadIdx.x; c < n_entries; c += (uint64_t)gridDim.x * blockDim.x) {
         const uint32_t lo = tab[c];
         const uint64_t hi = c + 1 < n_entries ? (uint64_t)tab[c + 1] : (uint64_t)lo;
-        uint32_t y = 0u;
-        if (hi == (uint64_t)lo + 1) y = sa_elem != nullptr ? sa_elem[lo] : k2[lo];
-        else if (hi > (uint64_t)lo + kTab2BitmapMax) y = 0xFFFFFFFFu;
-        else
-            for (uint64_t i = lo; i < hi; i++) {
-                const uint32_t key = k2[i];
-                if (key != kK2Above) y |= 1u << (key >> 27);
-            }
+        const uint32_t y = ktab_carry(k2, sa_elem, lo, hi, true).y;
         out[c] = make_uint2(lo, y);
     }
 }
@@ -478,17 +472,27 @@
     for (uint64_t c = (uint64_t)blockIdx.x * blockDim.x + threadIdx.x; c < n_entries; c += (uint64_t)gridDim.x * blockDim.x) {
         const uint32_t lo = tab[c].x;
         const uint64_t hi = c + 1 < n_entries ? (uint64_t)tab[c + 1].x : (uint64_t)lo;
-        uint32_t y = 0u;
-        if (k2 == nullptr) y = 0xFFFFFFFFu;
-        else if (hi == (uint64_t)lo + 1) y = sa_elem != nullptr ? sa_elem[lo] : k2[lo];
-        else if (hi > (uint64_t)lo + kTab2BitmapMax) y = 0xFFFFFFFFu;
-        else
-            for (uint64_t i = lo; i < hi; i++) {
-                const uint32_t key = k2[i];
-                if (key != kK2Above) y |= 1u << (key >> 27);
-            }
+        const uint32_t y = ktab_carry(k2, sa_elem, lo, hi, true).y;
         tab[c].y = y;
     }
+}
+
+__global__ void __launch_bounds__(256) k_fill_ktab4(uint4 *__restrict__ tab, const uint32_t *__restrict__ k2, uint64_t n_entries, const uint32_t *__restrict__ sa)
+{
+    uint32_t *__restrict__ w = reinterpret_cast<uint32_t *>(tab);
+    for (uint64_t c = (uint64_t)blockIdx.x * blockDim.x + threadIdx.x; c < n_entries; c += (uint64_t)gridDim.x * blockDim.x) {
+        const uint32_t lo = w[4 * c];
+        const uint32_t hi = c + 1 < n_entries ? w[4 * (c + 1)] : lo;
+        const KtabCarry e = ktab_carry(k2, sa, lo, hi, false);
+        w[4 * c + 1] = e.y;
+        w[4 * c + 2] = e.elem;
+        w[4 * c + 3] = hi;
+    }
+}
+
+void launch_fill_ktab4(void *tab4, const uint32_t *k2, uint64_t n_entries, hipStream_t s, const uint32_t *sa)
+{
+    hipLaunchKernelGGL(k_fill_ktab4, dim3(65536), dim3(256), 0, s, reinterpret_cast<uint4 *>(tab4), k2, n_entries, sa);
 }
 
 void launch_fill_ktab2_y(void *tab2, const uint32_t *k2, uint64_t n_entries, hipStream_t s, const uint32_t *sa_elem)
diff --git a/biokanga_amd/csrc/bk_search.hip b/biokanga_amd/csrc/bk_search.hip
--- a/biokanga_amd/csrc/bk_search.hip
+++ b/biokanga_amd/csrc/bk_search.hip
@@ -50,6 +50,12 @@
 }
 
 
+#ifdef BK_KTAB4_NO_HANDON
+constexpr bool kQuadHandOn = false;
+#else
+constexpr bool kQuadHandOn = true;
+#endif
+
 template <int ILP>
 __global__ void __launch_bounds__(256) k_search_a_ilp(DevIndex ix, DevAlignCfg cfg, DevBatch b, const uint32_t *__restrict__ act,
                                                       const uint32_t *__restrict__ p_n_act, int phase, int cmax, int nstr, int lazy,
@@ -79,6 +85,8 @@
     uint2 cv[ILP];
     bool cached[ILP];
     uint32_t key0[ILP];
+    uint32_t elem0[ILP];
+    const bool tab_y = ix.ktab2 != nullptr || ix.ktab4 != nullptr;
 #pragma unroll
     for (int u = 0; u < ILP; u++) {
         on[u] = false; push[u] = false; have_code[u] = false; slot[u] = 0; p0[u] = 0; q2raw[u] = 0; first[u] = 0; nval[u] = 0; cl[u] = 1; lo[u] = hi[u] = 0;
@@ -127,9 +135,13 @@
         push[u] = on[u];
         have_code[u] = on[u] && !cached[u] && cl[u] >= k && !(p0[u] & 0x4444444444444444ULL & top_mask(k));
         key0[u] = kK2Above;
+        elem0[u] = 0;
         if (have_code[u]) {
             const uint64_t code = (uint64_t)(squeeze2(p0[u]) >> (32 - 2 * k));
-            if (ix.ktab2 != nullptr) {
+            if (ix.ktab4 != nullptr) {
+                const uint4 e = ix.ktab4[code];
+                lo[u] = e.x; hi[u] = e.w; key0[u] = e.y; elem0[u] = e.z;
+            } else if (ix.ktab2 != nullptr) {
                 const uint2 e0 = ix.ktab2[code], e1 = ix.ktab2[code + 1];
                 lo[u] = e0.x; hi[u] = e1.x; key0[u] = e0.y;
             } else {
@@ -145,9 +157,9 @@
     for (int u = 0; u < ILP; u++) {
         const uint64_t size = hi[u] - lo[u];
         const uint32_t m = k2_mask(cl[u] - k);
-        absent[u] = have_code[u] && ix.ktab2 != nullptr && size >= 2 && ktab2_absent(key0[u], m, q2raw[u] & m);
+        absent[u] = have_code[u] && tab_y && size >= 2 && ktab2_absent(key0[u], m, q2raw[u] & m);
         carry[u] = have_code[u] && lazy && ix.ktab2 != nullptr && ix.ktab2_elem && size == 1;
-        const bool key_in_entry = size == 1 && ix.ktab2 != nullptr && !ix.ktab2_elem;
+        const bool key_in_entry = size == 1 && tab_y && !ix.ktab2_elem;
 #pragma unroll
         for (uint32_t j = 0; j < kInlineBucket; j++)
             key[u][j] = (have_code[u] && !absent[u] && !carry[u] && size <= kInlineBucket && j < size) ? (key_in_entry ? key0[u] : ix.k2[lo[u] + j]) : kK2Above;
@@ -193,7 +205,13 @@
                     first[u] = lo[u] + lb;
                     const uint32_t cnt = ub - lb;
                     leave = make_uint2((uint32_t)first[u], cnt);
-                    if (cnt == 0 || cl[u] <= k + kK2Bases) { nval[u] = cnt; push[u] = false; }
+                    if (kQuadHandOn && lazy && ix.ktab4 != nullptr && size == 1 && cnt == 1) {
+                        first[u] = elem0[u];
+                        nval[u] = 1u | kIvFlags;
+                        push[u] = false;
+                        leave = make_uint2(elem0[u], 1u | kIvFlags);
+                    }
+                    else if (cnt == 0 || cl[u] <= k + kK2Bases) { nval[u] = cnt; push[u] = false; }
                     else if (lazy && cnt <= kLazyBucket) { nval[u] = cnt | kLazyFlag; push[u] = false; }
                     else nval[u] = cnt | (kKindDeep << kKindShift);
                 }
diff --git a/biokanga_amd/csrc/bk_tune.cpp b/biokanga_amd/csrc/bk_tune.cpp
--- a/biokanga_amd/csrc/bk_tune.cpp
+++ b/biokanga_amd/csrc/bk_tune.cpp
@@ -98,7 +98,15 @@
         return rc ? rc : old;
     }
     if (n == "k3_resident") return (c->ix.kx[0] != nullptr) + (c->ix.kx[1] != nullptr);
-    if (n == "ktab2_resident") return c->ix.ktab2 != nullptr;
+    if (n == "ktab2_resident") return c->ix.ktab2 != nullptr || c->ix.ktab4 != nullptr;
+    if (n == "ktab4_resident") return c->ix.ktab4 != nullptr;
+    if (n == "ktab_quad") {
+        int64_t old = c->ktab_quad;
+        c->ktab_quad = value ? 1 : 0;
+        c->ktab_quad_yielded = false;
+        int rc = build_tables(c);
+        return rc ? rc : old;
+    }
     if (n == "ktab2_elem") return c->ix.ktab2 != nullptr && c->ix.ktab2_elem;
     if (n == "grow_after_reads") { int64_t old = (int64_t)c->grow_after; if (value > 0) c->grow_after = (uint64_t)value; return old; }
     if (n == "grow_state") return c->grow_enabled ? c->grow_state.load() : 5;
@@ -107,7 +115,7 @@
             grow_tick(c, 0, true);
             if (c->grow_state.load() != 4 && c->grow_state.load() != 0) grow_take_in(c);
         }
-        return (c->ix.kx[0] != nullptr) + (c->ix.kx[1] != nullptr) + (c->ix.ktab2 != nullptr ? 4 : 0);
+        return (c->ix.kx[0] != nullptr) + (c->ix.kx[1] != nullptr) + (c->ix.ktab2 != nullptr || c->ix.ktab4 != nullptr ? 4 : 0);
     }
     if (n == "use_ktab2") {
         int64_t old = c->use_ktab2;
```

Result: faster. 731.5 million, median of 6 (+1.1%).
